# topling/toplingdb

Hardware: NVIDIA H100
Metric: compaction_input_kv_MB_per_s (higher is better)
Workload: dtype u8

## Files before the change

toplingdb_b200/csrc/api.cu:

```cuda
#include <cuda_runtime.h>
#include <stdio.h>
#include <stdlib.h>
#include <string.h>

#include <algorithm>
#include <map>
#include <memory>
#include <mutex>
#include <unordered_map>
#include <string>
#include <thread>
#include <type_traits>
#include <vector>

#include "../../include/b200c.h"
#include "inflate_rules.h"
#include "kernels.h"
#include "range_plan.h"
#include "scan.cuh"
#include "sst_host.h"

using namespace b200c;

namespace {

thread_local std::string g_err;
size_t g_last_want = 0;
std::mutex g_host_allocs_mu;
std::unordered_map<void*, std::pair<size_t, int>> g_host_allocs;
int fail(int code, const std::string& msg) {
  g_err = msg;
  return code;
}
std::string mem_note() {
  size_t fr = 0, tot = 0;
  cudaMemGetInfo(&fr, &tot);
  cudaGetLastError();
  return " (requested " + std::to_string(g_last_want) + " bytes; device free " + std::to_string(fr) + " of " + std::to_string(tot) + ")";
}
#define CU(call)                                                                                                  \
  do {                                                                                                            \
    cudaError_t e_ = (call);                                                                                      \
    if (e_ != cudaSuccess) {                                                                                      \
      cudaGetLastError();                                                                                         \
      return fail(e_ == cudaErrorMemoryAllocation ? B200C_ERR_OUT_OF_MEMORY : B200C_ERR_CUDA,                      \
                  std::string(#call) + ": " + cudaGetErrorString(e_) + (e_ == cudaErrorMemoryAllocation ? mem_note() : ""));  \
    }                                                                                                             \
  } while (0)

constexpr int kCacheDevices = 16;
inline size_t size_class(size_t n) {
  size_t c = 4096;
  while (c < n) c <<= 1;
  if (c >= (size_t(1) << 20)) {
    const size_t step = c >> 4;
    c = (c >> 1) + ((n - (c >> 1) + step - 1) / step) * step;
  }
  return c;
}
class BufCache {
 public:
  BufCache(bool host, const char* env, size_t default_mb) : host_(host) {
    const char* e = getenv(env);
    cap_ = (e ? strtoull(e, nullptr, 10) : default_mb) << 20;
  }
  void* take(int dev, size_t n, size_t* got) {
    if (dev < 0 || dev >= kCacheDevices || cap_ == 0) return nullptr;
    std::lock_guard<std::mutex> l(mu_);
    auto it = free_[dev].lower_bound(n);
    if (it == free_[dev].end() || it->first > 2 * n) return nullptr;
    void* p = it->second;
    *got = it->first;
    held_[dev] -= it->first;
    free_[dev].erase(it);
    return p;
  }
  bool give(int dev, void* p, size_t n) {
    if (dev < 0 || dev >= kCacheDevices || cap_ == 0) return false;
    std::lock_guard<std::mutex> l(mu_);
    if (held_[dev] + n > cap_) return false;
    free_[dev].emplace(n, p);
    held_[dev] += n;
    return true;
  }
  void flush(int dev) {
    if (dev < 0 || dev >= kCacheDevices) return;
    std::multimap<size_t, void*> drop;
    {
      std::lock_guard<std::mutex> l(mu_);
      drop.swap(free_[dev]);
      held_[dev] = 0;
    }
    for (auto& kv : drop) {
      if (host_) cudaFreeHost(kv.second);
      else cudaFree(kv.second);
    }
  }

 private:
  bool host_;
  size_t cap_ = 0;
  std::mutex mu_;
  std::multimap<size_t, void*> free_[kCacheDevices];
  size_t held_[kCacheDevices] = {};
};
BufCache& dev_cache() {
  static BufCache* c = new BufCache(false, "B200C_CACHE_DEVICE_MB", 49152);
  return *c;
}
BufCache& host_cache() {
  static BufCache* c = new BufCache(true, "B200C_CACHE_HOST_MB", 16384);
  return *c;
}
inline int current_device() {
  int d = -1;
  cudaGetDevice(&d);
  return d;
}
cudaError_t cached_alloc(bool host, size_t n, void** out, size_t* cap, int* dev_out) {
  const int dev = current_device();
  const size_t want = size_class(n);
  *dev_out = dev;
  BufCache& c = host ? host_cache() : dev_cache();
  if (void* p = c.take(dev, want, cap)) {
    *out = p;
    return cudaSuccess;
  }
  g_last_want = want;
  auto raw = [&]() { return host ? cudaHostAlloc(out, want, cudaHostAllocMapped | cudaHostAllocPortable) : cudaMalloc(out, want); };
  cudaError_t e = raw();
  if (e == cudaErrorMemoryAllocation) {
    cudaGetLastError();
    dev_cache().flush(dev);
    host_cache().flush(dev);
    e = raw();
  }
  if (e == cudaSuccess) *cap = want;
  return e;
}
void cached_free(bool host, void* p, size_t cap, int dev) {
  if (!p) return;
  if ((host ? host_cache() : dev_cache()).give(dev, p, cap)) return;
  if (host) cudaFreeHost(p);
  else cudaFree(p);
}

template <bool kPinned>
struct Buf {
  uint8_t* p = nullptr;
  size_t cap = 0;
  int dev = -1;
  Buf() = default;
  Buf(Buf&& o) noexcept : p(o.p), cap(o.cap), dev(o.dev) {
    o.p = nullptr;
    o.cap = 0;
  }
  Buf(const Buf&) = delete;
  Buf& operator=(const Buf&) = delete;
  ~Buf() { cached_free(kPinned, p, cap, dev); }
  cudaError_t reserve(size_t n) {
    if (n <= cap) return cudaSuccess;
    if (p) kPinned ? cudaFreeHost(p) : cudaFree(p);
    p = nullptr;
    cap = 0;
    void* q = nullptr;
    const cudaError_t e = cached_alloc(kPinned, n + (n >> 4) + 256, &q, &cap, &dev);
    if (e == cudaSuccess) p = static_cast<uint8_t*>(q);
    return e;
  }
  template <class T>
  T* as() const {
    return reinterpret_cast<T*>(p);
  }
};
using DevBuf = Buf<false>;
using HostBuf = Buf<true>;
static_assert(!std::is_copy_constructible_v<DevBuf> && !std::is_copy_assignable_v<DevBuf>, "a buffer has one owner");

struct KeyBufs {
  DevBuf pfx, tr, vref, meta;
  cudaError_t reserve(uint64_t n) {
    cudaError_t e = pfx.reserve(16 * (n + 1));
    if (e == cudaSuccess) e = tr.reserve(8 * (n + 1));
    if (e == cudaSuccess) e = vref.reserve(8 * (n + 1));
    if (e == cudaSuccess) e = meta.reserve(4 * (n + 1));
    return e;
  }
  KeyColsMut mut() const { return {pfx.as<ulonglong2>(), tr.as<uint64_t>(), vref.as<uint64_t>(), meta.as<uint32_t>()}; }
  KeyCols cols(uint64_t n) const { return {pfx.as<ulonglong2>(), tr.as<uint64_t>(), vref.as<uint64_t>(), meta.as<uint32_t>(), n}; }
};

struct Input {
  int level;
  uint64_t file_number;
  const uint8_t* data;
  uint64_t len;
  int mem_kind;
  DevBuf staged;
  cudaEvent_t up_ev = nullptr;
  bool uploaded = false;
  bool shared_copy = false;
  DevBuf index_inflated;
  std::vector<uint8_t> index_host;
  const uint8_t* dev = nullptr;
  InputTail tail;
};
constexpr uint64_t kTailFetch = 4096;
struct Output {
  b200c_file_meta meta;
  uint64_t dev_off = 0;
  uint64_t host_off = 0;
};
struct KernelTime {
  const char* name;
  cudaEvent_t a, b;
  float us;
};

}

struct b200c_job {
  b200c_params p;
  std::vector<uint64_t> snapshots, fct;
  std::string cf_name, db_id, db_session_id, db_host_id;
  std::vector<Input> inputs;
  std::vector<Output> outputs;
  b200c_stats stats;
  int stage_done = 0;
  uint64_t launches = 0;
  int sms = 132;
  cudaStream_t st = nullptr;
  cudaStream_t st2 = nullptr;
  cudaStream_t st_up = nullptr;
  cudaEvent_t ev[5] = {nullptr, nullptr, nullptr, nullptr, nullptr};
  cudaEvent_t evx[4] = {nullptr, nullptr, nullptr, nullptr};
  DevBuf files_d, blk_off, blk_size, blk_state, scan_tmp, run_start, small;
  KeyBufs dec, mrg;
  DevBuf splits, tile_state, snaps_d;
  DevBuf esz, eshared, tstat, nxt, disk, rows, tstate, grows, gstate, gflag, gsync, idx_contrib, idx_contrib_off, blocks, files_rec, idx_esz, idx_eoff, idx_sep, out_buf, out_base_d;
  uint64_t n_total = 0, n_out = 0, nblk_in = 0, nblocks_out = 0;
  uint32_t nfiles_out = 0, nruns = 0;
  DevBuf bloom_contrib, bloom_contrib_off;
  DevBuf bloom_hashes;
  DevBuf kv_arena, kv_offs, kv_klens;
  DevBuf run_bounds, run_first_d;
  std::vector<uint64_t> run_start_h;
  HostBuf host_out;
  std::vector<GpKey> gp_small, gp_large;
  std::vector<uint64_t> gp_size;
  std::vector<uint8_t> gp_same;
  DevBuf gp_keys_d, gp_ranks_d, gp_size_d, gp_same_d, gp_cuts_d;
  BoundKey range_lo{}, range_hi{};
  DevBuf clip_d;
  DevBuf cslot, cslot_off, arena;
  std::vector<cudaEvent_t> range_events;
  std::vector<std::string> range_bounds;
  cudaEvent_t wait_ev = nullptr;
  DevBuf vfiles_d, vrun_start;
  HostBuf pin_small, pin_tails, pin_rd, pin_up;
  size_t pin_up_used = 0;
  std::vector<KernelTime> ktimes;
  size_t kt_used = 0;
  size_t kt_begin(const char* name, cudaStream_t s = nullptr) {
    if (!p.profile) return 0;
    if (kt_used == ktimes.size()) {
      KernelTime k{name, nullptr, nullptr, 0.f};
      cudaEventCreate(&k.a);
      cudaEventCreate(&k.b);
      ktimes.push_back(k);
    }
    ktimes[kt_used].name = name;
    cudaEventRecord(ktimes[kt_used].a, s ? s : st);
    return kt_used++;
  }
  void kt_end(size_t slot = ~(size_t)0, cudaStream_t s = nullptr) {
    if (!p.profile) return;
    cudaEventRecord(ktimes[slot == ~(size_t)0 ? kt_used - 1 : slot].b, s ? s : st);
  }
};

namespace {

enum { kSlotErr = 0, kSlotTicket = 1, kSlotTotalIn = 2, kSlotMinS1 = 3, kSlotTotals = 4 , kSlotDecTicket = 6, kSlotGpCuts = 7, kSlotCounters = 8 , kSlotClip = 16 , kSlotStitchDone = 18, kSlotArena = 19 , kSmallSlots = 32 };

int map_dev_err(uint32_t e) {
  e &= ~(uint32_t)kFlagHasSingleDelete;
  if (e == 0) return B200C_OK;
  std::string m = "device reported:";
  int code = B200C_ERR_CORRUPTION;
  if (e & kErrCorruptBlock) m += " corrupt-block";
  if (e & kErrChecksum) m += " block-checksum-mismatch";
  if (e & kErrKeyOrder) m += " key-order/partition";
  if (e & kErrCountMismatch) m += " entry-count-mismatch";
  if (e & kErrParanoid) m += " Paranoid checksums do not match (an output file does not read back as written)";
  if (e & kErrSingleDelContract) m += " SingleDelete and Delete of the same key in one snapshot stripe (enforce_single_del_contracts)";
  const uint32_t unsup = kErrKeyTooLong | kErrValueTooLong | kErrBadType | kErrCompressed | kErrBlockTooLong | kErrIrregularRestarts |
                         kErrGroupTooLong | kErrSdWriteConflict;
  if (e & unsup) {
    if (!(e & ~(unsup))) code = B200C_ERR_NOT_SUPPORTED;
    if (e & kErrKeyTooLong) m += " user-key-longer-than-16-bytes";
    if (e & kErrValueTooLong) m += " value>=128MiB";
    if (e & kErrBadType) m += " value-type-outside-{Value,Deletion,SingleDeletion}";
    if (e & kErrGroupTooLong) m += " SingleDelete-on-a-key-with-too-many-versions-or-with-more-than-16-runs";
    if (e & kErrSdWriteConflict) m += " SingleDelete-with-an-earliest_write_conflict_snapshot";
    if (e & kErrCompressed) m += " compressed-block";
    if (e & kErrBlockTooLong) m += " output-block-with-too-many-entries";
    if (e & kErrIrregularRestarts) m += " restart-intervals-of-unequal-length";
  }
  if (e & kErrInternal) {
    m += " internal";
    code = B200C_ERR_CUDA;
  }
  return fail(code, m);
}

bool trailer_ok(const Input& in, const uint8_t* blk, uint64_t size, const uint8_t* trailer) {
  const uint32_t stored = (uint32_t)trailer[1] | (uint32_t)trailer[2] << 8 | (uint32_t)trailer[3] << 16 | (uint32_t)trailer[4] << 24;
  return !in.tail.checksum_type || host_block_checksum(in.tail.checksum_type, blk, size, trailer[0]) == stored;
}

int fetch_tail(b200c_job* j, Input& in, const uint8_t* prefetched = nullptr) {
  auto read = [&](uint64_t off, uint64_t n, std::vector<uint8_t>& buf) -> int {
    buf.resize(n);
    if (in.mem_kind == B200C_MEM_HOST) {
      memcpy(buf.data(), in.data + off, n);
    } else {
      CU(cudaMemcpyAsync(buf.data(), in.data + off, n, cudaMemcpyDeviceToHost, j->st));
      CU(cudaStreamSynchronize(j->st));
    }
    return B200C_OK;
  };
  if (in.len < 53) return fail(B200C_ERR_CORRUPTION, "input shorter than a footer");
  const uint64_t tail_n = std::min<uint64_t>(in.len, kTailFetch);
  std::vector<uint8_t> tail, tmp;
  int rc = B200C_OK;
  if (prefetched) tail.assign(prefetched, prefetched + tail_n);
  else rc = read(in.len - tail_n, tail_n, tail);
  if (rc) return rc;
  std::string e = parse_footer(tail.data() + tail_n - 53, in.len, &in.tail);
  if (!e.empty()) return fail(B200C_ERR_CORRUPTION, e);
  auto view = [&](uint64_t off, uint64_t n, const uint8_t** p) -> int {
    if (off >= in.len - tail_n && off + n <= in.len) {
      *p = tail.data() + (off - (in.len - tail_n));
      return B200C_OK;
    }
    int r = read(off, n, tmp);
    *p = tmp.data();
    return r;
  };
  const uint8_t* blk;
  rc = view(in.tail.meta_off, in.tail.meta_size + 5, &blk);
  if (rc) return rc;
  if (!trailer_ok(in, blk, in.tail.meta_size, blk + in.tail.meta_size)) return fail(B200C_ERR_CORRUPTION, "metaindex block checksum mismatch");
  std::map<std::string, std::pair<uint64_t, uint64_t>> meta;
  e = parse_metaindex(blk, in.tail.meta_size, &meta);
  if (!e.empty()) return fail(B200C_ERR_CORRUPTION, e);
  for (auto& kv : meta) {
    if (kv.first == "rocksdb.range_del") in.tail.has_range_del = true;
    if (kv.first.compare(0, 11, "fullfilter.") == 0 || kv.first.compare(0, 18, "partitionedfilter.") == 0) in.tail.has_filter = true;
    if (kv.first == "rocksdb.compression_dict") in.tail.has_dict = true;
  }
  auto it = meta.find("rocksdb.properties");
  if (it == meta.end()) return fail(B200C_ERR_CORRUPTION, "input has no properties block");
  in.tail.props_off = it->second.first;
  in.tail.props_size = it->second.second;
  if (in.tail.props_off + in.tail.props_size + 5 > in.len) return fail(B200C_ERR_CORRUPTION, "properties handle out of range");
  rc = view(in.tail.props_off, in.tail.props_size + 5, &blk);
  if (rc) return rc;
  if (!trailer_ok(in, blk, in.tail.props_size, blk + in.tail.props_size)) return fail(B200C_ERR_CORRUPTION, "properties block checksum mismatch");
  e = parse_properties(blk, in.tail.props_size, &in.tail);
  if (!e.empty()) return fail(B200C_ERR_CORRUPTION, e);
  if (in.tail.index_type != 0)
    return fail(B200C_ERR_NOT_SUPPORTED, "input index type " + std::to_string(in.tail.index_type) + " (only kBinarySearch runs on the device)");
  if (in.tail.has_range_del || in.tail.num_range_deletions)
    return fail(B200C_ERR_NOT_SUPPORTED, "input holds range tombstones (CompactionRangeDelAggregator is not on the device path)");
  if (in.tail.num_merge_operands) return fail(B200C_ERR_NOT_SUPPORTED, "input holds merge operands");
  if (in.tail.has_dict) return fail(B200C_ERR_NOT_SUPPORTED, "input uses a compression dictionary");
  if (!in.tail.comparator_name.empty() && in.tail.comparator_name != "leveldb.BytewiseComparator")
    return fail(B200C_ERR_NOT_SUPPORTED, "comparator " + in.tail.comparator_name + " (only leveldb.BytewiseComparator runs on the device)");
  if (in.tail.num_data_blocks > 0xffffffffull) return fail(B200C_ERR_NOT_SUPPORTED, "too many data blocks");
  return B200C_OK;
}

bool input_is_compressed(const Input& in) { return !in.tail.compression_name.empty() && in.tail.compression_name != "NoCompression"; }
int host_inflated_index(const Input& in, std::vector<uint8_t>* out) {
  out->clear();
  const uint64_t off = in.tail.index_off, size = in.tail.index_size;
  if (off + size + 5 > in.len) return fail(B200C_ERR_CORRUPTION, "index handle out of range");
  uint8_t trailer[5];
  if (in.mem_kind == B200C_MEM_HOST) memcpy(trailer, in.data + off + size, 5);
  else CU(cudaMemcpy(trailer, in.data + off + size, 5, cudaMemcpyDeviceToHost));
  if (trailer[0] == 0) return B200C_OK;
  if (trailer[0] != 2) return fail(B200C_ERR_NOT_SUPPORTED, "index block compressed with a codec the device path does not decode");
  std::vector<uint8_t> comp;
  const uint8_t* cp = in.data + off;
  if (in.mem_kind != B200C_MEM_HOST) {
    comp.resize(size);
    CU(cudaMemcpy(comp.data(), in.data + off, size, cudaMemcpyDeviceToHost));
    cp = comp.data();
  }
  if (!trailer_ok(in, cp, size, trailer)) return fail(B200C_ERR_CORRUPTION, "index block checksum mismatch");
  uint64_t u = 0;
  uint32_t h = 0;
  for (int sft = 0; h < 5 && h < size; sft += 7) {
    const uint8_t c = cp[h++];
    u |= (uint64_t)(c & 127) << sft;
    if (c < 128) break;
  }
  if (u < 8 || u > (1ull << 31)) return fail(B200C_ERR_CORRUPTION, "compressed index block announces a bad size");
  out->resize(u);
  std::unique_ptr<b200c::InfWork> iw(new b200c::InfWork);
  if (b200c::inflate_raw(cp + h, (uint32_t)(size - h), out->data(), (uint32_t)u, iw.get()) != (long)u)
    return fail(B200C_ERR_CORRUPTION, "compressed index block does not inflate to its announced size");
  return B200C_OK;
}

int host_index_block(const Input& in, std::vector<uint8_t>* buf, const uint8_t** blk, uint64_t* len) {
  if (in.tail.index_off + in.tail.index_size + 5 > in.len) return fail(B200C_ERR_CORRUPTION, "index handle out of range");
  buf->clear();
  if (input_is_compressed(in))
    if (int rc = host_inflated_index(in, buf)) return rc;
  if (!buf->empty()) {
    *blk = buf->data();
    *len = buf->size();
    return B200C_OK;
  }
  *blk = in.data + in.tail.index_off;
  *len = in.tail.index_size;
  if (in.mem_kind != B200C_MEM_HOST) {
    buf->resize(*len);
    CU(cudaMemcpy(buf->data(), *blk, *len, cudaMemcpyDeviceToHost));
    *blk = buf->data();
  }
  return B200C_OK;
}

void ikey_bytes(const KeyRec& k, uint8_t* out, uint32_t* len) {
  uint32_t n = 0;
  for (uint32_t t = 0; t < k.ulen && t < 16; t++) out[n++] = (uint8_t)((t < 8 ? k.hi >> (56 - 8 * t) : k.lo >> (56 - 8 * (t - 8))) & 0xff);
  for (int t = 0; t < 8; t++) out[n++] = (uint8_t)(k.tr >> (8 * t));
  *len = n;
}

int upload_small(b200c_job* j, void* dev_dst, const void* host_src, size_t n) {
  const size_t kCap = 256 * 1024;
  CU(j->pin_up.reserve(kCap));
  const size_t off = (j->pin_up_used + 15) & ~(size_t)15;
  if (off + n > kCap) {
    CU(cudaMemcpyAsync(dev_dst, host_src, n, cudaMemcpyHostToDevice, j->st));
    return B200C_OK;
  }
  memcpy(j->pin_up.p + off, host_src, n);
  j->pin_up_used = off + n;
  launch_copy_small(j->pin_up.p + off, dev_dst, (uint32_t)n, j->st);
  return B200C_OK;
}

constexpr size_t kRdSmall = kSmallSlots * 8;
int gather_small(b200c_job* j, const FileRec* files) {
  const uint64_t* small = j->small.as<uint64_t>();
  CU(j->pin_rd.reserve(kRdSmall + sizeof(FileRec) * (size_t)kMaxOutFiles));
  launch_gather_small(small, (uint32_t)kRdSmall, files, files ? small + kSlotTotals + 1 : nullptr, j->pin_rd.p, j->st);
  return B200C_OK;
}
void take_small(b200c_job* j, uint64_t* h, const FileRec* files, std::vector<FileRec>* frs) {
  memcpy(h, j->pin_rd.p, kRdSmall);
  if (files && frs) {
    uint64_t n = h[kSlotTotals + 1];
    if (n > kMaxOutFiles) n = kMaxOutFiles;
    frs->resize(n);
    memcpy(frs->data(), j->pin_rd.p + kRdSmall, sizeof(FileRec) * n);
  }
}
int read_small(b200c_job* j, uint64_t* h, const FileRec* files = nullptr, std::vector<FileRec>* frs = nullptr) {
  if (int rc = gather_small(j, files)) return rc;
  CU(cudaStreamSynchronize(j->st));
  CU(cudaGetLastError());
  take_small(j, h, files, frs);
  return B200C_OK;
}
int checked_sync(b200c_job* j, uint64_t* h, const FileRec* files = nullptr, std::vector<FileRec>* frs = nullptr) {
  if (int rc = read_small(j, h, files, frs)) return rc;
  return map_dev_err((uint32_t)h[kSlotErr]);
}

int write_tails(b200c_job* j, const std::vector<FileRec>& frs, const std::vector<uint64_t>& base_off) {
  const b200c_params& P = j->p;
  const uint32_t nfiles = (uint32_t)frs.size();
  j->outputs.resize(nfiles);
  std::vector<TailCopy> tcs(nfiles);
  for (uint32_t f = 0; f < nfiles; f++) {
    const FileRec& fr = frs[f];
    OutputTailInput ti;
    ti.checksum_type = P.checksum;
    ti.format_version = P.format_version;
    ti.data_size = fr.data_size;
    ti.index_size = fr.index_size;
    ti.filter_size = fr.filter_bytes ? fr.filter_bytes - 5 : 0;
    ti.filter_entries = fr.filter_entries;
    ti.num_entries = fr.n_entries;
    ti.num_deletions = fr.num_deletions;
    ti.raw_key_size = fr.raw_key_size;
    ti.raw_value_size = fr.raw_value_size;
    ti.num_data_blocks = fr.n_blocks;
    ti.index_key_is_user_key = !fr.index_has_seq && P.format_version > 2;
    ti.column_family_id = P.column_family_id;
    ti.column_family_name = j->cf_name;
    ti.db_id = j->db_id;
    ti.db_session_id = j->db_session_id;
    ti.db_host_id = j->db_host_id;
    ti.creation_time = P.creation_time;
    ti.oldest_key_time = P.oldest_key_time;
    ti.file_creation_time = j->fct.empty() ? 0 : j->fct[std::min<size_t>(f, j->fct.size() - 1)];
    ti.orig_file_number = P.first_file_number + f;
    std::vector<uint8_t> tail = build_output_tail(ti);
    const uint64_t tail_off = fr.data_size + fr.filter_bytes + fr.index_size + 5;
    if (tail_off + tail.size() > base_off[f + 1] - base_off[f]) return fail(B200C_ERR_CUDA, "internal: output image overflow");
    const size_t so = (size_t)f * 4096;
    if (tail.size() > 4096) return fail(B200C_ERR_CUDA, "internal: tail larger than its staging slot");
    memcpy(j->pin_tails.p + so, tail.data(), tail.size());
    tcs[f] = TailCopy{base_off[f] + tail_off, (uint32_t)so, (uint32_t)tail.size()};
    Output& o = j->outputs[f];
    memset(&o.meta, 0, sizeof o.meta);
    o.dev_off = base_off[f];
    o.meta.file_number = ti.orig_file_number;
    o.meta.file_size = tail_off + tail.size();
    o.meta.smallest_seqno = fr.smallest_seq;
    o.meta.largest_seqno = fr.largest_seq;
    o.meta.num_entries = fr.n_entries;
    o.meta.num_deletions = fr.num_deletions;
    o.meta.raw_key_size = fr.raw_key_size;
    o.meta.raw_value_size = fr.raw_value_size;
    o.meta.num_data_blocks = fr.n_blocks;
    o.meta.data_size = fr.data_size;
    o.meta.index_size = fr.index_size;
    ikey_bytes(fr.smallest, o.meta.smallest_ikey, &o.meta.smallest_ikey_len);
    ikey_bytes(fr.largest, o.meta.largest_ikey, &o.meta.largest_ikey_len);
    j->stats.total_output_bytes += o.meta.file_size;
  }
  const size_t rec_bytes = sizeof(TailCopy) * nfiles;
  memcpy(j->pin_small.p, tcs.data(), rec_bytes);
  launch_scatter_tails(reinterpret_cast<const TailCopy*>(j->pin_small.p), nfiles, j->pin_tails.p, j->out_buf.as<uint8_t>(), j->st);
  j->launches++;
  return B200C_OK;
}

int paranoid_reread(b200c_job* j, KeyCols mcols, const std::vector<FileRec>& frs, const std::vector<uint64_t>& base_off) {
  const b200c_params& P = j->p;
  cudaStream_t st = j->st;
  const uint32_t nfiles = (uint32_t)frs.size();
  const uint64_t nblocks = j->nblocks_out, n_out = mcols.n;
  uint64_t* small = j->small.as<uint64_t>();
  uint32_t* err = reinterpret_cast<uint32_t*>(small + kSlotErr);
  std::vector<FileDesc> ofd(nfiles);
  uint32_t g = 0, maxb = 0;
  for (uint32_t f = 0; f < nfiles; f++) {
    const FileRec& fr = frs[f];
    FileDesc d;
    memset(&d, 0, sizeof d);
    d.base = j->out_buf.as<uint8_t>() + base_off[f];
    d.len = j->outputs[f].meta.file_size;
    d.index_off = fr.data_size + fr.filter_bytes;
    d.index_size = (uint32_t)fr.index_size;
    d.value_delta = P.format_version >= 4;
    d.cksum = P.checksum;
    d.gblk_first = g;
    d.nblocks = (uint32_t)fr.n_blocks;
    d.index_user_key = (!fr.index_has_seq && P.format_version > 2) ? 1u : 0u;
    g += d.nblocks;
    maxb = std::max(maxb, d.nblocks);
    ofd[f] = d;
  }
  if (g != nblocks) return fail(B200C_ERR_CUDA, "internal: block count of the outputs changed");
  CU(j->vfiles_d.reserve(sizeof(FileDesc) * nfiles));
  if (int rc = upload_small(j, j->vfiles_d.p, ofd.data(), sizeof(FileDesc) * nfiles)) return rc;
  CU(cudaStreamSynchronize(st));
  CU(j->blk_off.reserve(8 * (nblocks + 1)));
  CU(j->blk_size.reserve(4 * (nblocks + 1)));
  CU(j->blk_state.reserve(8 * (nblocks + 1)));
  CU(j->vrun_start.reserve(8 * ((size_t)nfiles + 1)));
  CU(j->dec.reserve(n_out));
  if (const char* flip = getenv("B200C_TEST_FLIP_OUTPUT_BYTE")) {
    const uint64_t at = strtoull(flip, nullptr, 10);
    if (at < j->outputs[0].meta.file_size) launch_flip_byte(j->out_buf.as<uint8_t>() + base_off[0] + at, st);
  }
  CU(cudaMemsetAsync(small + kSlotDecTicket, 0, 8, st));
  CU(cudaMemsetAsync(small + kSlotTotalIn, 0, 8, st));
  CU(cudaMemsetAsync(j->vrun_start.p, 0, 8 * ((size_t)nfiles + 1), st));
  CU(cudaMemsetAsync(j->blk_state.p, 0, 8 * (nblocks + 1), st));
  const FileDesc* vf = j->vfiles_d.as<FileDesc>();
  j->kt_begin("verify.reread");
  launch_index_decode(vf, (int)nfiles, maxb, j->blk_off.as<uint64_t>(), j->blk_size.as<uint32_t>(), BoundKey{}, 0, BoundKey{}, 0, err, st);
  launch_block_decode_fused(vf, (int)nfiles, j->blk_off.as<uint64_t>(), j->blk_size.as<uint32_t>(), (uint32_t)nblocks, 1, n_out, j->dec.mut(),
                            j->blk_state.as<unsigned long long>(), reinterpret_cast<uint32_t*>(small + kSlotDecTicket),
                            j->vrun_start.as<uint64_t>(), small + kSlotTotalIn, err, j->sms, st);
  launch_compare_columns(mcols, j->dec.cols(n_out), n_out, err, j->sms, st);
  j->kt_end();
  j->launches += 3;
  uint64_t hv[kSmallSlots];
  if (int rc = read_small(j, hv)) return rc;
  if ((uint32_t)hv[kSlotErr] & ~(uint32_t)kFlagHasSingleDelete) {
    map_dev_err((uint32_t)hv[kSlotErr]);
    const std::string detail = g_err;
    return fail(B200C_ERR_CORRUPTION, "Paranoid checksums do not match: " + detail);
  }
  if (hv[kSlotTotalIn] != n_out) return fail(B200C_ERR_CORRUPTION, "Paranoid checksums do not match (entry count of the outputs)");
  return B200C_OK;
}

int encode_stage(b200c_job* j, KeyCols mcols, uint64_t n_out, uint32_t min_s1, uint32_t max_s1, EncodeWork& W, uint32_t* err, uint64_t* small) {
  const b200c_params& P = j->p;
  cudaStream_t st = j->st;
  uint64_t h[kSmallSlots];
  std::vector<FileRec> frs;
  std::vector<uint64_t> base_off;
  if (n_out) {
    if (P.index_block_restart_interval != 1)
      return fail(B200C_ERR_NOT_SUPPORTED, "index_block_restart_interval != 1 is not built on the device");
    EncodeParams ep{};
    ep.block_size = P.block_size;
    ep.block_size_limit = P.block_size_deviation ? (uint32_t)(((uint64_t)P.block_size * (100 - P.block_size_deviation) + 99) / 100) : 0;
    ep.restart_interval = P.block_restart_interval;
    ep.checksum = P.checksum;
    ep.format_version = P.format_version;
    ep.output_level = (uint32_t)P.output_level;
    ep.max_output_file_size = P.max_output_file_size;
    if (!j->gp_small.empty() && P.output_level > 0) {
      const uint32_t G = (uint32_t)j->gp_small.size();
      CU(j->gp_keys_d.reserve(sizeof(GpKey) * 2 * G));
      CU(j->gp_ranks_d.reserve(8 * 3 * (size_t)G));
      CU(j->gp_size_d.reserve(8 * (size_t)G));
      CU(j->gp_same_d.reserve(G + 16));
      CU(j->gp_cuts_d.reserve(sizeof(GpCut) * (2 * (size_t)G + 2)));
      GpKey* keys = j->gp_keys_d.as<GpKey>();
      if (int rc = upload_small(j, keys, j->gp_small.data(), sizeof(GpKey) * G)) return rc;
      if (int rc = upload_small(j, keys + G, j->gp_large.data(), sizeof(GpKey) * G)) return rc;
      if (int rc = upload_small(j, j->gp_size_d.p, j->gp_size.data(), 8 * (size_t)G)) return rc;
      if (int rc = upload_small(j, j->gp_same_d.p, j->gp_same.data(), G)) return rc;
      uint64_t* ranks = j->gp_ranks_d.as<uint64_t>();
      launch_gp_ranks(mcols, keys, keys + G, G, ranks, ranks + G, ranks + 2 * G, st);
      j->launches += 1;
      ep.gp.n = G;
      ep.gp.dynamic_file_size = P.level_compaction_dynamic_file_size;
      ep.gp.lo = ranks;
      ep.gp.eq = ranks + G;
      ep.gp.hi = ranks + 2 * G;
      ep.gp.size = j->gp_size_d.as<uint64_t>();
      ep.gp.next_same = j->gp_same_d.as<uint8_t>();
      ep.gp.target_output_file_size = P.target_output_file_size ? P.target_output_file_size : P.max_output_file_size;
      ep.gp.max_compaction_bytes = P.max_compaction_bytes ? P.max_compaction_bytes : ep.gp.target_output_file_size * 25;
      ep.gp_cuts = j->gp_cuts_d.as<GpCut>();
      ep.gp_ncuts = reinterpret_cast<uint32_t*>(small + kSlotGpCuts);
    }
    uint64_t hop = (uint64_t)(P.block_size - 1) / std::max<uint32_t>(min_s1, 1) + 3;
    if (hop > (uint64_t)kEncHalo) return fail(B200C_ERR_NOT_SUPPORTED, "block_size / smallest entry exceeds the encoder's 2048-entry block window");
    const uint32_t hc = (uint32_t)hop;
    const uint64_t etiles = (n_out + kEncTile - 1) / kEncTile;
    CU(j->rows.reserve(sizeof(TileRow) * etiles * hc));
    CU(j->tstate.reserve(sizeof(TileState) * etiles));
    const uint64_t egroups = (etiles + kEncGroupTiles - 1) / kEncGroupTiles;
    CU(j->grows.reserve(sizeof(TileRow) * egroups * hc));
    CU(j->gstate.reserve(sizeof(TileState) * egroups));
    CU(j->gflag.reserve(4 * egroups));
    CU(j->nxt.reserve(2 * (n_out + 1)));
    CU(j->disk.reserve(4 * (n_out + 1)));
    CU(j->files_rec.reserve(sizeof(FileRec) * (kMaxOutFiles + 2)));
    W.rows = j->rows.as<TileRow>();
    W.tstate = j->tstate.as<TileState>();
    W.grows = j->grows.as<TileRow>();
    W.gstate = j->gstate.as<TileState>();
    W.gflag = j->gflag.as<uint32_t>();
    W.nxt = j->nxt.as<uint16_t>();
    W.disk = j->disk.as<uint32_t>();
    W.files = j->files_rec.as<FileRec>();
    W.scan_tmp = j->scan_tmp.as<uint64_t>();
    CU(j->gsync.reserve(8 * egroups + 16));
    CU(cudaMemsetAsync(j->gsync.p, 0, 8 * egroups + 16, st));
    W.gdone = j->gsync.as<uint32_t>();
    W.gready = W.gdone + egroups;
    uint32_t* sflag = reinterpret_cast<uint32_t*>(small + kSlotStitchDone);
    CU(cudaEventRecord(j->evx[0], st));
    CU(cudaStreamWaitEvent(j->st2, j->evx[0], 0));
    {
      const size_t slot = j->kt_begin("~encode.stitch", j->st2);
      launch_encode_stitch(mcols, ep, W, etiles, hc, err, 1, sflag, j->st2, &j->launches);
      j->kt_end(slot, j->st2);
    }
    j->kt_begin("encode.tables");
    launch_encode_tables(mcols, ep, W, etiles, hc, max_s1, err, st);
    j->kt_end();
    {
      const size_t slot = j->kt_begin("~encode.stitch_retry", j->st2);
      launch_encode_stitch(mcols, ep, W, etiles, hc, err, 2, sflag, j->st2, &j->launches);
      j->kt_end(slot, j->st2);
    }
    CU(cudaEventRecord(j->evx[1], j->st2));
    CU(cudaStreamWaitEvent(st, j->evx[1], 0));
    j->kt_begin("encode.tilestate");
    launch_encode_tilestate(mcols, W, etiles, hc, err, st, &j->launches);
    j->kt_end();
    j->launches += 1;
    if (P.bloom_millibits_per_key) {
      j->kt_begin("encode.bloom_count");
      CU(j->bloom_hashes.reserve(8 * (n_out + 1)));
      launch_bloom_count(mcols, n_out, W.files, small + kSlotTotals + 1, P.bloom_millibits_per_key, j->bloom_hashes.as<uint64_t>(), j->sms, st);
      j->kt_end();
      j->launches += 2;
    }
    if (int rc = checked_sync(j, h, W.files, &frs)) return rc;
    const uint64_t nblocks = j->nblocks_out = h[kSlotTotals];
    const uint32_t nfiles = j->nfiles_out = (uint32_t)h[kSlotTotals + 1];
    if (nfiles == 0 || nfiles > kMaxOutFiles) return fail(B200C_ERR_CUDA, "internal: bad output file count");
    CU(j->blocks.reserve(sizeof(BlockRec) * (nblocks + 1)));
    CU(j->idx_esz.reserve(4 * (nblocks + 1)));
    CU(j->idx_eoff.reserve(8 * (nblocks + 1)));
    CU(j->idx_sep.reserve(sizeof(KeyRec) * (nblocks + 1)));
    W.blocks = j->blocks.as<BlockRec>();
    W.idx_esz = j->idx_esz.as<uint32_t>();
    W.idx_eoff = j->idx_eoff.as<uint64_t>();
    W.idx_sep = j->idx_sep.as<KeyRec>();
    CU(j->pin_tails.reserve((size_t)nfiles * 4096 + 64));
    CU(j->pin_small.reserve(sizeof(TailCopy) * nfiles));
    base_off.resize(nfiles + 1);
    uint64_t off = 0;
    for (uint32_t f = 0; f < nfiles; f++) {
      base_off[f] = off;
      uint64_t cap = frs[f].data_size + frs[f].filter_bytes + frs[f].n_blocks * 48 + 64 + 4096;
      off += (cap + 255) & ~255ull;
    }
    base_off[nfiles] = off;
    CU(j->out_buf.reserve(off + 256));
    {
      std::vector<uint64_t> coff(nfiles + 1, 0);
      for (uint32_t f = 0; f < nfiles; f++) coff[f + 1] = coff[f] + (frs[f].n_blocks * 48 + 64) / 1024 + 1;
      CU(j->idx_contrib.reserve(64 * (coff[nfiles] + 1)));
      CU(j->idx_contrib_off.reserve(8 * (nfiles + 1)));
      if (int rc = upload_small(j, j->idx_contrib_off.p, coff.data(), 8 * (nfiles + 1))) return rc;
      W.idx_contrib = j->idx_contrib.as<uint64_t>();
      W.idx_contrib_off = j->idx_contrib_off.as<uint64_t>();
    }
    std::vector<uint8_t*> bases(nfiles);
    for (uint32_t f = 0; f < nfiles; f++) bases[f] = j->out_buf.as<uint8_t>() + base_off[f];
    CU(j->out_base_d.reserve(8 * nfiles));
    if (int rc = upload_small(j, j->out_base_d.p, bases.data(), 8 * nfiles)) return rc;
    uint8_t* const* out_base_d = j->out_base_d.as<uint8_t*>();
    j->kt_begin("encode.blocklist");
    launch_encode_blocklist(mcols, ep, W, etiles, nblocks, err, st);
    j->kt_end();
    j->kt_begin("encode.filestats+index_size");
    launch_encode_index_size(mcols, ep, W, nblocks, j->sms, st, &j->launches);
    launch_encode_filestats(mcols, W, nfiles, st);
    j->kt_end();
    if (int rc = gather_small(j, W.files)) return rc;
    CU(cudaEventRecord(j->evx[2], st));
    uint64_t data_bytes = 0;
    for (uint32_t f = 0; f < nfiles; f++) data_bytes += frs[f].data_size;
    j->kt_begin("encode.emit");
    launch_encode_emit(mcols, ep, W, nblocks, out_base_d, data_bytes, err, j->sms, st);
    j->kt_end();
    j->launches += 3;
    CU(cudaStreamWaitEvent(j->st2, j->evx[2], 0));
    {
      const size_t slot = j->kt_begin("~encode.index", j->st2);
      launch_encode_index_write(ep, W, nblocks, nfiles, out_base_d, j->sms, j->st2, &j->launches);
      j->kt_end(slot, j->st2);
    }
    CU(cudaEventRecord(j->evx[3], j->st2));
    if (P.bloom_millibits_per_key) {
      j->kt_begin("encode.bloom_build");
      std::vector<uint64_t> boff(nfiles + 1, 0);
      uint64_t max_fb = 0;
      for (uint32_t f = 0; f < nfiles; f++) {
        boff[f + 1] = boff[f] + frs[f].filter_bytes / 1024 + 1;
        max_fb = std::max<uint64_t>(max_fb, frs[f].filter_bytes);
      }
      CU(j->bloom_contrib.reserve(64 * (boff[nfiles] + 1)));
      CU(j->bloom_contrib_off.reserve(8 * (nfiles + 1)));
      if (int rc = upload_small(j, j->bloom_contrib_off.p, boff.data(), 8 * (nfiles + 1))) return rc;
      launch_bloom_build(j->bloom_hashes.as<uint64_t>(), n_out, W.files, nfiles, (uint32_t)std::min<uint64_t>(max_fb, 0xffffffffull), P.bloom_millibits_per_key, P.checksum,
                         out_base_d, j->bloom_contrib.as<uint64_t>(), j->bloom_contrib_off.as<uint64_t>(), st);
      j->kt_end();
      j->launches += 3;
    }
    CU(cudaEventSynchronize(j->evx[2]));
    CU(cudaGetLastError());
    take_small(j, h, W.files, &frs);
    CU(cudaStreamWaitEvent(st, j->evx[3], 0));
    int rc = map_dev_err((uint32_t)h[kSlotErr]);
    if (rc == B200C_OK && frs.size() != nfiles) rc = fail(B200C_ERR_CUDA, "internal: output file count changed");
    if (rc == B200C_OK) rc = write_tails(j, frs, base_off);
    if (rc != B200C_OK) {
      cudaStreamSynchronize(st);
      return rc;
    }
    if (P.paranoid_file_checks) {
      if (int rc = checked_sync(j, h)) return rc;
      return paranoid_reread(j, mcols, frs, base_off);
    }
  }
  return B200C_OK;
}

int finish_run(b200c_job* j) {
  const b200c_params& P = j->p;
  cudaStream_t st = j->st;
  CU(cudaEventRecord(j->ev[3], st));
  if (P.output_mem == B200C_MEM_HOST) {
    uint64_t tot = 0;
    for (auto& o : j->outputs) {
      o.host_off = tot;
      tot += (o.meta.file_size + 63) & ~63ull;
    }
    CU(j->host_out.reserve(tot + 64));
    for (auto& o : j->outputs)
      CU(cudaMemcpyAsync(j->host_out.p + o.host_off, j->out_buf.as<uint8_t>() + o.dev_off, o.meta.file_size, cudaMemcpyDeviceToHost, st));
  }
  CU(cudaEventRecord(j->ev[4], st));
  {
    uint64_t h[kSmallSlots];
    if (int rc = checked_sync(j, h)) return rc;
  }
  float ms;
  cudaEventElapsedTime(&ms, j->ev[0], j->ev[1]);
  j->stats.decode_us = ms * 1000.0;
  cudaEventElapsedTime(&ms, j->ev[1], j->ev[2]);
  j->stats.merge_us = ms * 1000.0;
  cudaEventElapsedTime(&ms, j->ev[2], j->ev[3]);
  j->stats.encode_us = ms * 1000.0;
  cudaEventElapsedTime(&ms, j->ev[0], j->ev[4]);
  j->stats.total_us = ms * 1000.0;
  for (size_t i = 0; i < j->kt_used; i++) {
    float kms = 0;
    cudaEventElapsedTime(&kms, j->ktimes[i].a, j->ktimes[i].b);
    j->ktimes[i].us = kms * 1000.f;
  }
  j->stats.num_output_files = j->nfiles_out;
  j->stats.kernel_launches = j->launches;
  j->stage_done = 3;
  return B200C_OK;
}

int encode_columns(b200c_job* j, uint64_t n, const void* pfx, const void* tr, const void* vref, const void* meta, bool prepared = false);

int run_merge_encode(b200c_job* j, int until, KeyCols decc, RunBounds runs, uint64_t n_decoded, uint64_t N, bool clipped,
                     uint64_t range_value_bytes, uint64_t* small, uint32_t* err);

int job_prepare(b200c_job* j) {
  CU(cudaSetDevice(j->p.device));
  if (!j->st) {
    CU(cudaStreamCreateWithFlags(&j->st, cudaStreamNonBlocking));
    {
      int prio_lo = 0, prio_hi = 0;
      CU(cudaDeviceGetStreamPriorityRange(&prio_lo, &prio_hi));
      CU(cudaStreamCreateWithPriority(&j->st2, cudaStreamNonBlocking, prio_hi));
    }
    for (auto& e : j->ev) CU(cudaEventCreate(&e));
    for (auto& e : j->evx) CU(cudaEventCreateWithFlags(&e, cudaEventDisableTiming));
    cudaDeviceProp prop;
    CU(cudaGetDeviceProperties(&prop, j->p.device));
    j->sms = prop.multiProcessorCount;
  }
  j->outputs.clear();
  j->stage_done = 0;
  j->launches = 0;
  j->nblocks_out = 0;
  j->nfiles_out = 0;
  j->kt_used = 0;
  j->pin_up_used = 0;
  memset(&j->stats, 0, sizeof j->stats);
  return B200C_OK;
}

int run_job(b200c_job* j, int until) {
  const b200c_params& P = j->p;
  if (int rc = job_prepare(j)) return rc;
  cudaStream_t st = j->st;
  if (j->wait_ev) CU(cudaStreamWaitEvent(st, j->wait_ev, 0));
  const int k = (int)j->inputs.size();
  if (k == 0) return fail(B200C_ERR_INVALID_ARGUMENT, "job has no inputs");

  CU(cudaEventRecord(j->ev[0], st));
  uint64_t nblk = 0, n_props = 0, in_bytes = 0;
  bool any_compressed = false;
  std::vector<FileDesc> fds(k);
  {
    bool any_dev = false;
    for (int i = 0; i < k; i++) any_dev = any_dev || j->inputs[i].mem_kind != B200C_MEM_HOST;
    if (any_dev) {
      CU(j->pin_small.reserve((size_t)k * kTailFetch));
      for (int i = 0; i < k; i++) {
        const Input& in = j->inputs[i];
        if (in.mem_kind == B200C_MEM_HOST || in.len < 53) continue;
        const uint64_t tn = std::min<uint64_t>(in.len, kTailFetch);
        CU(cudaMemcpyAsync(j->pin_small.p + (size_t)i * kTailFetch, in.data + in.len - tn, tn, cudaMemcpyDeviceToHost, st));
      }
      CU(cudaStreamSynchronize(st));
    }
  }
  for (int i = 0; i < k; i++) {
    Input& in = j->inputs[i];
    int rc = fetch_tail(j, in, in.mem_kind != B200C_MEM_HOST && in.len >= 53 ? j->pin_small.p + (size_t)i * kTailFetch : nullptr);
    if (rc) return rc;
    if (in.mem_kind == B200C_MEM_HOST) {
      if (in.uploaded) {
        CU(cudaStreamWaitEvent(st, in.up_ev, 0));
        in.uploaded = false;
      } else {
        CU(in.staged.reserve(in.len + 64));
        CU(cudaMemcpyAsync(in.staged.p, in.data, in.len, cudaMemcpyHostToDevice, st));
      }
      in.dev = in.staged.as<uint8_t>();
    } else {
      if ((uintptr_t)in.data & 15) return fail(B200C_ERR_INVALID_ARGUMENT, "device input images must be 16-byte aligned");
      in.dev = in.data;
    }
    FileDesc& fd = fds[i];
    fd.base = in.dev;
    fd.len = in.len;
    fd.index_off = in.tail.index_off;
    fd.index_size = (uint32_t)in.tail.index_size;
    fd.value_delta = in.tail.format_version >= 4;
    fd.cksum = in.tail.checksum_type;
    fd.gblk_first = (uint32_t)nblk;
    fd.nblocks = (uint32_t)in.tail.num_data_blocks;
    fd.index_user_key = in.tail.index_key_is_user_key ? 1u : 0u;
    fd.index_ptr = nullptr;
    if (input_is_compressed(in)) any_compressed = true;
    nblk += in.tail.num_data_blocks;
    n_props += in.tail.num_entries;
    in_bytes += in.len;
    if (in.tail.index_size > 0xffffffffull) return fail(B200C_ERR_NOT_SUPPORTED, "index block >= 4 GiB");
  }
  if (any_compressed) {
    std::vector<int> rcs(k, B200C_OK);
    std::vector<std::string> msgs(k);
    std::vector<std::thread> pool;
    for (int i = 0; i < k; i++) {
      if (!input_is_compressed(j->inputs[i])) continue;
      pool.emplace_back([&, i]() {
        cudaSetDevice(P.device);
        rcs[i] = host_inflated_index(j->inputs[i], &j->inputs[i].index_host);
        if (rcs[i]) msgs[i] = g_err;
      });
    }
    for (auto& th : pool) th.join();
    for (int i = 0; i < k; i++) {
      if (rcs[i]) return fail(rcs[i], msgs[i]);
      Input& in = j->inputs[i];
      if (!input_is_compressed(in) || in.index_host.empty()) continue;
      CU(in.index_inflated.reserve(in.index_host.size() + 64));
      CU(cudaMemcpyAsync(in.index_inflated.p, in.index_host.data(), in.index_host.size(), cudaMemcpyHostToDevice, st));
      fds[i].index_ptr = in.index_inflated.as<uint8_t>();
      fds[i].index_size = (uint32_t)in.index_host.size();
    }
  }
  if (nblk > 0xfffffff0ull) return fail(B200C_ERR_NOT_SUPPORTED, "too many data blocks");
  j->nblk_in = nblk;
  j->n_total = n_props;
  j->stats.num_input_files = k;
  j->stats.total_input_bytes = in_bytes;
  j->stats.num_input_records = n_props;

  CU(j->small.reserve(kSmallSlots * 8));
  CU(cudaMemsetAsync(j->small.p, 0, kSmallSlots * 8, st));
  uint64_t* small = j->small.as<uint64_t>();
  uint32_t* err = reinterpret_cast<uint32_t*>(small + kSlotErr);
  {
    uint32_t ff = 0xffffffffu;
    if (int rc = upload_small(j, small + kSlotMinS1, &ff, 4)) return rc;
  }
  CU(j->files_d.reserve(sizeof(FileDesc) * k));
  if (int rc = upload_small(j, j->files_d.p, fds.data(), sizeof(FileDesc) * k)) return rc;
  const uint64_t N = n_props;
  CU(j->blk_off.reserve(8 * (nblk + 1)));
  CU(j->blk_size.reserve(4 * (nblk + 1)));
  CU(j->blk_state.reserve(8 * (nblk + 1)));
  CU(j->scan_tmp.reserve(8 * ((std::max<uint64_t>(nblk, N) / kScanTile) + 2)));
  CU(j->run_start.reserve(8 * (k + 1)));
  CU(j->dec.reserve(N));
  const FileDesc* files_d = j->files_d.as<FileDesc>();

  uint32_t maxb = 0;
  for (auto& f : fds) maxb = std::max(maxb, f.nblocks);
  if (nblk) {
    j->kt_begin("decode.index");
    launch_index_decode(files_d, k, maxb, j->blk_off.as<uint64_t>(), j->blk_size.as<uint32_t>(), j->range_lo, P.has_range_start, j->range_hi,
                        P.has_range_end, err, st);
    j->kt_end();
    j->launches++;
  }
  const uint8_t* arena = nullptr;
  if (nblk && any_compressed) {
    CU(j->cslot.reserve(4 * (nblk + 1)));
    CU(j->cslot_off.reserve(8 * (nblk + 1)));
    j->kt_begin("decode.inflate");
    launch_block_usize(files_d, j->blk_off.as<uint64_t>(), j->blk_size.as<uint32_t>(), (uint32_t)nblk, j->cslot.as<uint32_t>(), err, st);
    exclusive_scan<uint32_t>(j->cslot.as<uint32_t>(), j->cslot_off.as<uint64_t>(), nblk, j->scan_tmp.as<uint64_t>(), small + kSlotArena, st, &j->launches);
    uint64_t hc[kSmallSlots];
    if (int rc = checked_sync(j, hc)) return rc;
    CU(j->arena.reserve(hc[kSlotArena] + 256));
    arena = j->arena.as<uint8_t>();
    launch_inflate_blocks(files_d, j->blk_off.as<uint64_t>(), j->blk_size.as<uint32_t>(), j->cslot.as<uint32_t>(), j->cslot_off.as<uint64_t>(),
                          (uint32_t)nblk, j->arena.as<uint8_t>(), P.verify_input_checksums, err, j->sms, st);
    j->kt_end();
    j->launches += 3;
  }
  CU(cudaMemsetAsync(j->run_start.p, 0, 8 * (k + 1), st));
  if (nblk) {
    CU(cudaMemsetAsync(j->blk_state.p, 0, 8 * (nblk + 1), st));
    j->kt_begin("decode.blocks");
    launch_block_decode_fused(files_d, k, j->blk_off.as<uint64_t>(), j->blk_size.as<uint32_t>(), (uint32_t)nblk, P.verify_input_checksums, N,
                              j->dec.mut(), j->blk_state.as<unsigned long long>(), reinterpret_cast<uint32_t*>(small + kSlotDecTicket),
                              j->run_start.as<uint64_t>(), small + kSlotTotalIn, err, j->sms, st, arena);
    j->kt_end();
    j->launches++;
  }
  CU(cudaEventRecord(j->ev[1], st));
  const KeyCols decc = j->dec.cols(N);
  if (until == 1) {
    uint64_t h[kSmallSlots];
    j->run_start_h.resize(k + 1);
    CU(cudaMemcpyAsync(j->run_start_h.data(), j->run_start.p, 8 * (k + 1), cudaMemcpyDeviceToHost, st));
    if (int rc = checked_sync(j, h)) return rc;
    if (h[kSlotTotalIn] != N && !(P.has_range_start || P.has_range_end))
      return fail(B200C_ERR_CORRUPTION, "decoded entry count differs from rocksdb.num.entries");
    j->stage_done = 1;
    j->stats.kernel_launches = j->launches;
    return B200C_OK;
  }

  std::vector<uint32_t> run_first;
  for (int i = 0; i < k; i++)
    if (i == 0 || j->inputs[i].level <= 0 || j->inputs[i].level != j->inputs[i - 1].level) run_first.push_back((uint32_t)i);
  const uint32_t K = (uint32_t)run_first.size();
  run_first.push_back((uint32_t)k);
  if (K > (uint32_t)kMaxRuns) return fail(B200C_ERR_NOT_SUPPORTED, "more than 64 sorted runs (L0 files + levels)");
  j->nruns = K;
  CU(j->run_bounds.reserve(16 * (size_t)(K + 1)));
  CU(j->run_first_d.reserve(4 * (size_t)(K + 2)));
  if (int rc = upload_small(j, j->run_first_d.p, run_first.data(), 4 * (size_t)(K + 1))) return rc;
  launch_run_bounds(decc, j->run_start.as<uint64_t>(), j->run_first_d.as<uint32_t>(), K, j->run_bounds.as<uint64_t>(), err, st);
  j->launches++;
  RunBounds runs{j->run_bounds.as<uint64_t>(), j->run_bounds.as<uint64_t>() + K};
  const bool clipped = P.has_range_start || P.has_range_end;
  const uint64_t n_decoded = N;
  uint64_t N_in = N, range_value_bytes = 0;
  if (clipped) {
    CU(j->clip_d.reserve(16 * (size_t)(K + 1)));
    j->kt_begin("merge.clip");
    launch_clip_runs(decc, runs, K, j->range_lo, P.has_range_start, j->range_hi, P.has_range_end,
                     j->clip_d.as<uint64_t>(), reinterpret_cast<unsigned long long*>(small + kSlotClip), st);
    j->kt_end();
    j->launches++;
    uint64_t hc[kSmallSlots];
    if (int rc = checked_sync(j, hc)) return rc;
    N_in = hc[kSlotClip];
    range_value_bytes = hc[kSlotClip + 1];
    if (N_in > n_decoded) return fail(B200C_ERR_CUDA, "internal: clipped entry count exceeds the input");
    runs = RunBounds{j->clip_d.as<uint64_t>(), j->clip_d.as<uint64_t>() + K};
    j->stats.num_input_records = N_in;
  }
  return run_merge_encode(j, until, decc, runs, n_decoded, N_in, clipped, range_value_bytes, small, err);
}

int run_merge_encode(b200c_job* j, int until, KeyCols decc, RunBounds runs, uint64_t n_decoded, uint64_t N, bool clipped,
                     uint64_t range_value_bytes, uint64_t* small, uint32_t* err) {
  const b200c_params& P = j->p;
  cudaStream_t st = j->st;
  const size_t k = j->nruns;
  const uint64_t mtiles = (N + kMergeNominal - 1) / kMergeNominal;
  CU(j->splits.reserve(8 * (mtiles + 1) * k));
  CU(j->tile_state.reserve(8 * (mtiles + 1)));
  CU(cudaMemsetAsync(j->tile_state.p, 0, 8 * (mtiles + 1), st));
  CU(j->snaps_d.reserve(8 * (P.num_snapshots + 1)));
  if (P.num_snapshots)
    if (int rc = upload_small(j, j->snaps_d.p, j->snapshots.data(), 8 * P.num_snapshots)) return rc;
  CU(j->mrg.reserve(N));
  CU(j->esz.reserve(4 * (N + 1)));
  CU(j->eshared.reserve(N + 1));
  CU(j->tstat.reserve(sizeof(TileStat) * (mtiles + 2)));
  MergeParams mp;
  mp.nruns = (uint32_t)k;
  mp.bottommost = P.bottommost_level != 0;
  mp.nsnapshots = P.num_snapshots;
  mp.snapshots = j->snaps_d.as<uint64_t>();
  mp.earliest_snapshot = P.num_snapshots ? j->snapshots[0] : kMaxSeq;
  mp.filter = P.compaction_filter;
  mp.ttl = P.ttl;
  mp.now = P.ttl_now;
  mp.write_conflict_snapshot = P.earliest_write_conflict_snapshot != 0 && P.earliest_write_conflict_snapshot < kMaxSeq;
  MergeCounters* counters = reinterpret_cast<MergeCounters*>(small + kSlotCounters);
  EncodeWork W;
  memset(&W, 0, sizeof W);
  W.esz = j->esz.as<uint32_t>();
  W.eshared = j->eshared.as<uint8_t>();
  W.tstat = j->tstat.as<TileStat>();
  W.min_s1 = reinterpret_cast<uint32_t*>(small + kSlotMinS1);
  W.totals = small + kSlotTotals;
  if (N) {
    j->kt_begin("merge.partition");
    launch_merge_partition(decc, runs, (uint32_t)k, N, mtiles, j->splits.as<uint64_t>(), err, j->sms, st);
    j->kt_end();
    const MergeSizes msz{W.esz, W.eshared, W.tstat, W.min_s1};
    W.tprefix = j->tile_state.as<unsigned long long>();
    W.nstat = mtiles;
    j->kt_begin("merge.tiles");
    launch_merge_tiles(decc, runs, mp, N, mtiles, j->splits.as<uint64_t>(),
                       j->tile_state.as<unsigned long long>(), reinterpret_cast<uint32_t*>(small + kSlotTicket), j->mrg.mut(), counters, msz, err, st);
    j->kt_end();
    j->kt_begin("merge.sizes_fix");
    launch_merge_sizes_fix(j->mrg.cols(0), j->tile_state.as<unsigned long long>(), mtiles, msz, st);
    j->kt_end();
    j->launches += 3;
  }
  CU(cudaEventRecord(j->ev[2], st));
  uint64_t h[kSmallSlots];
  if (int rc = checked_sync(j, h)) return rc;
  if (clipped ? h[kSlotTotalIn] > n_decoded : h[kSlotTotalIn] != n_decoded)
    return fail(B200C_ERR_CORRUPTION, "decoded entry count differs from rocksdb.num.entries");
  MergeCounters mc;
  memcpy(&mc, h + kSlotCounters, sizeof mc);
  const uint64_t n_out = mc.n_out;
  j->n_out = n_out;
  j->stats.num_output_records = n_out;
  j->stats.num_input_deletion_records = mc.n_input_deletions;
  j->stats.num_records_replaced = mc.n_hidden;
  j->stats.num_expired_deletion_records = mc.n_obsolete;
  j->stats.num_record_drop_user = mc.n_user_drop;
  j->stats.total_input_raw_key_bytes = mc.raw_key_bytes;
  {
    uint64_t all = 0;
    for (auto& in : j->inputs) all += in.tail.raw_value_size;
    if (clipped) all = range_value_bytes;
    j->stats.total_input_raw_value_bytes = all - mc.raw_value_bytes;
  }
  if (until == 2) {
    j->stage_done = 2;
    j->stats.kernel_launches = j->launches;
    return B200C_OK;
  }

  if (int rc = encode_stage(j, j->mrg.cols(n_out), n_out, (uint32_t)h[kSlotMinS1], (uint32_t)(h[kSlotMinS1] >> 32), W, err, small)) return rc;
  return finish_run(j);
}

int encode_columns(b200c_job* j, uint64_t n, const void* pfx, const void* tr, const void* vref, const void* meta, bool prepared) {
  int rc = prepared ? B200C_OK : job_prepare(j);
  if (rc) return rc;
  cudaStream_t st = j->st;
  CU(cudaEventRecord(j->ev[0], st));
  CU(cudaEventRecord(j->ev[1], st));
  CU(cudaEventRecord(j->ev[2], st));
  CU(j->small.reserve(kSmallSlots * 8));
  CU(cudaMemsetAsync(j->small.p, 0, kSmallSlots * 8, st));
  uint64_t* small = j->small.as<uint64_t>();
  uint32_t* err = reinterpret_cast<uint32_t*>(small + kSlotErr);
  uint32_t ff = 0xffffffffu;
  CU(cudaMemcpyAsync(small + kSlotMinS1, &ff, 4, cudaMemcpyHostToDevice, st));
  MergeCounters* counters = reinterpret_cast<MergeCounters*>(small + kSlotCounters);
  CU(cudaMemcpyAsync(&counters->n_out, &n, 8, cudaMemcpyHostToDevice, st));
  CU(j->esz.reserve(4 * (n + 1)));
  CU(j->eshared.reserve(n + 1));
  CU(j->tstat.reserve(sizeof(TileStat) * (n / kEncTile + 2)));
  CU(j->tile_state.reserve(8 * (n / kEncTile + 2)));
  CU(j->scan_tmp.reserve(8 * ((n / kScanTile) + 2)));
  EncodeWork W;
  memset(&W, 0, sizeof W);
  W.esz = j->esz.as<uint32_t>();
  W.eshared = j->eshared.as<uint8_t>();
  W.tstat = j->tstat.as<TileStat>();
  W.min_s1 = reinterpret_cast<uint32_t*>(small + kSlotMinS1);
  W.totals = small + kSlotTotals;
  KeyCols mcols{static_cast<const ulonglong2*>(pfx), static_cast<const uint64_t*>(tr), static_cast<const uint64_t*>(vref),
                static_cast<const uint32_t*>(meta), n};
  if (n) {
    j->kt_begin("encode.sizes");
    W.tprefix = j->tile_state.as<unsigned long long>();
    W.nstat = (n + kEncTile - 1) / kEncTile;
    launch_encode_sizes(mcols, reinterpret_cast<const unsigned long long*>(&counters->n_out), W, j->tile_state.as<unsigned long long>(), n, j->sms, st);
    j->kt_end();
    j->launches++;
  }
  uint64_t h[kSmallSlots];
  rc = checked_sync(j, h);
  if (rc) return rc;
  rc = encode_stage(j, mcols, n, (uint32_t)h[kSlotMinS1], (uint32_t)(h[kSlotMinS1] >> 32), W, err, small);
  if (rc) return rc;
  j->n_out = n;
  j->stats.num_output_records = n;
  return finish_run(j);
}

}

extern "C" {

const char* b200c_last_error(void) { return g_err.c_str(); }
uint32_t b200c_abi_version(void) { return B200C_ABI_VERSION; }
int b200c_device_count(void) {
  int n = 0;
  cudaError_t e = cudaGetDeviceCount(&n);
  if (e != cudaSuccess) {
    cudaGetLastError();
    g_err = std::string("cudaGetDeviceCount: ") + cudaGetErrorString(e);
    return -B200C_ERR_NO_DEVICE;
  }
  return n;
}

void b200c_params_init(b200c_params* p) {
  memset(p, 0, sizeof *p);
  p->abi_version = B200C_ABI_VERSION;
  p->device = 0;
  p->output_level = 1;
  p->bottommost_level = 0;
  p->max_output_file_size = 64ull << 20;
  p->block_size = 4096;
  p->block_size_deviation = 10;
  p->block_restart_interval = 16;
  p->index_block_restart_interval = 1;
  p->format_version = 5;
  p->checksum = B200C_CKSUM_XXH3;
  p->verify_input_checksums = 1;
  p->level_compaction_dynamic_file_size = 1;
  p->column_family_name = "default";
  p->output_mem = B200C_MEM_HOST;
}

int b200c_job_create(const b200c_params* p, b200c_job** out) {
  if (!p || !out) return fail(B200C_ERR_INVALID_ARGUMENT, "null argument");
  if (p->abi_version != B200C_ABI_VERSION) return fail(B200C_ERR_INVALID_ARGUMENT, "ABI version mismatch");
  if (p->block_size < 64 || p->block_size > (1u << 20)) return fail(B200C_ERR_INVALID_ARGUMENT, "block_size out of range");
  if (p->block_restart_interval < 1) return fail(B200C_ERR_INVALID_ARGUMENT, "block_restart_interval < 1");
  if (p->block_size_deviation > 100) return fail(B200C_ERR_INVALID_ARGUMENT, "block_size_deviation > 100");
  if (p->format_version < 3 || p->format_version > 5) return fail(B200C_ERR_NOT_SUPPORTED, "output format_version must be 3..5");
  if (p->compaction_filter != B200C_FILTER_NONE && p->compaction_filter != B200C_FILTER_REMOVE_EMPTY_VALUE &&
      p->compaction_filter != B200C_FILTER_TTL)
    return fail(B200C_ERR_NOT_SUPPORTED, "compaction filter is not one of the built-in device filters");
  if (p->checksum != B200C_CKSUM_XXH3 && p->checksum != B200C_CKSUM_CRC32C && p->checksum != B200C_CKSUM_NONE)
    return fail(B200C_ERR_NOT_SUPPORTED, "output checksum must be kNoChecksum, kCRC32c or kXXH3");
  for (uint32_t i = 1; i < p->num_snapshots; i++)
    if (p->snapshots[i] <= p->snapshots[i - 1]) return fail(B200C_ERR_INVALID_ARGUMENT, "snapshots must be strictly ascending");
  int n = b200c_device_count();
  if (n <= 0) return fail(B200C_ERR_NO_DEVICE, "no CUDA device: the compaction path has no CPU implementation in this library");
  if (p->device < 0 || p->device >= n) return fail(B200C_ERR_INVALID_ARGUMENT, "device ordinal out of range");
  b200c_job* j = new b200c_job();
  j->p = *p;
  if (p->num_snapshots) j->snapshots.assign(p->snapshots, p->snapshots + p->num_snapshots);
  if (p->num_file_creation_times) j->fct.assign(p->file_creation_times, p->file_creation_times + p->num_file_creation_times);
  j->cf_name = p->column_family_name ? p->column_family_name : "";
  j->db_id = p->db_id ? p->db_id : "";
  j->db_session_id = p->db_session_id ? p->db_session_id : "";
  j->db_host_id = p->db_host_id ? p->db_host_id : "";
  j->p.snapshots = nullptr;
  j->p.file_creation_times = nullptr;
  auto pack = [](const void* key, uint32_t len, GpKey* k) {
    uint8_t b[16] = {0};
    if (len) memcpy(b, key, len);
    k->hi = k->lo = 0;
    for (int i = 0; i < 8; i++) k->hi = (k->hi << 8) | b[i], k->lo = (k->lo << 8) | b[8 + i];
    k->ulen = len;
    k->pad = 0;
  };
  for (uint32_t i = 0; i < p->num_grandparents; i++) {
    const b200c_grandparent& g = p->grandparents[i];
    if (g.smallest_len > kMaxUserKey || g.largest_len > kMaxUserKey || (!g.smallest_user_key && g.smallest_len) ||
        (!g.largest_user_key && g.largest_len)) {
      delete j;
      return fail(B200C_ERR_NOT_SUPPORTED, "grandparent boundary key longer than 16 bytes");
    }
    GpKey a, b;
    pack(g.smallest_user_key, g.smallest_len, &a);
    pack(g.largest_user_key, g.largest_len, &b);
    if (i && (j->gp_large[i - 1].hi > a.hi || (j->gp_large[i - 1].hi == a.hi && (j->gp_large[i - 1].lo > a.lo ||
              (j->gp_large[i - 1].lo == a.lo && j->gp_large[i - 1].ulen > a.ulen))))) {
      delete j;
      return fail(B200C_ERR_INVALID_ARGUMENT, "grandparents must be sorted and non-overlapping");
    }
    j->gp_small.push_back(a);
    j->gp_large.push_back(b);
    j->gp_size.push_back(g.file_size);
  }
  for (uint32_t i = 0; i < p->num_grandparents; i++) {
    const bool same = i + 1 < p->num_grandparents && j->gp_small[i + 1].hi == j->gp_large[i].hi &&
                      j->gp_small[i + 1].lo == j->gp_large[i].lo && j->gp_small[i + 1].ulen == j->gp_large[i].ulen;
    j->gp_same.push_back(same ? 1 : 0);
  }
  j->p.grandparents = nullptr;
  if (p->bloom_millibits_per_key && (p->format_version < 5 || p->bloom_millibits_per_key < 1000)) {
    delete j;
    return fail(B200C_ERR_NOT_SUPPORTED, "Bloom filter block needs format_version >= 5 (FastLocalBloom) and >= 1000 millibits per key");
  }
  if ((p->has_range_start && (p->range_start_len > kMaxUserKey || (!p->range_start_user_key && p->range_start_len))) ||
      (p->has_range_end && (p->range_end_len > kMaxUserKey || (!p->range_end_user_key && p->range_end_len)))) {
    delete j;
    return fail(B200C_ERR_NOT_SUPPORTED, "sub-compaction range bound longer than 16 bytes");
  }
  if (p->has_range_start) pack(p->range_start_user_key, p->range_start_len, &j->range_lo);
  if (p->has_range_end) pack(p->range_end_user_key, p->range_end_len, &j->range_hi);
  j->p.range_start_user_key = j->p.range_end_user_key = nullptr;
  memset(&j->stats, 0, sizeof j->stats);
  *out = j;
  return B200C_OK;
}

int b200c_job_add_input(b200c_job* j, int level, uint64_t file_number, const void* data, uint64_t len, int mem_kind) {
  if (!j || !data) return fail(B200C_ERR_INVALID_ARGUMENT, "null argument");
  if (mem_kind != B200C_MEM_HOST && mem_kind != B200C_MEM_DEVICE && mem_kind != B200C_MEM_HOST_DEFERRED)
    return fail(B200C_ERR_INVALID_ARGUMENT, "bad mem_kind");
  const bool deferred = mem_kind == B200C_MEM_HOST_DEFERRED;
  if (deferred) mem_kind = B200C_MEM_HOST;
  j->inputs.emplace_back();
  Input& in = j->inputs.back();
  in.level = level;
  in.file_number = file_number;
  in.data = static_cast<const uint8_t*>(data);
  in.len = len;
  in.mem_kind = mem_kind;
  if (mem_kind == B200C_MEM_HOST && !deferred && len >= (1u << 20)) {
    if (cudaSetDevice(j->p.device) == cudaSuccess && (j->st_up || cudaStreamCreateWithFlags(&j->st_up, cudaStreamNonBlocking) == cudaSuccess) &&
        in.staged.reserve(len + 64) == cudaSuccess && cudaEventCreateWithFlags(&in.up_ev, cudaEventDisableTiming) == cudaSuccess &&
        cudaMemcpyAsync(in.staged.p, data, len, cudaMemcpyHostToDevice, j->st_up) == cudaSuccess &&
        cudaEventRecord(in.up_ev, j->st_up) == cudaSuccess) {
      in.uploaded = true;
    } else {
      cudaGetLastError();
    }
  }
  return B200C_OK;
}

namespace {
static_assert(kPlanMaxUserKey == kMaxUserKey, "range planning and the device columns agree on the key width");
}

int b200c_job_plan_ranges(b200c_job* j, uint32_t max_ranges, uint64_t min_range_bytes, uint8_t* keys, uint32_t* key_lens, uint32_t* n_boundaries) {
  if (!j || !n_boundaries || (max_ranges > 1 && (!keys || !key_lens))) return fail(B200C_ERR_INVALID_ARGUMENT, "null argument");
  *n_boundaries = 0;
  if (max_ranges <= 1 || j->inputs.empty()) return B200C_OK;
  if (b200c_device_count() <= 0) return fail(B200C_ERR_NO_DEVICE, "no CUDA device");
  CU(cudaSetDevice(j->p.device));
  std::vector<Anchor> anchors;
  uint64_t total = 0;
  std::vector<uint8_t> idx;
  for (Input& in : j->inputs) {
    if (int rc = fetch_tail(j, in)) return rc;
    total += in.tail.data_size ? in.tail.data_size : in.len;
    if (in.tail.num_data_blocks < 2) continue;
    const uint8_t* blk;
    uint64_t blk_len;
    if (int rc = host_index_block(in, &idx, &blk, &blk_len)) return rc;
    const std::string e = index_anchors(blk, blk_len, in.tail, 128, &anchors);
    if (!e.empty()) return fail(B200C_ERR_CORRUPTION, e);
  }
  const std::vector<Anchor> bnd = plan_boundaries(std::move(anchors), total, max_ranges, min_range_bytes);
  uint32_t nb = 0;
  for (const Anchor& a : bnd) {
    memcpy(keys + (size_t)nb * kMaxUserKey, a.key, kMaxUserKey);
    key_lens[nb] = a.klen;
    nb++;
  }
  *n_boundaries = nb;
  return B200C_OK;
}

int b200c_job_create_sub(b200c_job* parent, const b200c_params* p, b200c_job** out) {
  if (!parent || !p || !out) return fail(B200C_ERR_INVALID_ARGUMENT, "null argument");
  if (p->device != parent->p.device) return fail(B200C_ERR_INVALID_ARGUMENT, "a sub-job runs on its parent's device");
  if (parent->inputs.empty()) return fail(B200C_ERR_STATE, "parent job has no inputs");
  CU(cudaSetDevice(parent->p.device));
  for (Input& in : parent->inputs) {
    if (in.mem_kind != B200C_MEM_HOST || !parent->range_events.empty()) continue;
    if (in.uploaded) {
      CU(cudaEventSynchronize(in.up_ev));
    } else if (!in.shared_copy) {
      CU(in.staged.reserve(in.len + 64));
      CU(cudaMemcpy(in.staged.p, in.data, in.len, cudaMemcpyHostToDevice));
    }
    in.shared_copy = true;
  }
  b200c_job* j = nullptr;
  if (int rc = b200c_job_create(p, &j)) return rc;
  for (const Input& in : parent->inputs) {
    j->inputs.emplace_back();
    Input& s = j->inputs.back();
    s.level = in.level;
    s.file_number = in.file_number;
    s.len = in.len;
    s.mem_kind = B200C_MEM_DEVICE;
    s.data = in.mem_kind == B200C_MEM_HOST ? in.staged.as<uint8_t>() : in.data;
  }
  if (!parent->range_events.empty()) {
    size_t r = parent->range_events.size() - 1;
    if (p->has_range_end) {
      const std::string end(static_cast<const char*>(p->range_end_user_key ? p->range_end_user_key : ""), p->range_end_len);
      for (size_t i = 0; i < parent->range_bounds.size(); i++)
        if (parent->range_bounds[i] == end) {
          r = i;
          break;
        }
    }
    j->wait_ev = parent->range_events[r];
  }
  *out = j;
  return B200C_OK;
}

int b200c_job_upload_by_ranges(b200c_job* j, const uint8_t* keys, const uint32_t* key_lens, uint32_t nb) {
  if (!j || (nb && (!keys || !key_lens))) return fail(B200C_ERR_INVALID_ARGUMENT, "null argument");
  if (j->inputs.empty()) return fail(B200C_ERR_STATE, "job has no inputs");
  if (!j->range_events.empty()) return fail(B200C_ERR_STATE, "the inputs of this job are already uploaded by ranges");
  if (b200c_device_count() <= 0) return fail(B200C_ERR_NO_DEVICE, "no CUDA device");
  CU(cudaSetDevice(j->p.device));
  if (!j->st_up) CU(cudaStreamCreateWithFlags(&j->st_up, cudaStreamNonBlocking));
  std::vector<Anchor> bounds(nb);
  for (uint32_t r = 0; r < nb; r++) {
    if (key_lens[r] > (uint32_t)kMaxUserKey) return fail(B200C_ERR_NOT_SUPPORTED, "range boundary longer than 16 bytes");
    memset(&bounds[r], 0, sizeof(Anchor));
    memcpy(bounds[r].key, keys + (size_t)r * kMaxUserKey, key_lens[r]);
    bounds[r].klen = key_lens[r];
    if (r && anchor_cmp(bounds[r - 1], bounds[r]) >= 0) return fail(B200C_ERR_INVALID_ARGUMENT, "range boundaries must be strictly ascending");
  }
  const size_t k = j->inputs.size();
  std::vector<std::vector<uint64_t>> cuts(k, std::vector<uint64_t>(nb, 0));
  std::vector<uint64_t> data_end(k, 0);
  std::vector<uint8_t> idx;
  for (size_t f = 0; f < k; f++) {
    Input& in = j->inputs[f];
    if (in.mem_kind != B200C_MEM_HOST || in.uploaded)
      return fail(B200C_ERR_STATE, "upload by ranges needs host inputs added with B200C_MEM_HOST_DEFERRED");
    if (int rc = fetch_tail(j, in)) return rc;
    const uint8_t* blk;
    uint64_t blk_len;
    if (int rc = host_index_block(in, &idx, &blk, &blk_len)) return rc;
    const std::string e = index_range_cuts(blk, blk_len, in.tail, in.len, bounds.data(), nb, cuts[f].data(), &data_end[f]);
    if (!e.empty()) return fail(B200C_ERR_CORRUPTION, e);
    CU(in.staged.reserve(in.len + 64));
  }
  for (size_t f = 0; f < k; f++) {
    Input& in = j->inputs[f];
    if (in.len > data_end[f])
      CU(cudaMemcpyAsync(in.staged.as<uint8_t>() + data_end[f], in.data + data_end[f], in.len - data_end[f], cudaMemcpyHostToDevice, j->st_up));
  }
  j->range_events.resize((size_t)nb + 1, nullptr);
  for (uint32_t r = 0; r <= nb; r++) {
    for (size_t f = 0; f < k; f++) {
      Input& in = j->inputs[f];
      const uint64_t lo = r == 0 ? 0 : cuts[f][r - 1], hi = r == nb ? data_end[f] : cuts[f][r];
      if (hi > lo) CU(cudaMemcpyAsync(in.staged.as<uint8_t>() + lo, in.data + lo, hi - lo, cudaMemcpyHostToDevice, j->st_up));
    }
    CU(cudaEventCreateWithFlags(&j->range_events[r], cudaEventDisableTiming));
    CU(cudaEventRecord(j->range_events[r], j->st_up));
  }
  j->range_bounds.clear();
  for (uint32_t r = 0; r < nb; r++) j->range_bounds.emplace_back(reinterpret_cast<const char*>(bounds[r].key), bounds[r].klen);
  for (Input& in : j->inputs) in.shared_copy = true;
  return B200C_OK;
}

int b200c_host_alloc(int device, uint64_t bytes, void** out) {
  if (!out) return fail(B200C_ERR_INVALID_ARGUMENT, "null argument");
  *out = nullptr;
  if (b200c_device_count() <= 0) return fail(B200C_ERR_NO_DEVICE, "no CUDA device");
  CU(cudaSetDevice(device));
  size_t cap = 0;
  int dev = -1;
  CU(cached_alloc(true, bytes ? bytes : 1, out, &cap, &dev));
  std::lock_guard<std::mutex> l(g_host_allocs_mu);
  g_host_allocs[*out] = {cap, dev};
  return B200C_OK;
}
void b200c_host_free(void* p) {
  if (!p) return;
  std::pair<size_t, int> rec{0, -1};
  {
    std::lock_guard<std::mutex> l(g_host_allocs_mu);
    auto it = g_host_allocs.find(p);
    if (it == g_host_allocs.end()) return;
    rec = it->second;
    g_host_allocs.erase(it);
  }
  cached_free(true, p, rec.first, rec.second);
}

int b200c_job_run(b200c_job* j) {
  if (!j) return fail(B200C_ERR_INVALID_ARGUMENT, "null job");
  return run_job(j, 3);
}
int b200c_job_run_until(b200c_job* j, int stage) {
// ... 194 lines not shown
```

toplingdb_b200/csrc/encode.cu:

```cuda
#include "bloom_rules.h"
#include "common.cuh"
#include "gp_rules.h"
#include "kernels.h"
#include "scan.cuh"

namespace b200c {

constexpr int kTT = kEncTile;
constexpr int kW = kEncTile + kEncHalo;
constexpr int kEncThreads = 256;

__global__ void __launch_bounds__(256)
encode_sizes_kernel(KeyCols m, const unsigned long long* __restrict__ n_dev, uint32_t* __restrict__ esz, uint8_t* __restrict__ eshared,
                    TileStat* __restrict__ tstat, unsigned long long* __restrict__ tprefix, uint32_t* __restrict__ min_s1) {
  const uint64_t n = *n_dev;
  const uint64_t ntiles = (n + kEncTile - 1) / kEncTile;
  uint32_t mn = 0xffffffffu, mxs = 0;
  __shared__ unsigned long long red[5];
  __shared__ uint32_t s_mn, s_mx;
  if (threadIdx.x == 0) {
    s_mn = 0xffffffffu;
    s_mx = 0;
  }
  for (uint64_t tile = blockIdx.x; tile < ntiles; tile += gridDim.x) {
// ... 73 lines not shown
    if (threadIdx.x == 0) {
      tstat[tile] = TileStat{red[0], red[1], red[2], red[3], red[4]};
      tprefix[tile] = t1;
    }
    __syncthreads();
  }
  mn = __reduce_min_sync(0xffffffffu, mn);
  mxs = __reduce_max_sync(0xffffffffu, mxs);
  __syncthreads();
  if ((threadIdx.x & 31) == 0) {
    atomicMin(&s_mn, mn);
    atomicMax(&s_mx, mxs);
  }
  __syncthreads();
  if (threadIdx.x == 0 && s_mn != 0xffffffffu) {
    atomicMin(min_s1, s_mn);
    atomicMax(min_s1 + 1, s_mx);
  }
}

template <typename PT>
struct Window {
  PT P[kW + 1];
  uint32_t Q[kW];
  uint64_t ws[33];
  uint32_t wlen;
  uint32_t at_end;
  uint32_t smax;
};

template <typename PT>
__device__ void build_window(Window<PT>& w, const KeyCols& m, const uint32_t* esz, const uint8_t* eshared, uint64_t n, uint64_t tile,
                             uint32_t R) {
  const uint64_t wstart = tile * (uint64_t)kTT;
  const uint32_t wlen = (uint32_t)((n - wstart) < (uint64_t)kW ? (n - wstart) : (uint64_t)kW);
  uint32_t mx = 0;
  if (threadIdx.x == 0) w.smax = 0;
  constexpr int kBatch = 8;
  for (uint32_t jb = 0; jb < wlen; jb += kBatch * kEncThreads) {
    uint32_t s1v[kBatch], shv[kBatch], mtv[kBatch];
#pragma unroll
    for (int i = 0; i < kBatch; i++) {
      const uint32_t j = jb + i * kEncThreads + threadIdx.x;
      s1v[i] = shv[i] = mtv[i] = 0;
      if (j < wlen) {
        s1v[i] = esz[wstart + j];
        shv[i] = eshared[wstart + j];
        mtv[i] = m.meta[wstart + j];
      }
    }
#pragma unroll
    for (int i = 0; i < kBatch; i++) {
      const uint32_t j = jb + i * kEncThreads + threadIdx.x;
      if (j < wlen) {
        const uint32_t sh = shv[i], ks = meta_ulen(mtv[i]) + 8;
        const uint32_t d = 1u + varint_len32(ks) + sh - varint_len32(sh) - varint_len32(ks - sh);
        w.Q[j] = d;
        w.P[j + 1] = (PT)s1v[i];
        mx = s1v[i] + d > mx ? s1v[i] + d : mx;
      }
    }
  }
  __syncthreads();
  constexpr int kPer = ((kW + kEncThreads - 1) / kEncThreads) | 1;
  const uint32_t j0 = threadIdx.x * kPer;
  uint64_t loc[kPer], sum = 0;
#pragma unroll
  for (int i = 0; i < kPer; i++) {
    const uint32_t j = j0 + i;
    loc[i] = j < wlen ? w.P[j + 1] : 0;
    sum += loc[i];
  }
#pragma unroll
  for (int d = 16; d; d >>= 1) {
    uint32_t o = __shfl_xor_sync(0xffffffffu, mx, d);
    mx = o > mx ? o : mx;
  }
  uint64_t ex = block_excl_scan64(sum, nullptr, w.ws);
  if ((threadIdx.x & 31) == 0) atomicMax(&w.smax, mx);
#pragma unroll
  for (int i = 0; i < kPer; i++) {
    uint32_t j = j0 + i;
    if (j <= wlen && j <= (uint32_t)kW) w.P[j] = (PT)ex;
    ex += loc[i];
  }
  if (threadIdx.x == 0) {
    w.wlen = wlen;
    w.at_end = (wstart + wlen == n);
  }
  __syncthreads();
  if ((R & (R - 1)) == 0 && R <= 32 && kEncThreads % R == 0) {
    const uint32_t c = threadIdx.x & (R - 1), part = threadIdx.x / R, nparts = kEncThreads / R;
    const uint32_t per_class = (wlen + R - 1) / R;
    const uint32_t chunk = (per_class + nparts - 1) / nparts;
    const uint32_t first = part * chunk;
    uint32_t sum = 0;
    for (uint32_t i = 0; i < chunk; i++) {
      const uint32_t j = c + R * (first + i);
      if (j < wlen) sum += w.Q[j];
    }
    __shared__ uint32_t part_sum[kEncThreads];
    part_sum[threadIdx.x] = sum;
    __syncthreads();
    uint32_t run = 0;
    for (uint32_t q = 0; q < part; q++) run += part_sum[c + R * q];
    for (uint32_t i = 0; i < chunk; i++) {
      const uint32_t j = c + R * (first + i);
      if (j < wlen) {
        run += w.Q[j];
        w.Q[j] = run;
      }
    }
    __syncthreads();
  } else {
    for (uint32_t off = R; off < wlen; off <<= 1) {
      uint32_t add[kPer];
#pragma unroll
      for (int i = 0; i < kPer; i++) {
        uint32_t j = j0 + i;
        add[i] = (j < wlen && j >= off) ? w.Q[j - off] : 0;
      }
      __syncthreads();
#pragma unroll
      for (int i = 0; i < kPer; i++) {
        uint32_t j = j0 + i;
        if (j < wlen) w.Q[j] += add[i];
      }
      __syncthreads();
    }
  }
}

struct CutParams {
  uint32_t BS, LIM, R, rshift;
};
__host__ __device__ __forceinline__ CutParams make_cut(uint32_t bs, uint32_t lim, uint32_t r) {
  CutParams c{bs, lim, r, 32};
  if ((r & (r - 1)) == 0) {
    uint32_t sft = 0;
    while ((1u << sft) < r) sft++;
    c.rshift = sft;
  }
  return c;
}
__device__ __forceinline__ uint32_t div_r(uint32_t x, const CutParams& cp) { return cp.rshift < 32 ? x >> cp.rshift : x / cp.R; }
template <typename PT>
struct BlockStart {
  uint32_t a;
  PT pa;
  uint32_t qa;
};
template <typename PT>
__device__ __forceinline__ BlockStart<PT> block_start(const Window<PT>& w, uint32_t a, const CutParams& cp) {
  BlockStart<PT> s;
  s.a = a;
  s.pa = w.P[a];
  s.qa = a >= cp.R ? w.Q[a - cp.R] : 0u;
  return s;
}
template <typename PT>
__device__ __forceinline__ PT blk_payload(const Window<PT>& w, const BlockStart<PT>& s, uint32_t b, const CutParams& cp) {
  const uint32_t nrm1 = div_r(b - 1 - s.a, cp);
  const uint32_t last = s.a + cp.R * nrm1;
  const uint32_t q = w.Q[last] - s.qa;
  return (PT)(w.P[b] - s.pa) + (PT)q + (PT)(4u * (nrm1 + 1) + 4u);
}
template <typename PT>
__device__ __forceinline__ PT blk_payload(const Window<PT>& w, uint32_t a, uint32_t b, const CutParams& cp) {
  return blk_payload(w, block_start(w, a, cp), b, cp);
}
template <typename PT>
__device__ __forceinline__ uint32_t next_block(const Window<PT>& w, uint32_t a, const CutParams& cp, uint32_t hint, PT* pay_out) {
  const uint32_t wlen = w.wlen;
  const BlockStart<PT> bs = block_start(w, a, cp);
  PT thr = (PT)(cp.BS - 1);
  if (cp.LIM) {
    thr = (PT)cp.LIM;
    const uint64_t guard = (uint64_t)w.smax + 7;
    if (cp.BS > guard && cp.BS - guard - 1 > thr) thr = (PT)(cp.BS - guard - 1);
  }
  uint32_t lo = a + 1, hi = wlen + 1;
  PT ec_hi = 0;
  if (hint > a + 1 && hint <= wlen) {
    const PT ph = blk_payload(w, bs, hint, cp);
    uint32_t step = 1;
    if (ph > thr) {
      hi = hint;
      ec_hi = ph;
      while (hi - lo >= step) {
        const uint32_t mid = hi - step;
        const PT pm = blk_payload(w, bs, mid, cp);
        if (pm > thr) {
          hi = mid;
          ec_hi = pm;
          step <<= 1;
        } else {
          lo = mid + 1;
          break;
        }
      }
    } else {
      lo = hint + 1;
      while (lo + step - 1 <= wlen) {
        const uint32_t mid = lo + step - 1;
        const PT pm = blk_payload(w, bs, mid, cp);
        if (pm > thr) {
          hi = mid;
          ec_hi = pm;
          break;
        }
        lo = mid + 1;
        step <<= 1;
      }
    }
  }
  while (lo < hi) {
    const uint32_t mid = (lo + hi) >> 1;
    const PT pm = blk_payload(w, bs, mid, cp);
    if (pm > thr) {
      hi = mid;
      ec_hi = pm;
    } else {
      lo = mid + 1;
    }
  }
  if (lo >= wlen) {
    if (!w.at_end) return 0xffffffffu;
    *pay_out = blk_payload(w, bs, wlen, cp);
    return wlen;
  }
  PT ec = ec_hi;
  uint32_t m = lo - a;
  uint32_t mr = cp.rshift < 32 ? (m & (cp.R - 1)) : (m % cp.R);
  for (uint32_t b = lo; b < wlen; b++) {
    if (ec >= cp.BS) {
      *pay_out = ec;
      return b;
    }
    const PT s1 = (PT)(w.P[b + 1] - w.P[b]);
    const bool at_restart = mr == 0;
    const PT d = at_restart ? (PT)(w.Q[b] - (b >= cp.R ? w.Q[b - cp.R] : 0u)) : (PT)0;
    if (cp.LIM) {
      const PT dfull = at_restart ? d : (PT)(w.Q[b] - (b >= cp.R ? w.Q[b - cp.R] : 0u));
      if (ec + s1 + dfull + 3 + (at_restart ? 4 : 0) > cp.BS) {
        *pay_out = ec;
        return b;
      }
    }
    ec += s1 + (at_restart ? d + 4 : 0);
    mr = mr + 1 == cp.R ? 0 : mr + 1;
  }
  if (!w.at_end) return 0xffffffffu;
  *pay_out = ec;
  return wlen;
}

constexpr int kEncGroup = kEncGroupTiles;
__device__ __forceinline__ TileRow ldcg_row(const TileRow* p) {
  const uint4 v = __ldcg(reinterpret_cast<const uint4*>(p));
  TileRow r;
  r.exit = v.x;
  r.nblk = v.y;
  r.bytes = (uint64_t)v.z | ((uint64_t)v.w << 32);
  return r;
}
static_assert(sizeof(TileRow) == 16, "TileRow is moved as one 16-byte vector");
__device__ void compose_group(const EncodeWork& wk, uint64_t n, uint64_t g, uint64_t t0, uint64_t t1, uint32_t hc) {
  const uint64_t gstart = t0 * (uint64_t)kTT;
  for (uint32_t c = threadIdx.x; c < hc; c += blockDim.x) {
    uint64_t x = gstart + c, bytes = 0;
    uint32_t nb = 0;
    bool bad = false;
    for (uint64_t t = t0; t < t1 && x < n; t++) {
      const uint64_t tstart = t * (uint64_t)kTT, tend = (tstart + kTT) < n ? (tstart + kTT) : n;
      if (x >= tend) continue;
      const uint64_t cc = x - tstart;
      if (cc >= hc) {
        bad = true;
        break;
      }
      const TileRow r = ldcg_row(&wk.rows[t * hc + cc]);
      if (r.exit == 0xffffffffu) {
        bad = true;
        break;
      }
      x = tstart + r.exit;
      nb += r.nblk;
      bytes += r.bytes;
    }
    TileRow o;
    o.exit = bad ? 0xffffffffu : (uint32_t)(x - gstart);
    o.nblk = nb;
    o.bytes = bytes;
    wk.grows[g * hc + c] = o;
  }
}

template <typename PT>
struct TablesSmem {
  Window<PT> w;
  uint16_t nxt[kTT];
  uint32_t disk[kTT];
};
template <typename PT>
__global__ void __launch_bounds__(kEncThreads, sizeof(PT) == 4 ? 3 : 2)
encode_tables_kernel(KeyCols m, EncodeParams ep, EncodeWork wk, uint64_t n, uint32_t hc, uint16_t* __restrict__ g_nxt,
                     uint32_t* __restrict__ g_disk, uint32_t* __restrict__ err) {
  extern __shared__ __align__(16) uint8_t smem_raw[];
  TablesSmem<PT>& s = *reinterpret_cast<TablesSmem<PT>*>(smem_raw);
  const uint64_t tile = blockIdx.x, wstart = tile * (uint64_t)kTT;
  const CutParams cp = make_cut(ep.block_size, ep.block_size_limit, ep.restart_interval);
  build_window(s.w, m, wk.esz, wk.eshared, n, tile, cp.R);
  const uint32_t tl = s.w.wlen < (uint32_t)kTT ? s.w.wlen : (uint32_t)kTT;
  {
    constexpr int kPer = kTT / kEncThreads;
    const PT total = s.w.P[s.w.wlen];
    const uint32_t per_block = total ? (uint32_t)(((uint64_t)ep.block_size * s.w.wlen) / total) : 0;
    uint32_t prev_pos = 0, prev_b = 0;
    for (int i = 0; i < kPer; i++) {
      const uint32_t j = threadIdx.x * kPer + ((i + threadIdx.x) & (kPer - 1));
      if (j >= tl) continue;
      uint32_t hint = j + 1 + per_block;
      if (prev_b) hint = prev_b + j - prev_pos;
      if (hint > s.w.wlen) hint = s.w.wlen;
      PT pay = 0;
      uint32_t b = next_block(s.w, j, cp, hint, &pay);
      prev_pos = j;
      prev_b = b == 0xffffffffu ? 0 : b;
      uint16_t nx = 0xffff;
      uint32_t dk = 0;
      if (b != 0xffffffffu) {
        nx = (uint16_t)b;
        const uint64_t pay5 = (uint64_t)pay + 5;
        dk = pay5 > 0xffffffffull ? 0xffffffffu : (uint32_t)pay5;
      }
      s.nxt[j] = nx;
      s.disk[j] = dk;
    }
  }
  __syncthreads();
  for (uint32_t j = threadIdx.x; j < tl; j += kEncThreads) {
    g_nxt[wstart + j] = s.nxt[j];
    g_disk[wstart + j] = s.disk[j];
  }
  __syncthreads();
  for (uint32_t c = threadIdx.x; c < hc; c += kEncThreads) {
    uint32_t x = c, nb = 0;
    uint64_t bytes = 0;
    bool bad = false;
    while (x < tl) {
      uint32_t y = s.nxt[x];
      if (y == 0xffff || y <= x) {
        bad = true;
        break;
      }
      bytes += s.disk[x];
      nb++;
      x = y;
    }
    TileRow r;
    r.exit = bad ? 0xffffffffu : x;
    r.nblk = nb;
    r.bytes = bytes;
    wk.rows[tile * hc + c] = r;
  }
  (void)err;
  __threadfence();
  __syncthreads();
  __shared__ uint32_t s_last;
  const uint64_t g = tile / kEncGroupTiles, ntiles = (n + kTT - 1) / kTT;
  const uint64_t t0 = g * kEncGroupTiles, t1 = (t0 + kEncGroupTiles) < ntiles ? (t0 + kEncGroupTiles) : ntiles;
  if (threadIdx.x == 0) s_last = atomicAdd(&wk.gdone[g], 1u) + 1 == (uint32_t)(t1 - t0);
  __syncthreads();
  if (!s_last) return;
  __threadfence();
  compose_group(wk, n, g, t0, t1, hc);
  __threadfence();
  __syncthreads();
  if (threadIdx.x == 0) atomicExch(&wk.gready[g], 1u);
}

struct WalkState {
  uint64_t a;
  uint64_t blk;
  uint64_t foff;
  uint64_t f_first_entry, f_first_blk;
  uint32_t f;
};
__device__ __forceinline__ void close_file(FileRec* files, WalkState& st, uint64_t end_entry, uint32_t* err) {
  if (files == nullptr) return;
  if (st.f >= kMaxOutFiles) {
    atomicOr(err, kErrInternal);
    return;
  }
  FileRec& fr = files[st.f];
  fr.first_entry = st.f_first_entry;
  fr.n_entries = end_entry - st.f_first_entry;
  fr.first_block = st.f_first_blk;
  fr.n_blocks = st.blk - st.f_first_blk;
  fr.data_size = st.foff;
  fr.index_size = 0;
  fr.raw_key_size = fr.raw_value_size = fr.num_deletions = 0;
  fr.smallest_seq = ~0ull;
  fr.largest_seq = 0;
  fr.index_has_seq = 0;
  fr.filter_entries = fr.filter_bytes = 0;
}
__device__ __forceinline__ uint64_t single_entry_block_bytes(const KeyCols& m, const EncodeWork& wk, uint64_t y) {
  uint32_t sh = wk.eshared[y], ks = meta_ulen(m.meta[y]) + 8;
  uint64_t s0 = (uint64_t)wk.esz[y] + 1u + varint_len32(ks) + sh - varint_len32(sh) - varint_len32(ks - sh);
  return s0 + 4 + 4 + 5;
}
__device__ uint64_t truncated_block_bytes(const KeyCols& m, const EncodeWork& wk, uint32_t R, uint64_t a, uint64_t e) {
  uint64_t sum = 0;
  for (uint64_t j0 = a; j0 < e; j0 += 8) {
    uint32_t s1[8], sh[8], mt[8];
#pragma unroll
    for (int q = 0; q < 8; q++) {
      const uint64_t j = j0 + q;
      s1[q] = sh[q] = mt[q] = 0;
      if (j < e) {
        s1[q] = wk.esz[j];
        sh[q] = wk.eshared[j];
        mt[q] = m.meta[j];
      }
    }
#pragma unroll
    for (int q = 0; q < 8; q++) {
      const uint64_t j = j0 + q;
      if (j < e) {
        sum += s1[q];
        if ((j - a) % R == 0) {
          const uint32_t ks = meta_ulen(mt[q]) + 8;
          sum += 1u + varint_len32(ks) + sh[q] - varint_len32(sh[q]) - varint_len32(ks - sh[q]);
        }
      }
    }
  }
  const uint64_t nrest = (e - a + R - 1) / R;
  return sum + 4 * nrest + 4 + 5;
}

template <int kGp>
__device__ __forceinline__ bool chase_tile(const uint16_t* nxt, const uint32_t* disk, uint64_t tstart, uint32_t tl, uint64_t n,
                                           const EncodeParams& ep, const KeyCols& m, const EncodeWork& wk, WalkState& st_io, FileRec* files,
                                           BlockRec* emit, uint64_t emit_cap, uint32_t* err, GpState* gp_io = nullptr) {
  WalkState st = st_io;
  GpState g{};
  if (kGp == 1) g = *gp_io;
  uint32_t ncuts = 0, cut_i = 0;
  if (kGp == 2) {
    ncuts = *ep.gp_ncuts;
    uint32_t lo = 0, hi = ncuts;
    while (lo < hi) {
      const uint32_t mid = (lo + hi) >> 1;
      if (ep.gp_cuts[mid].entry <= st.a) lo = mid + 1;
      else hi = mid;
    }
    cut_i = lo;
  }
  const uint64_t tend = tstart + tl;
  const bool cut_files = ep.output_level != 0;
  const uint64_t fmax = ep.max_output_file_size;
  bool ok = true;
  while (st.a < tend) {
    const uint32_t x = (uint32_t)(st.a - tstart);
    const uint32_t yr = nxt[x];
    if (yr == 0xffff || yr <= x) {
      ok = false;
      break;
    }
    const uint64_t y = tstart + yr;
    if (kGp != 0 && cut_files) {
      uint64_t cut_at = ~0ull, cut_bytes = 0;
      if (kGp == 1) {
        uint64_t ev;
        while ((ev = gp_next_event(g, ep.gp)) <= y && ev < n) {
          const uint64_t prev_overlapped = g.overlapped;
          const uint32_t crossed = gp_advance(g, ep.gp, ev);
          if (ev > st.f_first_entry && gp_should_stop(g, ep.gp, crossed, prev_overlapped, st.foff)) {
            cut_at = ev;
            cut_bytes = ev == y ? (uint64_t)disk[x] : truncated_block_bytes(m, wk, ep.restart_interval, st.a, ev);
            const uint32_t ci = *ep.gp_ncuts;
            ep.gp_cuts[ci] = GpCut{cut_at, cut_bytes};
            *ep.gp_ncuts = ci + 1;
            break;
          }
        }
      } else if (cut_i < ncuts && ep.gp_cuts[cut_i].entry <= y) {
        cut_at = ep.gp_cuts[cut_i].entry;
        cut_bytes = ep.gp_cuts[cut_i].block_bytes;
        cut_i++;
      }
      if (cut_at != ~0ull) {
        if (emit && st.blk < emit_cap) emit[st.blk] = BlockRec{st.a, st.foff, st.f, (uint32_t)(cut_at - st.a)};
        st.foff += cut_bytes;
        st.blk++;
        close_file(files, st, cut_at, err);
        st.f++;
        st.foff = 0;
        st.f_first_entry = cut_at;
        st.f_first_blk = st.blk;
        st.a = cut_at;
        if (kGp == 1) gp_file_started(g, ep.gp, cut_at);
        continue;
      }
    }
    if (emit && st.blk < emit_cap) emit[st.blk] = BlockRec{st.a, st.foff, st.f, (uint32_t)(y - st.a)};
    st.foff += disk[x];
    st.blk++;
    if (y >= n) {
      close_file(files, st, n, err);
      st.a = n;
      st.f++;
      break;
    }
    if (cut_files && st.foff >= fmax) {
      const uint64_t d1 = single_entry_block_bytes(m, wk, y);
      if (emit && st.blk < emit_cap) emit[st.blk] = BlockRec{y, st.foff, st.f, 1u};
      st.foff += d1;
      st.blk++;
      close_file(files, st, y + 1, err);
      st.f++;
      st.foff = 0;
      st.f_first_entry = y + 1;
      st.f_first_blk = st.blk;
      st.a = y + 1;
      if (kGp == 1 && y + 1 < n) {
        gp_advance(g, ep.gp, y + 1);
        gp_file_started(g, ep.gp, y + 1);
      }
    } else {
      st.a = y;
    }
  }
  st_io = st;
  if (kGp == 1) *gp_io = g;
  return ok;
}

struct StitchSmem {
  uint16_t nxt[kTT];
  uint32_t disk[kTT];
  uint64_t nd[kTT];
  WalkState st;
  GpState gp;
  uint64_t g, t, tend;
  uint64_t ga, ta;
  uint32_t gn, tn;
  uint64_t req_idx;
  uint32_t req;
  uint32_t done;
  uint32_t refill;
};
template <typename T, int kDepth>
__device__ __forceinline__ void coop_copy_cg(T* __restrict__ dst, const T* __restrict__ src, uint32_t n) {
  const uint32_t nt = blockDim.x;
  for (uint32_t base = 0; base < n; base += kDepth * nt) {
    T v[kDepth];
#pragma unroll
    for (int k = 0; k < kDepth; k++) {
      const uint32_t i = base + k * nt + threadIdx.x;
      if (i < n) v[k] = __ldcg(src + i);
    }
#pragma unroll
    for (int k = 0; k < kDepth; k++) {
      const uint32_t i = base + k * nt + threadIdx.x;
      if (i < n) dst[i] = v[k];
    }
  }
}
__global__ void __launch_bounds__(kEncThreads)
encode_stitch_kernel(KeyCols m, EncodeParams ep, EncodeWork wk, uint64_t n, uint64_t ntiles, uint32_t hc, uint32_t cache_bytes,
                     uint32_t* __restrict__ err, uint32_t attempt, uint32_t* __restrict__ sflag, uint32_t timeout_ns) {
  extern __shared__ __align__(16) uint8_t smem_raw[];
  StitchSmem& s = *reinterpret_cast<StitchSmem*>(smem_raw);
  if (attempt == 2 && *reinterpret_cast<volatile uint32_t*>(sflag) != 0) return;
  bool first_wait = attempt == 1;
  TileRow* gcache = reinterpret_cast<TileRow*>(smem_raw + ((sizeof(StitchSmem) + 15) & ~(size_t)15));
  TileRow* tcache = gcache + cache_bytes / sizeof(TileRow);
  const uint32_t cache_rows = cache_bytes / (uint32_t)sizeof(TileRow) / hc;
  const uint64_t ngroups = (ntiles + kEncGroup - 1) / kEncGroup;
  if (threadIdx.x == 0) {
    s.st = WalkState{0, 0, 0, 0, 0, 0};
    s.gp = gp_initial_state();
    if (ep.gp.n) {
      *ep.gp_ncuts = 0;
      if (n) gp_advance(s.gp, ep.gp, 0);
    }
    s.done = (n == 0);
    s.req = 0;
    s.g = s.t = s.tend = 0;
    s.ga = s.ta = 0;
    s.gn = s.tn = 0;
  }
  __syncthreads();
  for (;;) {
    if (threadIdx.x == 0) {
      WalkState st = s.st;
      const GpState gps = s.gp;
      const uint64_t next_ev = ep.gp.n ? gp_next_event(gps, ep.gp) : ~0ull;
      uint64_t cg = s.g, ct = s.t;
      const uint64_t ctend_in = s.tend, cga = s.ga, cta = s.ta;
      uint64_t ctend = ctend_in;
      const uint32_t cgn = s.gn, ctn = s.tn;
      uint32_t req = 0, fin = 0;
      uint64_t req_idx = 0;
      for (;;) {
        if (st.a >= n) {
          fin = 1;
          break;
        }
        if (ct < ctend) {
          const uint64_t t = ct, tstart = t * (uint64_t)kTT, tend = (tstart + kTT) < n ? (tstart + kTT) : n;
          if (st.a < tend && !(t >= cta && t < cta + ctn)) {
            req = 3;
            req_idx = t;
            break;
          }
          TileState ts{st.a, st.blk, st.foff, st.f, 0};
          wk.tstate[t] = ts;
          ct++;
          if (st.a >= tend) continue;
          const uint64_t cc = st.a - tstart;
          TileRow r;
          r.exit = 0xffffffffu;
          if (cc < hc) r = tcache[(t - cta) * hc + cc];
          const bool table_ok = cc < hc && r.exit != 0xffffffffu;
          const bool cut = !table_ok || (ep.output_level != 0 && st.foff + r.bytes >= ep.max_output_file_size) || tstart + r.exit >= n ||
                           next_ev <= tstart + r.exit;
          if (cut) {
            req = 1;
            req_idx = t;
            break;
          }
          st.a = tstart + r.exit;
          st.blk += r.nblk;
          st.foff += r.bytes;
          continue;
        }
        if (cg >= ngroups) {
          fin = 1;
          break;
        }
        const uint64_t gg = cg, t0 = gg * kEncGroup, gstart = t0 * (uint64_t)kTT;
        const uint64_t t1 = (t0 + kEncGroup) < ntiles ? (t0 + kEncGroup) : ntiles;
        const uint64_t gend = (t1 * (uint64_t)kTT) < n ? (t1 * (uint64_t)kTT) : n;
        if (st.a < gend && !(gg >= cga && gg < cga + cgn)) {
          req = 2;
          req_idx = gg;
          break;
        }
        TileState gs{st.a, st.blk, st.foff, st.f, 0};
        wk.gstate[gg] = gs;
        wk.gflag[gg] = 0;
        cg++;
        if (st.a >= gend) continue;
        const uint64_t cc = st.a - gstart;
        TileRow r;
        r.exit = 0xffffffffu;
        if (cc < hc) r = gcache[(gg - cga) * hc + cc];
        const bool table_ok = cc < hc && r.exit != 0xffffffffu;
        const bool cut = !table_ok || (ep.output_level != 0 && st.foff + r.bytes >= ep.max_output_file_size) || gstart + r.exit >= n ||
                         next_ev <= gstart + r.exit;
        if (cut) {
          wk.gflag[gg] = 1;
          ct = t0;
          ctend = t1;
          continue;
        }
        st.a = gstart + r.exit;
        st.blk += r.nblk;
        st.foff += r.bytes;
      }
      s.st = st;
      s.g = cg;
      s.t = ct;
      s.tend = ctend;
      s.req = req;
      s.req_idx = req_idx;
      if (fin) s.done = 1;
    }
    __syncthreads();
    const uint32_t req = s.req;
    const uint64_t ridx = s.req_idx;
    uint32_t done = s.done;
    if (req == 2 || req == 3) {
      const uint64_t total = req == 2 ? ngroups : s.tend;
      uint32_t cnt = (uint32_t)((total - ridx) < cache_rows ? (total - ridx) : cache_rows);
      if (req == 2) {
        if (threadIdx.x == 0) {
          volatile uint32_t* rdy = wk.gready;
          if (first_wait) {
            unsigned long long t0, t1;
            asm volatile("mov.u64 %0, %globaltimer;" : "=l"(t0));
            while (rdy[ridx] == 0) {
              __nanosleep(256);
              asm volatile("mov.u64 %0, %globaltimer;" : "=l"(t1));
              if (t1 - t0 > timeout_ns) {
                s.done = 2;
                break;
              }
            }
          } else {
            while (rdy[ridx] == 0) __nanosleep(256);
          }
          uint32_t have = 1;
          while (have < cnt && rdy[ridx + have] != 0) have++;
          s.refill = have;
          __threadfence();
        }
        __syncthreads();
        if (s.done == 2) return;
        first_wait = false;
        cnt = s.refill;
      }
      const uint4* src = reinterpret_cast<const uint4*>((req == 2 ? wk.grows : wk.rows) + ridx * hc);
      uint4* dst = reinterpret_cast<uint4*>(req == 2 ? gcache : tcache);
      coop_copy_cg<uint4, 8>(dst, src, cnt * hc);
      if (threadIdx.x == 0) {
        if (req == 2) {
          s.ga = ridx;
          s.gn = cnt;
        } else {
          s.ta = ridx;
          s.tn = cnt;
        }
      }
    } else if (req == 1) {
      const uint64_t tstart = ridx * (uint64_t)kTT;
      const uint32_t tl = (uint32_t)(((tstart + kTT) < n ? (tstart + kTT) : n) - tstart);
      const uint32_t c0 = (uint32_t)(s.st.a > tstart ? (s.st.a - tstart) & ~7ull : 0);
      const uint32_t c1 = (tl + 7u) & ~7u;
      coop_copy_cg<uint4, 4>(reinterpret_cast<uint4*>(s.nxt + c0), reinterpret_cast<const uint4*>(wk.nxt + tstart + c0), (c1 - c0) / 8);
      coop_copy_cg<uint4, 8>(reinterpret_cast<uint4*>(s.disk + c0), reinterpret_cast<const uint4*>(wk.disk + tstart + c0), (c1 - c0) / 4);
      __syncthreads();
      if (ep.gp.n == 0) {
        for (uint32_t i = c0 + threadIdx.x; i < tl; i += blockDim.x) s.nd[i] = ((uint64_t)s.nxt[i] << 32) | s.disk[i];
        __syncthreads();
      }
      if (threadIdx.x == 0) {
        WalkState st = s.st;
        GpState g = s.gp;
        bool chased = true;
        if (ep.gp.n) {
          chased = chase_tile<1>(s.nxt, s.disk, tstart, tl, n, ep, m, wk, st, wk.files, nullptr, 0, err, &g);
        } else {
          const uint32_t nd_base = (uint32_t)__cvta_generic_to_shared(s.nd);
          const uint64_t left = n - tstart;
          const uint32_t nlocal = left < 0xffffull ? (uint32_t)left : 0xffffu;
          const bool cut_files = ep.output_level != 0;
          const uint64_t fmax = ep.max_output_file_size;
          uint32_t x = (uint32_t)(st.a - tstart);
          uint64_t foff = st.foff, blk = st.blk;
          while (x < tl) {
            for (;;) {
              uint64_t v;
              asm volatile("ld.shared.u64 %0, [%1];" : "=l"(v) : "r"(nd_base + 8u * x));
              const uint32_t yr = (uint32_t)(v >> 32), d = (uint32_t)v;
              const uint64_t nf = foff + d;
              if (yr <= x || yr >= nlocal || (cut_files && nf >= fmax)) break;
              foff = nf;
              blk++;
              x = yr;
              if (x >= tl) break;
            }
            if (x >= tl) break;
            st.a = tstart + x;
            st.foff = foff;
            st.blk = blk;
            chased = chase_tile<0>(s.nxt, s.disk, tstart, x + 1, n, ep, m, wk, st, wk.files, nullptr, 0, err);
            if (!chased || st.a >= n) break;
            x = (uint32_t)(st.a - tstart);
            foff = st.foff;
            blk = st.blk;
          }
          if (chased && st.a < n && x >= tl && st.a < tstart + x) {
            st.a = tstart + x;
            st.foff = foff;
            st.blk = blk;
          }
        }
        s.gp = g;
        if (!chased) {
          atomicOr(err, kErrBlockTooLong);
          s.done = 1;
        }
        s.st = st;
      }
      __syncthreads();
      done = s.done;
    }
    __syncthreads();
    if (done) break;
  }
  if (threadIdx.x == 0) {
    wk.totals[0] = s.st.blk;
    wk.totals[1] = s.st.f;
    TileState ts{n, s.st.blk, 0, s.st.f, 0};
    for (uint64_t t = s.t; t < s.tend; t++) wk.tstate[t] = ts;
    for (uint64_t gg = s.g; gg < ngroups; gg++) {
      wk.gstate[gg] = ts;
      wk.gflag[gg] = 0;
    }
    __threadfence();
    if (attempt == 1) atomicExch(sflag, 1u);
  }
}

__global__ void encode_tilestate_kernel(EncodeWork wk, uint64_t n, uint64_t ntiles, uint32_t hc, uint32_t* __restrict__ err) {
  const uint64_t g = blockIdx.x * (uint64_t)blockDim.x + threadIdx.x;
  const uint64_t ngroups = (ntiles + kEncGroup - 1) / kEncGroup;
  if (g >= ngroups || wk.gflag[g]) return;
  const TileState gs = wk.gstate[g];
  uint64_t a = gs.entry, blk = gs.blk, foff = gs.file_off;
  const uint64_t t0 = g * kEncGroup, t1 = (t0 + kEncGroup) < ntiles ? (t0 + kEncGroup) : ntiles;
  for (uint64_t t = t0; t < t1; t++) {
    const uint64_t tstart = t * (uint64_t)kTT, tend = (tstart + kTT) < n ? (tstart + kTT) : n;
    TileState ts{a < n ? a : n, blk, foff, gs.file_idx, 0};
    wk.tstate[t] = ts;
    if (a >= n || a >= tend) continue;
    const uint64_t cc = a - tstart;
    if (cc >= hc) {
      atomicOr(err, kErrBlockTooLong);
      return;
    }
    const TileRow r = wk.rows[t * hc + cc];
    if (r.exit == 0xffffffffu) {
      atomicOr(err, kErrBlockTooLong);
      return;
    }
    a = tstart + r.exit;
    blk += r.nblk;
    foff += r.bytes;
  }
}

struct BlistSmem {
  uint16_t nxt[kTT];
  uint32_t disk[kTT];
  uint8_t is_start[kTT];
  uint64_t ws[33];
  uint32_t serial;
};
__global__ void __launch_bounds__(kEncThreads)
encode_blocklist_kernel(KeyCols m, EncodeParams ep, EncodeWork wk, uint64_t n, uint64_t nblk_cap, uint32_t* __restrict__ err) {
  __shared__ BlistSmem s;
  const uint64_t tile = blockIdx.x, tstart = tile * (uint64_t)kTT;
  const uint64_t tend = (tstart + kTT) < n ? (tstart + kTT) : n;
  const uint32_t tl = (uint32_t)(tend - tstart);
  const TileState ts = wk.tstate[tile];
  if (ts.entry >= tend) return;
  for (uint32_t j = threadIdx.x; j < tl; j += kEncThreads) {
    s.nxt[j] = wk.nxt[tstart + j];
    s.disk[j] = wk.disk[tstart + j];
    s.is_start[j] = 0;
  }
  __syncthreads();
  if (threadIdx.x == 0) {
    uint32_t x = (uint32_t)(ts.entry - tstart);
    uint64_t bytes = 0;
    bool bad = false, ends = false;
    while (x < tl) {
      uint32_t y = s.nxt[x];
      if (y == 0xffff || y <= x) {
        bad = true;
        break;
      }
      s.is_start[x] = 1;
      bytes += s.disk[x];
      if (tstart + y >= n) ends = true;
      x = y;
    }
    if (bad) atomicOr(err, kErrBlockTooLong);
    bool gp_cut = false;
    if (ep.gp.n && !bad) {
      const uint32_t nc = *ep.gp_ncuts;
      uint32_t lo = 0, hi = nc;
      while (lo < hi) {
        const uint32_t mid = (lo + hi) >> 1;
        if (ep.gp_cuts[mid].entry <= ts.entry) lo = mid + 1;
        else hi = mid;
      }
      gp_cut = lo < nc && ep.gp_cuts[lo].entry <= tstart + x;
    }
    s.serial = bad ? 2 : ((ends || gp_cut || (ep.output_level != 0 && ts.file_off + bytes >= ep.max_output_file_size)) ? 1 : 0);
    if (s.serial == 1) {
      WalkState st;
      st.a = ts.entry;
      st.blk = ts.blk;
      st.foff = ts.file_off;
      st.f = ts.file_idx;
      st.f_first_entry = 0;
      st.f_first_blk = 0;
      const bool chased = ep.gp.n ? chase_tile<2>(s.nxt, s.disk, tstart, tl, n, ep, m, wk, st, nullptr, wk.blocks, nblk_cap, err)
                                  : chase_tile<0>(s.nxt, s.disk, tstart, tl, n, ep, m, wk, st, nullptr, wk.blocks, nblk_cap, err);
      if (!chased) atomicOr(err, kErrBlockTooLong);
    }
  }
  __syncthreads();
  if (s.serial != 0) return;
  constexpr int kPer = kTT / kEncThreads;
  const uint32_t j0 = threadIdx.x * kPer;
  uint32_t cnt = 0;
  uint64_t bytes = 0;
#pragma unroll
  for (int i = 0; i < kPer; i++) {
    uint32_t j = j0 + i;
    if (j < tl && s.is_start[j]) {
      cnt++;
      bytes += s.disk[j];
    }
  }
  uint64_t packed = ((uint64_t)cnt << 48) | bytes;
  uint64_t ex = block_excl_scan64(packed, nullptr, s.ws);
  uint64_t r = ts.blk + (ex >> 48), off = ts.file_off + (ex & ((1ull << 48) - 1));
#pragma unroll
  for (int i = 0; i < kPer; i++) {
    uint32_t j = j0 + i;
    if (j < tl && s.is_start[j]) {
      if (r < nblk_cap) wk.blocks[r] = BlockRec{tstart + j, off, ts.file_idx, (uint32_t)(s.nxt[j] - j)};
      r++;
      off += s.disk[j];
    }
  }
}

__device__ __forceinline__ uint64_t index_entries_bytes(const EncodeWork& wk, uint64_t b0, uint64_t nb) {
  return wk.idx_eoff[b0 + nb - 1] + wk.idx_esz[b0 + nb - 1] - wk.idx_eoff[b0];
}

__global__ void encode_filestats_kernel(KeyCols m, EncodeWork wk, uint32_t nfiles) {
  const uint32_t f = blockIdx.x;
  if (f >= nfiles) return;
  const uint64_t f0 = wk.files[f].first_entry, f1 = f0 + wk.files[f].n_entries;
  __shared__ unsigned long long red[5];
  if (threadIdx.x < 5) red[threadIdx.x] = threadIdx.x == 3 ? ~0ull : 0ull;
  __syncthreads();
  const unsigned long long kVal = (1ull << 62) - 1;
  unsigned long long kb = 0, vb = 0, nd = 0, smin = ~0ull, smax = 0;
  if (f1 > f0) {
    auto tile_start = [&](uint64_t t) -> uint64_t { return t ? (wk.tprefix[t - 1] & kVal) : 0; };
    auto first_tile_starting_at_or_after = [&](uint64_t e) -> uint64_t {
      uint64_t lo = 0, hi = wk.nstat;
      while (lo < hi) {
        const uint64_t mid = lo + ((hi - lo) >> 1);
        if (tile_start(mid) < e) lo = mid + 1;
        else hi = mid;
      }
      return lo;
    };
    const uint64_t tA = first_tile_starting_at_or_after(f0);
    uint64_t tB = 0;
    {
      uint64_t lo = 0, hi = wk.nstat;
      while (lo < hi) {
        const uint64_t mid = lo + ((hi - lo) >> 1);
        if ((wk.tprefix[mid] & kVal) <= f1) lo = mid + 1;
        else hi = mid;
      }
      tB = lo;
    }
    auto scan_entries = [&](uint64_t lo, uint64_t hi) {
      for (uint64_t i = lo + threadIdx.x; i < hi; i += blockDim.x) {
        const uint64_t tr = m.tr[i];
        const uint32_t mt = m.meta[i];
        kb += meta_ulen(mt) + 8;
        vb += meta_vlen(mt);
        nd += is_deletion_type((uint32_t)(tr & 0xff));
        const uint64_t sq = tr >> 8;
        smin = sq < smin ? sq : smin;
        smax = sq > smax ? sq : smax;
      }
    };
    if (tA >= tB) {
      scan_entries(f0, f1);
    } else {
      scan_entries(f0, tile_start(tA));
      scan_entries(wk.tprefix[tB - 1] & kVal, f1);
      for (uint64_t t = tA + threadIdx.x; t < tB; t += blockDim.x) {
        const TileStat ts = wk.tstat[t];
        kb += ts.raw_key;
        vb += ts.raw_value;
        nd += ts.deletions;
        smin = ts.smallest_seq < smin ? ts.smallest_seq : smin;
        smax = ts.largest_seq > smax ? ts.largest_seq : smax;
      }
    }
    if (threadIdx.x < 2) {
      const uint64_t i = threadIdx.x == 0 ? f0 : f1 - 1;
      const ulonglong2 p = m.pfx[i];
      const KeyRec kr{p.x, p.y, m.tr[i], meta_ulen(m.meta[i]), 0};
      if (threadIdx.x == 0) wk.files[f].smallest = kr;
      else wk.files[f].largest = kr;
    }
  }
#pragma unroll
  for (int d = 16; d; d >>= 1) {
    kb += __shfl_xor_sync(0xffffffffu, kb, d);
    vb += __shfl_xor_sync(0xffffffffu, vb, d);
    nd += __shfl_xor_sync(0xffffffffu, nd, d);
    const unsigned long long a = __shfl_xor_sync(0xffffffffu, smin, d), b = __shfl_xor_sync(0xffffffffu, smax, d);
    smin = a < smin ? a : smin;
    smax = b > smax ? b : smax;
  }
  if ((threadIdx.x & 31) == 0) {
    atomicAdd(&red[0], kb);
    atomicAdd(&red[1], vb);
    atomicAdd(&red[2], nd);
    atomicMin(&red[3], smin);
    atomicMax(&red[4], smax);
  }
  __syncthreads();
  if (threadIdx.x == 0) {
    wk.files[f].raw_key_size = red[0];
    wk.files[f].raw_value_size = red[1];
    wk.files[f].num_deletions = red[2];
    wk.files[f].smallest_seq = red[3];
    wk.files[f].largest_seq = red[4];
    const uint64_t b0 = wk.files[f].first_block, nb = wk.files[f].n_blocks;
    if (nb) wk.files[f].index_size = index_entries_bytes(wk, b0, nb) + 4 * nb + 4;
  }
}

constexpr int kEmitWarps = 4;
__device__ __forceinline__ void key_suffix_words(uint64_t hi, uint64_t lo, uint32_t ulen, uint64_t tr, uint32_t sh, uint64_t* S0,
                                                 uint64_t* S1, uint64_t* S2) {
  const uint64_t U0 = bswap64(hi), U1 = bswap64(lo);
  uint64_t I0, I1, I2;
  {
    const uint32_t ws = ulen >> 3, bs = (ulen & 7) * 8;
    const uint64_t T0 = tr << bs, T1 = bs ? tr >> (64 - bs) : 0;
    if (ws == 0) {
      I0 = U0 | T0;
      I1 = T1;
      I2 = 0;
    } else if (ws == 1) {
      I0 = U0;
      I1 = U1 | T0;
      I2 = T1;
    } else {
      I0 = U0;
      I1 = U1;
      I2 = tr;
    }
  }
  const uint32_t ws = sh >> 3, bs = (sh & 7) * 8;
  const uint64_t A = ws == 0 ? I0 : ws == 1 ? I1 : ws == 2 ? I2 : 0;
  const uint64_t B = ws == 0 ? I1 : ws == 1 ? I2 : 0;
  const uint64_t Cw = ws == 0 ? I2 : 0;
  *S0 = bs ? (A >> bs) | (B << (64 - bs)) : A;
  *S1 = bs ? (B >> bs) | (Cw << (64 - bs)) : B;
  *S2 = Cw >> bs;
}
__device__ __forceinline__ void store_stream28(uint8_t* p, const uint32_t* w, uint32_t L) {
  uint32_t head = (4 - (uint32_t)((uintptr_t)p & 3)) & 3;
  if (head > L) head = L;
  if (head > 0) p[0] = (uint8_t)w[0];
  if (head > 1) p[1] = (uint8_t)(w[0] >> 8);
  if (head > 2) p[2] = (uint8_t)(w[0] >> 16);
  const uint32_t bs = head * 8, nwords = (L - head) >> 2;
  uint32_t* d32 = reinterpret_cast<uint32_t*>(p + head);
  uint32_t tailv = 0;
#pragma unroll
  for (int k = 0; k < 7; k++) {
    const uint32_t v = __funnelshift_r(w[k], w[k + 1], bs);
    if ((uint32_t)k < nwords) d32[k] = v;
    if ((uint32_t)k == nwords) tailv = v;
  }
  const uint32_t done = head + 4 * nwords, rem = L - done;
  if (rem > 0) p[done] = (uint8_t)tailv;
  if (rem > 1) p[done + 1] = (uint8_t)(tailv >> 8);
  if (rem > 2) p[done + 2] = (uint8_t)(tailv >> 16);
}
__device__ __forceinline__ void store_bytes24(uint8_t* p, uint64_t S0, uint64_t S1, uint64_t S2, uint32_t n) {
#pragma unroll
  for (int k = 0; k < 8; k++)
    if ((uint32_t)k < n) p[k] = (uint8_t)(S0 >> (8 * k));
#pragma unroll
  for (int k = 0; k < 8; k++)
    if ((uint32_t)(8 + k) < n) p[8 + k] = (uint8_t)(S1 >> (8 * k));
#pragma unroll
  for (int k = 0; k < 8; k++)
    if ((uint32_t)(16 + k) < n) p[16 + k] = (uint8_t)(S2 >> (8 * k));
}
__device__ __forceinline__ void copy_value_small(uint8_t* dst, const uint8_t* src, uint32_t n) {
  const uint32_t a = (uint32_t)((uintptr_t)src & 3);
  const uint32_t* ws = reinterpret_cast<const uint32_t*>((uintptr_t)src - a);
  const uint32_t nw = (a + n + 3) >> 2;
  uint32_t w[18];
#pragma unroll
  for (int i = 0; i < 17; i++) w[i] = (uint32_t)i < nw ? __ldg(ws + i) : 0u;
  w[17] = 0;
  uint32_t head = (4 - (uint32_t)((uintptr_t)dst & 3)) & 3;
  if (head > n) head = n;
  {
    const uint32_t v = __funnelshift_r(w[0], w[1], a * 8);
    if (head > 0) dst[0] = (uint8_t)v;
    if (head > 1) dst[1] = (uint8_t)(v >> 8);
    if (head > 2) dst[2] = (uint8_t)(v >> 16);
  }
  const uint32_t t0 = a + head, bs = (t0 & 3) * 8;
  const uint32_t nwords = (n - head) >> 2;
  uint32_t* d32 = reinterpret_cast<uint32_t*>(dst + head);
  uint32_t last;
  if ((t0 >> 2) == 0) {
#pragma unroll
    for (int mI = 0; mI < 16; mI++)
      if ((uint32_t)mI < nwords) d32[mI] = __funnelshift_r(w[mI], w[mI + 1], bs);
    last = 0;
  } else {
#pragma unroll
    for (int mI = 0; mI < 16; mI++)
      if ((uint32_t)mI < nwords) d32[mI] = __funnelshift_r(w[mI + 1], w[mI + 2], bs);
    last = 1;
  }
// ... 338 lines not shown
#pragma unroll
    for (int i = 0; i < kEmitPerLane; i++) {
      unsigned big = __ballot_sync(0xffffffffu, vs[i] > 64);
      while (big) {
        const int sl = __ffs(big) - 1;
        big &= big - 1;
        const uint32_t vl = __shfl_sync(0xffffffffu, vs[i], sl);
        const uint32_t vo = __shfl_sync(0xffffffffu, voff[i], sl);
        emit_copy_long_value(img + vo, (const uint8_t*)(uintptr_t)c_vref[sl * kEmitPerLane + i], vl, lane);
      }
    }
    load_next();
    emit_block_finish(img, gdst, shift, body, nrest, ep.checksum, xtab, lane);
  }
  if (lane == 0) asm volatile("cp.async.bulk.wait_group 0;" ::: "memory");
  (void)err;
}

constexpr int kEmitLongWarps = 8, kEmitLongCtasPerSm = 4;
__global__ void __launch_bounds__(kEmitLongWarps * 32, kEmitLongCtasPerSm)
encode_emit_long_kernel(KeyCols m, EncodeParams ep, EncodeWork wk, uint64_t nblocks, uint8_t* const* __restrict__ out_base,
                   uint32_t slot_bytes, uint32_t* __restrict__ err) {
  extern __shared__ __align__(128) uint8_t smem[];
  __shared__ XxhLaneTab s_xtab;
  const unsigned lane = threadIdx.x & 31, w = threadIdx.x >> 5;
  uint8_t* const slot = smem + (size_t)w * slot_bytes;
  fill_xxh_lane_tab(&s_xtab);
  __syncthreads();
  const uint32_t xtab = (uint32_t)__cvta_generic_to_shared(&s_xtab);
  const uint32_t R = ep.restart_interval;
  const uint32_t rmask = (R & (R - 1)) == 0 ? R - 1 : 0xffffffffu;
  const uint64_t stride = (uint64_t)gridDim.x * kEmitLongWarps;
  for (uint64_t b = (uint64_t)blockIdx.x * kEmitLongWarps + w; b < nblocks; b += stride) {
    const BlockRec br = wk.blocks[b];
    const uint32_t E = br.n_entries;
    const uint64_t e0 = br.first_entry;
    uint8_t* const gdst = out_base[br.file_idx] + br.file_off;
    const uint32_t shift = (uint32_t)((uintptr_t)gdst & 15);
    uint8_t* const img = slot + shift;
    const uint32_t nrest = (E + R - 1) / R;
    uint32_t sz[kEmitPerLane], pk[kEmitPerLane], vs[kEmitPerLane];
    uint64_t vrf[kEmitPerLane];
    uint32_t tsum = 0;
    uint64_t inc = 0;
    bool fallback = E > (uint32_t)kEmitMaxEntries;
    if (!fallback) {
      uint32_t mtv[kEmitPerLane], shv[kEmitPerLane];
#pragma unroll
      for (int i = 0; i < kEmitPerLane; i++) {
        const uint32_t x = lane * kEmitPerLane + i;
        mtv[i] = 0;
        shv[i] = 0;
        vrf[i] = 0;
        if (x < E) {
          mtv[i] = m.meta[e0 + x];
          shv[i] = wk.eshared[e0 + x];
          vrf[i] = m.vref[e0 + x];
        }
      }
#pragma unroll
      for (int i = 0; i < kEmitPerLane; i++) {
        const uint32_t x = lane * kEmitPerLane + i;
        sz[i] = pk[i] = vs[i] = 0;
        if (x < E) {
          sz[i] = entry_pack(mtv[i], shv[i], x, R, rmask, &pk[i], &vs[i]);
          tsum += sz[i];
        }
      }
      inc = warp_incl_scan64(tsum);
      fallback = __shfl_sync(0xffffffffu, inc, 31) + 4ull * nrest + 4 + 5 + 32 + 16 > slot_bytes;
    }
    if (lane == 0) bulk_wait_read0();
    __syncwarp();
    if (fallback) {
      emit_block_warp(m, wk.eshared, br, gdst, slot, slot_bytes, R, ep.checksum, xtab);
      continue;
    }
    const uint32_t body = (uint32_t)__shfl_sync(0xffffffffu, inc, 31);
    uint32_t off[kEmitPerLane];
    {
      uint32_t run = (uint32_t)(inc - tsum);
#pragma unroll
      for (int i = 0; i < kEmitPerLane; i++) {
        off[i] = run;
        run += sz[i];
      }
    }
    uint32_t voff[kEmitPerLane];
    {
      ulonglong2 ppv[kEmitPerLane];
      uint64_t trv[kEmitPerLane];
#pragma unroll
      for (int i = 0; i < kEmitPerLane; i++) {
        const uint32_t x = lane * kEmitPerLane + i;
        ppv[i] = make_ulonglong2(0, 0);
        trv[i] = 0;
        if (x < E) {
          ppv[i] = m.pfx[e0 + x];
          trv[i] = m.tr[e0 + x];
        }
      }
#pragma unroll
      for (int i = 0; i < kEmitPerLane; i++) {
        const uint32_t x = lane * kEmitPerLane + i;
        voff[i] = 0;
        if (x < E) {
          voff[i] = emit_entry_key(img, off[i], pk[i], vs[i], ppv[i].x, ppv[i].y, trv[i], x, body, R, rmask);
        }
      }
    }
    {
      constexpr int kNW = 9;
      bool all_short = true;
#pragma unroll
      for (int i = 0; i < kEmitPerLane; i++) all_short = all_short && vs[i] <= 32;
      if (all_short) {
        uint32_t vw[kEmitPerLane][kNW + 1];
#pragma unroll
        for (int i = 0; i < kEmitPerLane; i++) {
          const uint32_t a = (uint32_t)(vrf[i] & 3);
          const uint32_t* wsrc = reinterpret_cast<const uint32_t*>((uintptr_t)vrf[i] - a);
          const uint32_t nw = vs[i] ? (a + vs[i] + 3) >> 2 : 0;
#pragma unroll
          for (int k = 0; k < kNW; k++) vw[i][k] = (uint32_t)k < nw ? __ldg(wsrc + k) : 0u;
          vw[i][kNW] = 0;
        }
#pragma unroll
        for (int i = 0; i < kEmitPerLane; i++) store_value_words<kNW>(img + voff[i], vw[i], (uint32_t)(vrf[i] & 3), vs[i]);
      } else {
#pragma unroll
        for (int i = 0; i < kEmitPerLane; i++)
          if (vs[i] && vs[i] <= 64) copy_value_small(img + voff[i], (const uint8_t*)(uintptr_t)vrf[i], vs[i]);
      }
    }
#pragma unroll
    for (int i = 0; i < kEmitPerLane; i++) {
      unsigned big = __ballot_sync(0xffffffffu, vs[i] > 64);
      while (big) {
        const int sl = __ffs(big) - 1;
        big &= big - 1;
        const uint32_t vl = __shfl_sync(0xffffffffu, vs[i], sl);
        const uint32_t vo = __shfl_sync(0xffffffffu, voff[i], sl);
        const uint64_t vrr = __shfl_sync(0xffffffffu, vrf[i], sl);
        emit_copy_long_value(img + vo, (const uint8_t*)(uintptr_t)vrr, vl, lane);
      }
    }
    emit_block_finish(img, gdst, shift, body, nrest, ep.checksum, xtab, lane);
  }
  if (lane == 0) asm volatile("cp.async.bulk.wait_group 0;" ::: "memory");
  (void)err;
}

__global__ void encode_index_sep_kernel(KeyCols m, EncodeWork wk, uint64_t nblocks) {
  for (uint64_t b = blockIdx.x * (uint64_t)blockDim.x + threadIdx.x; b < nblocks; b += (uint64_t)gridDim.x * blockDim.x) {
    const BlockRec br = wk.blocks[b];
    const uint64_t le = br.first_entry + br.n_entries - 1;
    ulonglong2 lp = m.pfx[le];
    uint32_t lul = meta_ulen(m.meta[le]);
    KeyRec sep{lp.x, lp.y, m.tr[le], lul, 0};
    const bool has_next = b + 1 < nblocks && wk.blocks[b + 1].file_idx == br.file_idx;
    if (has_next) {
      const uint64_t ne = le + 1;
      ulonglong2 np = m.pfx[ne];
      uint32_t nul = meta_ulen(m.meta[ne]);
      if (np.x == lp.x && np.y == lp.y && nul == lul) {
        atomicOr(&wk.files[br.file_idx].index_has_seq, 1u);
      } else {
        uint8_t s[kMaxUserKey], l[kMaxUserKey];
        for (uint32_t t = 0; t < lul; t++) s[t] = (uint8_t)ikey_byte(lp.x, lp.y, lul, 0, t);
        for (uint32_t t = 0; t < nul; t++) l[t] = (uint8_t)ikey_byte(np.x, np.y, nul, 0, t);
        uint32_t minl = lul < nul ? lul : nul, d = 0, tn = lul;
        while (d < minl && s[d] == l[d]) d++;
        bool changed = false;
        if (d < minl && s[d] < l[d]) {
          if (d < nul - 1 || (uint32_t)s[d] + 1 < (uint32_t)l[d]) {
            s[d]++;
            tn = d + 1;
            changed = true;
          } else {
            d++;
            while (d < tn) {
              if (s[d] < 0xff) {
                s[d]++;
                tn = d + 1;
                changed = true;
                break;
              }
              d++;
            }
          }
        }
        if (changed) {
          uint64_t hi = 0, lo = 0;
          for (uint32_t t = 0; t < 8; t++) hi = (hi << 8) | (t < tn ? s[t] : 0);
          for (uint32_t t = 8; t < 16; t++) lo = (lo << 8) | (t < tn ? s[t] : 0);
          sep = KeyRec{hi, lo, (kMaxSeq << 8) | 0x16, tn, 1};
        }
      }
    }
    wk.idx_sep[b] = sep;
  }
}
__device__ __forceinline__ uint64_t block_payload_size(const EncodeWork& wk, uint64_t b, uint64_t nblocks) {
  const BlockRec br = wk.blocks[b];
  const bool has_next = b + 1 < nblocks && wk.blocks[b + 1].file_idx == br.file_idx;
  uint64_t end = has_next ? wk.blocks[b + 1].file_off : wk.files[br.file_idx].data_size;
  return end - br.file_off - 5;
}
__global__ void encode_index_size_kernel(EncodeWork wk, uint64_t nblocks, uint32_t format_version) {
  for (uint64_t b = blockIdx.x * (uint64_t)blockDim.x + threadIdx.x; b < nblocks; b += (uint64_t)gridDim.x * blockDim.x) {
    const BlockRec br = wk.blocks[b];
    const KeyRec sep = wk.idx_sep[b];
    const uint32_t klen = sep.ulen + (wk.files[br.file_idx].index_has_seq ? 8 : 0);
    const uint32_t hlen = (uint32_t)varint_len(br.file_off) + (uint32_t)varint_len(block_payload_size(wk, b, nblocks));
    wk.idx_esz[b] = 1 + (uint32_t)varint_len(klen) + (format_version >= 4 ? 0 : (uint32_t)varint_len(hlen)) + klen + hlen;
  }
}
__global__ void encode_index_write_kernel(EncodeWork wk, uint64_t nblocks, uint32_t format_version,
                                          uint8_t* const* __restrict__ out_base) {
  for (uint64_t b = blockIdx.x * (uint64_t)blockDim.x + threadIdx.x; b < nblocks; b += (uint64_t)gridDim.x * blockDim.x) {
    const BlockRec br = wk.blocks[b];
    const FileRec& fr = wk.files[br.file_idx];
    const KeyRec sep = wk.idx_sep[b];
    const uint32_t klen = sep.ulen + (fr.index_has_seq ? 8 : 0);
    const uint64_t eoff = wk.idx_eoff[b] - wk.idx_eoff[fr.first_block];
    const uint64_t entries_bytes = index_entries_bytes(wk, fr.first_block, fr.n_blocks);
    uint8_t* ib = out_base[br.file_idx] + fr.data_size + fr.filter_bytes;
    uint8_t* p = ib + eoff;
    uint8_t h[20];
    uint32_t hn = (uint32_t)put_varint(h, br.file_off);
    hn += (uint32_t)put_varint(h + hn, block_payload_size(wk, b, nblocks));
    p += put_varint(p, 0);
    p += put_varint(p, klen);
    if (format_version < 4) p += put_varint(p, hn);
    for (uint32_t t = 0; t < klen; t++) *p++ = (uint8_t)ikey_byte(sep.hi, sep.lo, sep.ulen, sep.tr, t);
    for (uint32_t t = 0; t < hn; t++) *p++ = h[t];
    const uint64_t bi = b - fr.first_block;
    put_fixed32(ib + entries_bytes + 4 * bi, (uint32_t)eoff);
    if (bi == 0) put_fixed32(ib + entries_bytes + 4 * fr.n_blocks, (uint32_t)fr.n_blocks);
  }
}
enum FileBlock : uint32_t { kIndexBlock, kFilterBlock };
__device__ __forceinline__ uint64_t file_block(const FileRec& fr, uint32_t which, uint64_t* start) {
  if (which == kFilterBlock) {
    *start = fr.data_size;
    return fr.filter_bytes ? fr.filter_bytes - 5 : 0;
  }
  *start = fr.data_size + fr.filter_bytes;
  return fr.n_blocks ? fr.index_size : 0;
}
__global__ void file_block_contrib_kernel(const FileRec* __restrict__ files, uint32_t nfiles, uint32_t which, uint8_t* const* __restrict__ out_base,
                                          uint64_t* __restrict__ contrib, const uint64_t* __restrict__ contrib_off) {
  const uint32_t f = blockIdx.y;
  if (f >= nfiles) return;
  uint64_t start;
  const uint64_t len = file_block(files[f], which, &start);
  if (len <= 240) return;
  const uint8_t* p = out_base[f] + start;
  const uint64_t nb_blocks = (len - 1) / 1024;
  const unsigned lane = threadIdx.x & 31;
  const XxhLaneSecret ks = xxh_lane_secret();
  for (uint64_t k = (uint64_t)blockIdx.x * (blockDim.x >> 5) + (threadIdx.x >> 5); k < nb_blocks; k += (uint64_t)gridDim.x * (blockDim.x >> 5)) {
    const uint64_t part = xxh3_block_contrib<false>(p + 1024 * k, 16, ks);
    if (lane < 8) contrib[(contrib_off[f] + k) * 8 + lane] = part;
  }
}
__global__ void file_block_trailer_kernel(const FileRec* __restrict__ files, uint32_t nfiles, uint32_t which, uint32_t cksum,
                                          uint8_t* const* __restrict__ out_base, const uint64_t* __restrict__ contrib,
                                          const uint64_t* __restrict__ contrib_off) {
  const uint32_t f = blockIdx.x * (blockDim.x >> 5) + (threadIdx.x >> 5);
  if (f >= nfiles) return;
  uint64_t start;
  const uint64_t len = file_block(files[f], which, &start);
  if (len == 0) return;
  uint8_t* p = out_base[f] + start;
  uint32_t ck;
  if (cksum == 4) ck = (uint32_t)xxh3_64_warp_t<false>(p, len, contrib + contrib_off[f] * 8);
  else ck = block_checksum_warp(cksum, p, len, 0);
  if ((threadIdx.x & 31) == 0) put_block_trailer(p + len, ck);
}

__global__ void block_checksums_kernel(uint32_t type, const uint8_t* __restrict__ data, const uint64_t* __restrict__ offsets, uint32_t n,
                                       uint8_t last_byte, uint32_t* __restrict__ out) {
  const uint32_t i = blockIdx.x * (blockDim.x >> 5) + (threadIdx.x >> 5);
  if (i >= n) return;
  uint32_t ck = block_checksum_warp(type, data + offsets[i], offsets[i + 1] - offsets[i], last_byte);
  if ((threadIdx.x & 31) == 0) out[i] = ck;
}

__device__ __forceinline__ uint64_t entry_key_hash(const KeyCols& m, uint64_t e) {
  const ulonglong2 p = m.pfx[e];
  return xxph3_of_key(p.x, p.y, meta_ulen(m.meta[e]));
}
__device__ __forceinline__ uint32_t file_of_entry(const FileRec* __restrict__ files, uint32_t nfiles, uint64_t e) {
  uint32_t lo = 0, hi = nfiles;
  while (hi - lo > 1) {
    const uint32_t mid = (lo + hi) >> 1;
    if (files[mid].first_entry <= e) lo = mid;
    else hi = mid;
  }
  return lo;
}
__global__ void __launch_bounds__(256)
bloom_count_kernel(KeyCols m, uint64_t n, FileRec* __restrict__ files, const uint64_t* __restrict__ nfiles_dev, uint64_t* __restrict__ hashes) {
  const uint32_t nfiles = (uint32_t)*nfiles_dev;
  if (nfiles == 0 || nfiles > kMaxOutFiles) return;
  const unsigned lane = threadIdx.x & 31;
  constexpr int kU = 4;
  const uint64_t warp0 = ((uint64_t)blockIdx.x * blockDim.x + threadIdx.x) >> 5, nwarps = ((uint64_t)gridDim.x * blockDim.x) >> 5;
  const uint64_t per_warp = ((n + nwarps - 1) / nwarps + 32 * kU - 1) / (32 * kU) * (32 * kU);
  const uint64_t w_begin = warp0 * per_warp, w_end = w_begin + per_warp < n ? w_begin + per_warp : n;
  unsigned long long acc = 0;
  uint32_t acc_f = 0xffffffffu;
  for (uint64_t e0 = w_begin; e0 < w_end; e0 += 32 * kU) {
    ulonglong2 kp[kU];
    uint32_t km[kU];
#pragma unroll
    for (int u = 0; u < kU; u++) {
      const uint64_t e = e0 + 32 * u + lane;
      if (e < n) {
        kp[u] = m.pfx[e];
        km[u] = m.meta[e];
      }
    }
    const uint64_t e_last = e0 + 32 * kU - 1 < n ? e0 + 32 * kU - 1 : n - 1;
    const uint32_t f_lo = file_of_entry(files, nfiles, e0), f_hi = file_of_entry(files, nfiles, e_last);
    uint64_t carry = 0;
#pragma unroll
    for (int u = 0; u < kU; u++) {
      const uint64_t e = e0 + 32 * u + lane;
      uint32_t f = 0xffffffffu;
      bool add = false;
      const uint64_t h = e < n ? xxph3_of_key(kp[u].x, kp[u].y, meta_ulen(km[u])) : 0;
      if (e < n) hashes[e] = h;
      uint64_t ph = __shfl_up_sync(0xffffffffu, h, 1);
      if (lane == 0) ph = carry;
      if (e < n) {
        f = f_lo == f_hi ? f_lo : file_of_entry(files, nfiles, e);
        const uint64_t ff = files[f].first_entry;
        if (u == 0 && lane == 0 && e > ff) ph = entry_key_hash(m, e - 1);
        add = e == ff || ph != h;
      }
      carry = __shfl_sync(0xffffffffu, h, 31);
      const uint32_t f0 = __shfl_sync(0xffffffffu, f, 0);
      const bool uniform = __all_sync(0xffffffffu, f == f0 || f == 0xffffffffu);
      if (uniform) {
        const unsigned cnt = __popc(__ballot_sync(0xffffffffu, add));
        if (f0 != 0xffffffffu) {
          if (f0 != acc_f) {
            if (lane == 0 && acc) atomicAdd(reinterpret_cast<unsigned long long*>(&files[acc_f].filter_entries), acc);
            acc = 0;
            acc_f = f0;
          }
          acc += cnt;
        }
      } else if (add) {
        atomicAdd(reinterpret_cast<unsigned long long*>(&files[f].filter_entries), 1ull);
      }
    }
  }
  if (lane == 0 && acc) atomicAdd(reinterpret_cast<unsigned long long*>(&files[acc_f].filter_entries), acc);
}
__global__ void bloom_layout_kernel(FileRec* __restrict__ files, const uint64_t* __restrict__ nfiles_dev, uint32_t millibits) {
  const uint32_t nfiles = (uint32_t)*nfiles_dev;
  for (uint32_t f = blockIdx.x * blockDim.x + threadIdx.x; f < nfiles && f < kMaxOutFiles; f += gridDim.x * blockDim.x) {
    const uint64_t cnt = files[f].filter_entries;
    files[f].filter_bytes = cnt ? (uint64_t)bloom_bits_bytes(cnt, millibits) + kBloomMetadataLen + 5 : 0;
  }
}
void launch_bloom_count(KeyCols m, uint64_t n, FileRec* files, const uint64_t* nfiles_dev, uint32_t millibits, uint64_t* hashes, int sms, cudaStream_t st) {
  if (n == 0) return;
  const uint64_t blocks = (n + 1023) / 1024;
  bloom_count_kernel<<<(unsigned)(blocks < (unsigned)sms * 8 ? blocks : (unsigned)sms * 8), 256, 0, st>>>(m, n, files, nfiles_dev, hashes);
  bloom_layout_kernel<<<(kMaxOutFiles + 255) / 256, 256, 0, st>>>(files, nfiles_dev, millibits);
}
constexpr uint32_t kBloomSliceBytes = 176 * 1024;
constexpr int kBloomThreads = 1024;
constexpr uint32_t kBloomStage = 64;
__global__ void __launch_bounds__(kBloomThreads, 1)
bloom_slices_kernel(const uint64_t* __restrict__ hashes, const FileRec* __restrict__ files, uint32_t nfiles, int probes,
                    uint8_t* const* __restrict__ out_base) {
  extern __shared__ __align__(128) uint8_t bsm[];
  const uint32_t f = blockIdx.y;
  if (f >= nfiles) return;
  const FileRec& fr = files[f];
  if (fr.filter_bytes <= kBloomMetadataLen + 5) return;
  const uint32_t bits_bytes = (uint32_t)(fr.filter_bytes - kBloomMetadataLen - 5);
  const uint32_t s0 = blockIdx.x * kBloomSliceBytes;
  if (s0 >= bits_bytes) return;
  const uint32_t s1 = s0 + kBloomSliceBytes < bits_bytes ? s0 + kBloomSliceBytes : bits_bytes;
  uint8_t* const gdst = out_base[f] + fr.data_size + s0;
  const uint32_t shift = (uint32_t)((uintptr_t)gdst & 15);
  uint8_t* const img = bsm + shift;
  uint32_t* const w32 = reinterpret_cast<uint32_t*>(bsm);
  for (uint32_t i = threadIdx.x; i < (kBloomSliceBytes + 16) / 4; i += kBloomThreads) w32[i] = 0;
  __syncthreads();
  const uint64_t e0 = fr.first_entry, e1 = e0 + fr.n_entries;
  constexpr int kU = 8;
  uint64_t* const stage = reinterpret_cast<uint64_t*>(bsm + kBloomSliceBytes + 16) + (threadIdx.x >> 5) * kBloomStage;
  const unsigned lane = threadIdx.x & 31;
  uint32_t queued = 0;
  auto set_bits = [&](uint64_t h) {
    const uint32_t line = bloom_line_offset(h, bits_bytes);
    uint32_t p = bloom_first_probe(h);
    for (int k = 0; k < probes; k++, p = bloom_next_probe(p)) {
      const uint32_t bit = bloom_probe_bit(p);
      const uint32_t byte = shift + (line - s0) + (bit >> 3);
      atomicOr(&w32[byte >> 2], 1u << (8 * (byte & 3) + (bit & 7)));
    }
  };
  for (uint64_t eb = e0; eb < e1; eb += (uint64_t)kU * kBloomThreads) {
    uint64_t hv[kU], pv[kU];
#pragma unroll
    for (int u = 0; u < kU; u++) {
      const uint64_t e = eb + (uint64_t)u * kBloomThreads + threadIdx.x;
      hv[u] = pv[u] = 0;
      if (e < e1) {
        hv[u] = hashes[e];
        if (e > e0) pv[u] = hashes[e - 1];
      }
    }
#pragma unroll
    for (int u = 0; u < kU; u++) {
      const uint64_t e = eb + (uint64_t)u * kBloomThreads + threadIdx.x;
      const uint64_t h = hv[u];
      bool mine = e < e1 && !(e > e0 && pv[u] == h);
      if (mine) {
        const uint32_t line = bloom_line_offset(h, bits_bytes);
        mine = line >= s0 && line < s1;
      }
      const unsigned mask = __ballot_sync(0xffffffffu, mine);
      if (mine) stage[queued + __popc(mask & ((1u << lane) - 1u))] = h;
      queued += __popc(mask);
      __syncwarp();
      if (queued >= 32) {
        const uint64_t hq = stage[lane];
        const uint64_t rest = lane + 32 < queued ? stage[lane + 32] : 0;
        __syncwarp();
        queued -= 32;
        if (lane < queued) stage[lane] = rest;
        set_bits(hq);
        __syncwarp();
      }
    }
  }
  if (lane < queued) set_bits(stage[lane]);
  __syncthreads();
  const uint32_t total = s1 - s0;
  uint32_t head = shift ? 16 - shift : 0;
  if (head > total) head = total;
  const uint32_t mid = (total - head) & ~15u;
  fence_async_smem();
  __syncthreads();
  if (threadIdx.x == 0 && mid) {
    bulk_s2g(gdst + head, (uint32_t)__cvta_generic_to_shared(img + head), mid);
    asm volatile("cp.async.bulk.wait_group 0;" ::: "memory");
  }
  if (threadIdx.x < head) gdst[threadIdx.x] = img[threadIdx.x];
  const uint32_t done = head + mid;
  if (done + threadIdx.x < total) gdst[done + threadIdx.x] = img[done + threadIdx.x];
  if (s1 == bits_bytes && threadIdx.x == 32) {
    uint8_t* md = out_base[f] + fr.data_size + bits_bytes;
    md[0] = 0xff;
    md[1] = 0;
    md[2] = (uint8_t)probes;
    md[3] = 0;
    md[4] = 0;
  }
}
void launch_bloom_build(const uint64_t* hashes, uint64_t n, const FileRec* files, uint32_t nfiles, uint32_t max_filter_bytes, uint32_t millibits,
                        uint32_t cksum, uint8_t* const* out_base, uint64_t* contrib, const uint64_t* contrib_off, cudaStream_t st) {
  if (n == 0 || nfiles == 0) return;
  const int probes = bloom_num_probes((int)millibits);
  static PerDeviceFlag attr;
  const uint64_t dev_bit = attr.bit_of_current_device();
  const int smem = (int)kBloomSliceBytes + 16 + (kBloomThreads / 32) * kBloomStage * 8;
  if (!attr.is_set(dev_bit)) {
    cudaFuncSetAttribute(bloom_slices_kernel, cudaFuncAttributeMaxDynamicSharedMemorySize, smem);
    attr.set(dev_bit);
  }
  const unsigned slices = (max_filter_bytes + kBloomSliceBytes - 1) / kBloomSliceBytes;
  bloom_slices_kernel<<<dim3(slices ? slices : 1, nfiles), kBloomThreads, smem, st>>>(hashes, files, nfiles, probes, out_base);
  if (cksum == 4) file_block_contrib_kernel<<<dim3(32, nfiles), 256, 0, st>>>(files, nfiles, kFilterBlock, out_base, contrib, contrib_off);
  file_block_trailer_kernel<<<(nfiles + 3) / 4, 128, 0, st>>>(files, nfiles, kFilterBlock, cksum, out_base, contrib, contrib_off);
}

__global__ void gp_rank_kernel(KeyCols m, const GpKey* __restrict__ smallest, const GpKey* __restrict__ largest, uint32_t n,
                               uint64_t* __restrict__ lo, uint64_t* __restrict__ eq, uint64_t* __restrict__ hi) {
  const uint32_t i = blockIdx.x * blockDim.x + threadIdx.x;
  if (i >= n) return;
  auto bound = [&](const GpKey& k, bool upper) -> uint64_t {
    uint64_t a = 0, b = m.n;
    while (a < b) {
      const uint64_t mid = a + ((b - a) >> 1);
      const ulonglong2 p = m.pfx[mid];
      const int c = ukey_cmp(p.x, p.y, meta_ulen(m.meta[mid]), k.hi, k.lo, k.ulen);
      if (c < 0 || (upper && c == 0)) a = mid + 1;
      else b = mid;
    }
    return a;
  };
  lo[i] = bound(smallest[i], false);
  eq[i] = bound(largest[i], false);
  hi[i] = bound(largest[i], true);
}
void launch_gp_ranks(KeyCols m, const GpKey* smallest, const GpKey* largest, uint32_t n, uint64_t* lo, uint64_t* eq, uint64_t* hi,
                     cudaStream_t st) {
  if (n) gp_rank_kernel<<<(n + 63) / 64, 64, 0, st>>>(m, smallest, largest, n, lo, eq, hi);
}

__global__ void scatter_tails_kernel(const TailCopy* __restrict__ recs, const uint8_t* __restrict__ staged, uint8_t* __restrict__ out) {
  const TailCopy r = recs[blockIdx.x];
  for (uint32_t i = threadIdx.x; i < r.len; i += blockDim.x) out[r.dst_off + i] = staged[r.src_off + i];
}

__global__ void gather_small_kernel(const uint64_t* __restrict__ small, uint32_t small_words, const FileRec* __restrict__ files,
                                    const uint64_t* __restrict__ nfiles_dev, uint64_t* __restrict__ dst) {
  const uint32_t t = blockIdx.x * blockDim.x + threadIdx.x, nt = gridDim.x * blockDim.x;
  for (uint32_t i = t; i < small_words; i += nt) dst[i] = small[i];
  if (files) {
    uint64_t n = *nfiles_dev;
    if (n > kMaxOutFiles) n = kMaxOutFiles;
    const uint64_t words = n * (sizeof(FileRec) / 8);
    const uint64_t* src = reinterpret_cast<const uint64_t*>(files);
    for (uint64_t i = t; i < words; i += nt) dst[small_words + i] = src[i];
  }
}
static_assert(sizeof(FileRec) % 8 == 0, "FileRec is copied word-wise");

void launch_gather_small(const uint64_t* small, uint32_t small_bytes, const FileRec* files, const uint64_t* nfiles_dev, uint8_t* dst,
                         cudaStream_t st) {
  gather_small_kernel<<<files ? 8 : 1, 256, 0, st>>>(small, small_bytes / 8, files, nfiles_dev, reinterpret_cast<uint64_t*>(dst));
}
__global__ void copy_small_kernel(const uint8_t* __restrict__ src, uint8_t* __restrict__ dst, uint32_t n) {
  for (uint32_t i = threadIdx.x; i < n; i += blockDim.x) dst[i] = src[i];
}
void launch_copy_small(const void* src, void* dst, uint32_t n, cudaStream_t st) {
  if (n) copy_small_kernel<<<1, 256, 0, st>>>(static_cast<const uint8_t*>(src), static_cast<uint8_t*>(dst), n);
}
void launch_scatter_tails(const TailCopy* recs, uint32_t n, const uint8_t* staged, uint8_t* out, cudaStream_t st) {
  if (n) scatter_tails_kernel<<<n, 256, 0, st>>>(recs, staged, out);
}
void launch_encode_sizes(KeyCols m, const unsigned long long* n_dev, EncodeWork w, unsigned long long* tprefix_out, uint64_t n_cap,
                         int sms, cudaStream_t st) {
  if (n_cap == 0) return;
  const uint64_t tiles = (n_cap + kEncTile - 1) / kEncTile;
  encode_sizes_kernel<<<(unsigned)(tiles < (unsigned)sms * 8 ? tiles : (unsigned)sms * 8), 256, 0, st>>>(m, n_dev, w.esz, w.eshared, w.tstat, tprefix_out, w.min_s1);
}
void launch_encode_tables(KeyCols m, EncodeParams ep, EncodeWork w, uint64_t ntiles, uint32_t hc, uint32_t max_s1, uint32_t* err,
                          cudaStream_t st) {
  if (ntiles == 0) return;
  static PerDeviceFlag attr;
  const uint64_t dev_bit = attr.bit_of_current_device();
  if (!attr.is_set(dev_bit)) {
    cudaFuncSetAttribute(encode_tables_kernel<uint32_t>, cudaFuncAttributeMaxDynamicSharedMemorySize, (int)sizeof(TablesSmem<uint32_t>));
    cudaFuncSetAttribute(encode_tables_kernel<uint64_t>, cudaFuncAttributeMaxDynamicSharedMemorySize, (int)sizeof(TablesSmem<uint64_t>));
    attr.set(dev_bit);
  }
  if (((uint64_t)max_s1 + 64) * (uint64_t)(kW + 1) < (1ull << 32))
    encode_tables_kernel<uint32_t><<<(unsigned)ntiles, kEncThreads, sizeof(TablesSmem<uint32_t>), st>>>(m, ep, w, m.n, hc, w.nxt, w.disk, err);
  else
    encode_tables_kernel<uint64_t><<<(unsigned)ntiles, kEncThreads, sizeof(TablesSmem<uint64_t>), st>>>(m, ep, w, m.n, hc, w.nxt, w.disk, err);
}
void launch_encode_stitch(KeyCols m, EncodeParams ep, EncodeWork w, uint64_t ntiles, uint32_t hc, uint32_t* err, uint32_t attempt,
                          uint32_t* sflag, cudaStream_t st, uint64_t* launches) {
  if (ntiles == 0) return;
  static PerDeviceFlag attr;
  const uint64_t dev_bit = attr.bit_of_current_device();
  constexpr size_t kSolo = 200 * 1024;
  if (!attr.is_set(dev_bit)) {
    cudaFuncSetAttribute(encode_stitch_kernel, cudaFuncAttributeMaxDynamicSharedMemorySize, (int)kSolo);
    attr.set(dev_bit);
  }
  const size_t fixed = (sizeof(StitchSmem) + 15) & ~(size_t)15;
  uint32_t cache_bytes = 16 * 1024;
  while (cache_bytes < hc * (uint32_t)sizeof(TileRow)) cache_bytes *= 2;
  size_t smem = fixed + 2 * (size_t)cache_bytes;
  if (attempt == 1) {
    const uint32_t big = (uint32_t)(((kSolo - fixed) / 2) & ~(size_t)15);
    if (big > cache_bytes) cache_bytes = big;
    smem = kSolo;
  }
  encode_stitch_kernel<<<1, kEncThreads, smem, st>>>(m, ep, w, m.n, ntiles, hc, cache_bytes, err, attempt, sflag, 300000u);
  if (launches) *launches += 1;
}
void launch_encode_tilestate(KeyCols m, EncodeWork w, uint64_t ntiles, uint32_t hc, uint32_t* err, cudaStream_t st, uint64_t* launches) {
  if (ntiles == 0) return;
  const uint64_t ngroups = (ntiles + kEncGroup - 1) / kEncGroup;
  encode_tilestate_kernel<<<(unsigned)((ngroups + 63) / 64), 64, 0, st>>>(w, m.n, ntiles, hc, err);
  if (launches) *launches += 1;
}
void launch_encode_blocklist(KeyCols m, EncodeParams ep, EncodeWork w, uint64_t ntiles, uint64_t nblk_cap, uint32_t* err,
                             cudaStream_t st) {
  if (ntiles == 0) return;
  encode_blocklist_kernel<<<(unsigned)ntiles, kEncThreads, 0, st>>>(m, ep, w, m.n, nblk_cap, err);
}
void launch_encode_filestats(KeyCols m, EncodeWork w, uint32_t nfiles, cudaStream_t st) {
  if (m.n == 0 || nfiles == 0) return;
  encode_filestats_kernel<<<nfiles, 256, 0, st>>>(m, w, nfiles);
}
constexpr uint32_t kEmitMaxSmem = 224 * 1024;
uint32_t encode_emit_slice(uint32_t block_size) {
  uint32_t s = block_size + block_size / 4 + 512;
  s = (s + 255) & ~255u;
  if (s < 5632) s = 5632;
  if (s > 24 * 1024) s = 24 * 1024;
  return s;
}
static_assert(kEmitWarps * (24 * 1024 + 2 * kStageBytes) <= kEmitMaxSmem, "the largest slots and their column stages fit one CTA");
void launch_encode_emit(KeyCols m, EncodeParams ep, EncodeWork w, uint64_t nblocks, uint8_t* const* out_base, uint64_t data_bytes,
                        uint32_t* err, int sms, cudaStream_t st) {
  if (nblocks == 0) return;
  static PerDeviceFlag attr;
  const uint64_t dev_bit = attr.bit_of_current_device();
  if (!attr.is_set(dev_bit)) {
    cudaFuncSetAttribute(encode_emit_kernel, cudaFuncAttributeMaxDynamicSharedMemorySize, kEmitMaxSmem);
    cudaFuncSetAttribute(encode_emit_long_kernel, cudaFuncAttributeMaxDynamicSharedMemorySize, kEmitMaxSmem);
    attr.set(dev_bit);
  }
  const bool long_entries = data_bytes > 64 * m.n;
  const int warps = long_entries ? kEmitLongWarps : kEmitWarps, ctas = long_entries ? kEmitLongCtasPerSm : kEmitCtasPerSm;
  const uint32_t slot = encode_emit_slice(ep.block_size);
  const size_t smem = (size_t)warps * (slot + (long_entries ? 0 : 2 * kStageBytes));
  int per_sm = 0;
  cudaOccupancyMaxActiveBlocksPerMultiprocessor(&per_sm, long_entries ? (const void*)encode_emit_long_kernel : (const void*)encode_emit_kernel,
                                                warps * 32, smem);
  if (per_sm < 1) per_sm = 1;
  if (per_sm > ctas) per_sm = ctas;
  const uint64_t want = (nblocks + warps - 1) / warps;
  const uint64_t cap = (uint64_t)sms * per_sm;
  const unsigned grid = (unsigned)(want < cap ? want : cap);
  if (long_entries) encode_emit_long_kernel<<<grid, warps * 32, smem, st>>>(m, ep, w, nblocks, out_base, slot, err);
  else encode_emit_kernel<<<grid, warps * 32, smem, st>>>(m, ep, w, nblocks, out_base, slot, err);
}
static unsigned index_grid(uint64_t nblocks, int sms) {
  const uint64_t g = (nblocks + 255) / 256;
  return (unsigned)(g < (uint64_t)sms * 8 ? g : (uint64_t)sms * 8);
}
void launch_encode_index_size(KeyCols m, EncodeParams ep, EncodeWork w, uint64_t nblocks, int sms, cudaStream_t st, uint64_t* launches) {
  if (nblocks == 0) return;
  const unsigned g = index_grid(nblocks, sms);
  encode_index_sep_kernel<<<g, 256, 0, st>>>(m, w, nblocks);
  encode_index_size_kernel<<<g, 256, 0, st>>>(w, nblocks, ep.format_version);
  exclusive_scan<uint32_t>(w.idx_esz, w.idx_eoff, nblocks, w.scan_tmp, nullptr, st, launches);
  if (launches) *launches += 2;
}
void launch_encode_index_write(EncodeParams ep, EncodeWork w, uint64_t nblocks, uint32_t nfiles, uint8_t* const* out_base, int sms,
                               cudaStream_t st, uint64_t* launches) {
  if (nblocks == 0) return;
  encode_index_write_kernel<<<index_grid(nblocks, sms), 256, 0, st>>>(w, nblocks, ep.format_version, out_base);
  if (ep.checksum == 4) {
    file_block_contrib_kernel<<<dim3(64, nfiles), 256, 0, st>>>(w.files, nfiles, kIndexBlock, out_base, w.idx_contrib, w.idx_contrib_off);
    if (launches) *launches += 1;
  }
  file_block_trailer_kernel<<<(nfiles + 3) / 4, 128, 0, st>>>(w.files, nfiles, kIndexBlock, ep.checksum, out_base, w.idx_contrib, w.idx_contrib_off);
  if (launches) *launches += 2;
}
void launch_block_checksums(uint32_t type, const uint8_t* data, const uint64_t* offsets, uint32_t n, uint8_t last_byte, uint32_t* out,
                            cudaStream_t st) {
  if (n == 0) return;
  block_checksums_kernel<<<(n + 3) / 4, 128, 0, st>>>(type, data, offsets, n, last_byte, out);
}

}
```

toplingdb_b200/csrc/kernels.h:

```cpp
#pragma once
#include <cuda_runtime.h>
#include <stdint.h>

#include <atomic>

#include "common.cuh"
#include "gp_rules.h"

namespace b200c {

struct PerDeviceFlag {
  std::atomic<uint64_t> mask{0};
  uint64_t bit_of_current_device() const {
    int d = 0;
    cudaGetDevice(&d);
    return 1ull << (d & 63);
  }
  bool is_set(uint64_t bit) const { return (mask.load(std::memory_order_acquire) & bit) != 0; }
  void set(uint64_t bit) { mask.fetch_or(bit, std::memory_order_release); }
};

struct FileDesc {
  const uint8_t* base;
  uint64_t len;
  uint64_t index_off;
  uint32_t index_size;
  uint32_t value_delta;
  uint32_t cksum;
  uint32_t gblk_first;
  uint32_t nblocks;
  uint32_t index_user_key;
  const uint8_t* index_ptr;
};

struct BoundKey {
  uint64_t hi, lo;
  uint32_t ulen, pad;
};

void launch_index_decode(const FileDesc* files_dev, int nfiles, uint32_t max_blocks_per_file, uint64_t* blk_off,
                         uint32_t* blk_size, BoundKey start, uint32_t has_start, BoundKey end, uint32_t has_end, uint32_t* err, cudaStream_t st);
void launch_block_decode_fused(const FileDesc* files_dev, int nfiles, const uint64_t* blk_off, const uint32_t* blk_size, uint32_t nblk,
                               uint32_t verify, uint64_t n_total, KeyColsMut out, unsigned long long* blk_state, uint32_t* ticket,
                               uint64_t* run_start, uint64_t* total_out, uint32_t* err, int sms, cudaStream_t st,
                               const uint8_t* arena = nullptr);
void launch_block_usize(const FileDesc* files_dev, const uint64_t* blk_off, const uint32_t* blk_size, uint32_t nblk, uint32_t* slot, uint32_t* err,
                        cudaStream_t st);
void launch_inflate_blocks(const FileDesc* files_dev, uint64_t* blk_off, uint32_t* blk_size, const uint32_t* slot, const uint64_t* slot_off,
                           uint32_t nblk, uint8_t* arena, uint32_t verify, uint32_t* err, int sms, cudaStream_t st);
void launch_flip_byte(uint8_t* p, cudaStream_t st);
void launch_compare_columns(KeyCols written, KeyCols reread, uint64_t n, uint32_t* err, int sms, cudaStream_t st);
void launch_gather_values(KeyCols in, const uint64_t* dst_off, uint8_t* dst, cudaStream_t st);
void launch_meta_vlen(const uint32_t* meta, uint64_t n, uint32_t* vlen, cudaStream_t st);
void launch_kv_to_columns(const uint8_t* arena, const uint64_t* offs, const uint32_t* klens, uint64_t n, KeyColsMut out, uint32_t* err,
                          int sms, cudaStream_t st);

struct TailCopy {
  uint64_t dst_off;
  uint32_t src_off, len;
};
struct FileRec;
void launch_gather_small(const uint64_t* small, uint32_t small_bytes, const FileRec* files, const uint64_t* nfiles_dev, uint8_t* dst,
                         cudaStream_t st);
void launch_copy_small(const void* src, void* dst, uint32_t n, cudaStream_t st);
void launch_scatter_tails(const TailCopy* recs, uint32_t n, const uint8_t* staged, uint8_t* out, cudaStream_t st);

constexpr int kMergeTile = 2048;
constexpr int kSdSpill = 32;
constexpr int kMergeNominal = kMergeTile - kSdSpill;
constexpr int kMaxRuns = 64;
struct MergeParams {
  uint32_t nruns;
  uint32_t bottommost;
  uint32_t nsnapshots;
  const uint64_t* snapshots;
  uint64_t earliest_snapshot;
  uint32_t filter;
  int32_t ttl;
  int64_t now;
  uint32_t write_conflict_snapshot;
};
struct TileStat {
  uint64_t raw_key, raw_value, deletions, smallest_seq, largest_seq;
};
struct MergeSizes {
  uint32_t* esz;
  uint8_t* eshared;
  TileStat* tstat;
  uint32_t* min_s1;
};
struct MergeCounters {
  unsigned long long n_out, n_input_deletions, n_hidden, n_obsolete, raw_key_bytes, raw_value_bytes, n_silent, n_user_drop;
};
struct RunBounds {
  const uint64_t* begin;
  const uint64_t* end;
};
void launch_clip_runs(KeyCols in, RunBounds runs, uint32_t nruns, BoundKey start, uint32_t has_start, BoundKey end,
                      uint32_t has_end, uint64_t* clip, unsigned long long* totals, cudaStream_t st);
void launch_run_bounds(KeyCols in, const uint64_t* file_start, const uint32_t* run_first, uint32_t nruns, uint64_t* bounds, uint32_t* err,
                       cudaStream_t st);
void launch_merge_partition(KeyCols in, RunBounds runs, uint32_t nruns, uint64_t n_total, uint64_t ntiles,
                            uint64_t* splits, uint32_t* err, int sms, cudaStream_t st);
void launch_merge_tiles(KeyCols in, RunBounds runs, MergeParams mp, uint64_t n_total, uint64_t ntiles,
                        const uint64_t* splits, unsigned long long* tile_state, uint32_t* ticket, KeyColsMut out,
                        MergeCounters* counters, MergeSizes ms, uint32_t* err, cudaStream_t st);
void launch_merge_sizes_fix(KeyCols merged, const unsigned long long* tile_state, uint64_t ntiles, MergeSizes ms, cudaStream_t st);

struct GpCut {
  uint64_t entry;
  uint64_t block_bytes;
};
struct EncodeParams {
  uint32_t block_size, block_size_limit , restart_interval;
  uint32_t checksum, format_version, output_level;
  uint64_t max_output_file_size;
  GpCtx gp;
  GpCut* gp_cuts;
  uint32_t* gp_ncuts;
};
using GpKey = BoundKey;
void launch_bloom_count(KeyCols m, uint64_t n, FileRec* files, const uint64_t* nfiles_dev, uint32_t millibits, uint64_t* hashes, int sms, cudaStream_t st);
void launch_bloom_build(const uint64_t* hashes, uint64_t n, const FileRec* files, uint32_t nfiles, uint32_t max_filter_bytes, uint32_t millibits, uint32_t cksum,
                        uint8_t* const* out_base, uint64_t* contrib, const uint64_t* contrib_off, cudaStream_t st);
void launch_gp_ranks(KeyCols m, const GpKey* smallest, const GpKey* largest, uint32_t n, uint64_t* lo, uint64_t* eq, uint64_t* hi,
                     cudaStream_t st);
struct BlockRec {
  uint64_t first_entry;
  uint64_t file_off;
  uint32_t file_idx;
  uint32_t n_entries;
};
struct KeyRec {
  uint64_t hi, lo, tr;
  uint32_t ulen, pad;
};
struct FileRec {
  uint64_t first_entry, n_entries;
  uint64_t first_block, n_blocks;
  uint64_t data_size;
  uint64_t index_size;
  uint64_t raw_key_size, raw_value_size, num_deletions;
  uint64_t smallest_seq, largest_seq;
  KeyRec smallest, largest;
  uint32_t index_has_seq;
  uint64_t filter_entries;
  uint64_t filter_bytes;
};
struct TileRow {
  uint32_t exit;
  uint32_t nblk;
  uint64_t bytes;
};
struct TileState {
  uint64_t entry;
  uint64_t blk;
  uint64_t file_off;
  uint32_t file_idx;
  uint32_t pad;
};
constexpr int kEncTile = 4096;
constexpr int kEncHalo = 2048;
constexpr int kEncGroupTiles = 16;
constexpr uint32_t kMaxOutFiles = 4096;

struct EncodeWork {
  uint32_t* esz;
  uint8_t* eshared;
  TileStat* tstat;
  const unsigned long long* tprefix;
  uint64_t nstat;
  uint32_t* min_s1;
  TileRow* rows;
  TileRow* grows;
  TileState* gstate;
  uint32_t* gflag;
  uint32_t* gdone;
  uint32_t* gready;
  TileState* tstate;
  uint64_t* totals;
  BlockRec* blocks;
  FileRec* files;
  uint32_t* idx_esz;
  uint64_t* idx_eoff;
  KeyRec* idx_sep;
  uint64_t* scan_tmp;
  uint64_t* idx_contrib;
  uint64_t* idx_contrib_off;
  uint16_t* nxt;
  uint32_t* disk;
};
void launch_encode_sizes(KeyCols m, const unsigned long long* n_dev, EncodeWork w, unsigned long long* tprefix_out, uint64_t n_cap, int sms, cudaStream_t st);
void launch_encode_tables(KeyCols m, EncodeParams ep, EncodeWork w, uint64_t ntiles, uint32_t hc, uint32_t max_s1, uint32_t* err,
                          cudaStream_t st);
void launch_encode_stitch(KeyCols m, EncodeParams ep, EncodeWork w, uint64_t ntiles, uint32_t hc, uint32_t* err, uint32_t attempt,
                          uint32_t* sflag, cudaStream_t st, uint64_t* launches);
void launch_encode_tilestate(KeyCols m, EncodeWork w, uint64_t ntiles, uint32_t hc, uint32_t* err, cudaStream_t st, uint64_t* launches);
void launch_encode_blocklist(KeyCols m, EncodeParams ep, EncodeWork w, uint64_t ntiles, uint64_t nblk_cap, uint32_t* err,
                             cudaStream_t st);
void launch_encode_filestats(KeyCols m, EncodeWork w, uint32_t nfiles, cudaStream_t st);
uint32_t encode_emit_slice(uint32_t block_size);
void launch_encode_emit(KeyCols m, EncodeParams ep, EncodeWork w, uint64_t nblocks, uint8_t* const* out_base, uint64_t data_bytes,
                        uint32_t* err, int sms, cudaStream_t st);
void launch_encode_index_size(KeyCols m, EncodeParams ep, EncodeWork w, uint64_t nblocks, int sms, cudaStream_t st, uint64_t* launches);
void launch_encode_index_write(EncodeParams ep, EncodeWork w, uint64_t nblocks, uint32_t nfiles, uint8_t* const* out_base, int sms,
                               cudaStream_t st, uint64_t* launches);
void launch_block_checksums(uint32_t type, const uint8_t* data, const uint64_t* offsets, uint32_t n, uint8_t last_byte,
                            uint32_t* out, cudaStream_t st);

}
```

Baseline: 282,500.

## Remove host sync between merge and encode by sizing encoder from device counts

Drops the host round-trip that read merge counts and min entry size before launching the encode tables stage. Encoding is now enqueued right away, sized to the capacity bound, and reads the real entry count and halo width on the device through a new begin kernel. Both precision variants of the tables kernel are launched, with the device choosing which one runs. If the guessed halo capacity is too small, the encode is re-enqueued after the sync. This adds launches and work sized to capacity rather than the true count, in exchange for one fewer host stall.

```diff
diff --git a/toplingdb_b200/csrc/api.cu b/toplingdb_b200/csrc/api.cu
--- a/toplingdb_b200/csrc/api.cu
+++ b/toplingdb_b200/csrc/api.cu
@@ -4,6 +4,7 @@
 #include <string.h>
 
 #include <algorithm>
+#include <functional>
 #include <map>
 #include <memory>
 #include <mutex>
@@ -240,6 +241,7 @@
   DevBuf esz, eshared, tstat, nxt, disk, rows, tstate, grows, gstate, gflag, gsync, idx_contrib, idx_contrib_off, blocks, files_rec, idx_esz, idx_eoff, idx_sep, out_buf, out_base_d;
   uint64_t n_total = 0, n_out = 0, nblk_in = 0, nblocks_out = 0;
   uint32_t nfiles_out = 0, nruns = 0;
+  uint32_t hc_cap = 0;
   DevBuf bloom_contrib, bloom_contrib_off;
   DevBuf bloom_hashes;
   DevBuf kv_arena, kv_offs, kv_klens;
@@ -281,7 +283,7 @@
 
 namespace {
 
-enum { kSlotErr = 0, kSlotTicket = 1, kSlotTotalIn = 2, kSlotMinS1 = 3, kSlotTotals = 4 , kSlotDecTicket = 6, kSlotGpCuts = 7, kSlotCounters = 8 , kSlotClip = 16 , kSlotStitchDone = 18, kSlotArena = 19 , kSmallSlots = 32 };
+enum { kSlotErr = 0, kSlotTicket = 1, kSlotTotalIn = 2, kSlotMinS1 = 3, kSlotTotals = 4 , kSlotDecTicket = 6, kSlotGpCuts = 7, kSlotCounters = 8 , kSlotClip = 16 , kSlotStitchDone = 18, kSlotArena = 19 , kSlotEnc = 20 , kSmallSlots = 32 };
 
 int map_dev_err(uint32_t e) {
   e &= ~(uint32_t)kFlagHasSingleDelete;
@@ -608,106 +610,147 @@
   return B200C_OK;
 }
 
-int encode_stage(b200c_job* j, KeyCols mcols, uint64_t n_out, uint32_t min_s1, uint32_t max_s1, EncodeWork& W, uint32_t* err, uint64_t* small) {
+struct EncodeSource {
+  const unsigned long long* n_out;
+  const uint64_t* total_in;
+  uint64_t n_decoded;
+  bool clipped;
+};
+
+int enqueue_tables(b200c_job* j, KeyCols mcols, const EncodeParams& ep, const EncodeSource& src, EncodeWork& W, uint32_t* err, uint64_t* small) {
   const b200c_params& P = j->p;
+  const uint64_t n_cap = mcols.n;
+  cudaStream_t st = j->st;
+  const uint32_t hc_cap = j->hc_cap;
+  const uint64_t etiles = (n_cap + kEncTile - 1) / kEncTile;
+  const uint64_t egroups = (etiles + kEncGroupTiles - 1) / kEncGroupTiles;
+  CU(j->rows.reserve(sizeof(TileRow) * etiles * hc_cap));
+  CU(j->tstate.reserve(sizeof(TileState) * etiles));
+  CU(j->grows.reserve(sizeof(TileRow) * egroups * hc_cap));
+  CU(j->gstate.reserve(sizeof(TileState) * egroups));
+  CU(j->gflag.reserve(4 * egroups));
+  CU(j->nxt.reserve(2 * (n_cap + 1)));
+  CU(j->disk.reserve(4 * (n_cap + 1)));
+  CU(j->files_rec.reserve(sizeof(FileRec) * (kMaxOutFiles + 2)));
+  W.enc_n = small + kSlotEnc;
+  W.enc_hc = reinterpret_cast<const uint32_t*>(small + kSlotEnc + 1);
+  W.rows = j->rows.as<TileRow>();
+  W.tstate = j->tstate.as<TileState>();
+  W.grows = j->grows.as<TileRow>();
+  W.gstate = j->gstate.as<TileState>();
+  W.gflag = j->gflag.as<uint32_t>();
+  W.nxt = j->nxt.as<uint16_t>();
+  W.disk = j->disk.as<uint32_t>();
+  W.files = j->files_rec.as<FileRec>();
+  W.scan_tmp = j->scan_tmp.as<uint64_t>();
+  CU(j->gsync.reserve(8 * egroups + 16));
+  CU(cudaMemsetAsync(j->gsync.p, 0, 8 * egroups + 16, st));
+  W.gdone = j->gsync.as<uint32_t>();
+  W.gready = W.gdone + egroups;
+  uint32_t* sflag = reinterpret_cast<uint32_t*>(small + kSlotStitchDone);
+  launch_encode_begin(src.n_out, src.total_in, src.n_decoded, src.clipped, W.min_s1, err, P.block_size, hc_cap, small + kSlotEnc, sflag, st);
+  j->launches += 1;
+  if (ep.gp.n) {
+    const GpKey* keys = j->gp_keys_d.as<GpKey>();
+    uint64_t* ranks = j->gp_ranks_d.as<uint64_t>();
+    launch_gp_ranks(mcols, W.enc_n, keys, keys + ep.gp.n, ep.gp.n, ranks, ranks + ep.gp.n, ranks + 2 * ep.gp.n, st);
+    j->launches += 1;
+  }
+  CU(cudaEventRecord(j->evx[0], st));
+  CU(cudaStreamWaitEvent(j->st2, j->evx[0], 0));
+  {
+    const size_t slot = j->kt_begin("~encode.stitch", j->st2);
+    launch_encode_stitch(mcols, ep, W, etiles, hc_cap, err, 1, sflag, j->st2, &j->launches);
+    j->kt_end(slot, j->st2);
+  }
+  j->kt_begin("encode.tables");
+  launch_encode_tables(mcols, ep, W, etiles, err, st, &j->launches);
+  j->kt_end();
+  {
+    const size_t slot = j->kt_begin("~encode.stitch_retry", j->st2);
+    launch_encode_stitch(mcols, ep, W, etiles, hc_cap, err, 2, sflag, j->st2, &j->launches);
+    j->kt_end(slot, j->st2);
+  }
+  CU(cudaEventRecord(j->evx[1], j->st2));
+  CU(cudaStreamWaitEvent(st, j->evx[1], 0));
+  j->kt_begin("encode.tilestate");
+  launch_encode_tilestate(W, etiles, err, st, &j->launches);
+  j->kt_end();
+  if (P.bloom_millibits_per_key) {
+    j->kt_begin("encode.bloom_count");
+    CU(j->bloom_hashes.reserve(8 * (n_cap + 1)));
+    launch_bloom_count(mcols, W.enc_n, n_cap, W.files, small + kSlotTotals + 1, P.bloom_millibits_per_key, j->bloom_hashes.as<uint64_t>(), j->sms, st);
+    j->kt_end();
+    j->launches += 2;
+  }
+  return B200C_OK;
+}
+
+int encode_stage(b200c_job* j, const KeyCols cols, const EncodeSource& src, EncodeWork& W, uint32_t* err, uint64_t* small,
+                 const std::function<int(const uint64_t* h, uint64_t* n_out)>& counts) {
+  const b200c_params& P = j->p;
+  const uint64_t n_cap = cols.n;
   cudaStream_t st = j->st;
   uint64_t h[kSmallSlots];
   std::vector<FileRec> frs;
   std::vector<uint64_t> base_off;
+  EncodeParams ep{};
+  ep.block_size = P.block_size;
+  ep.block_size_limit = P.block_size_deviation ? (uint32_t)(((uint64_t)P.block_size * (100 - P.block_size_deviation) + 99) / 100) : 0;
+  ep.restart_interval = P.block_restart_interval;
+  ep.checksum = P.checksum;
+  ep.format_version = P.format_version;
+  ep.output_level = (uint32_t)P.output_level;
+  ep.max_output_file_size = P.max_output_file_size;
+  const bool run = n_cap && P.index_block_restart_interval == 1;
+  if (run && !j->gp_small.empty() && P.output_level > 0) {
+    const uint32_t G = (uint32_t)j->gp_small.size();
+    CU(j->gp_keys_d.reserve(sizeof(GpKey) * 2 * G));
+    CU(j->gp_ranks_d.reserve(8 * 3 * (size_t)G));
+    CU(j->gp_size_d.reserve(8 * (size_t)G));
+    CU(j->gp_same_d.reserve(G + 16));
+    CU(j->gp_cuts_d.reserve(sizeof(GpCut) * (2 * (size_t)G + 2)));
+    GpKey* keys = j->gp_keys_d.as<GpKey>();
+    if (int rc = upload_small(j, keys, j->gp_small.data(), sizeof(GpKey) * G)) return rc;
+    if (int rc = upload_small(j, keys + G, j->gp_large.data(), sizeof(GpKey) * G)) return rc;
+    if (int rc = upload_small(j, j->gp_size_d.p, j->gp_size.data(), 8 * (size_t)G)) return rc;
+    if (int rc = upload_small(j, j->gp_same_d.p, j->gp_same.data(), G)) return rc;
+    uint64_t* ranks = j->gp_ranks_d.as<uint64_t>();
+    ep.gp.n = G;
+    ep.gp.dynamic_file_size = P.level_compaction_dynamic_file_size;
+    ep.gp.lo = ranks;
+    ep.gp.eq = ranks + G;
+    ep.gp.hi = ranks + 2 * G;
+    ep.gp.size = j->gp_size_d.as<uint64_t>();
+    ep.gp.next_same = j->gp_same_d.as<uint8_t>();
+    ep.gp.target_output_file_size = P.target_output_file_size ? P.target_output_file_size : P.max_output_file_size;
+    ep.gp.max_compaction_bytes = P.max_compaction_bytes ? P.max_compaction_bytes : ep.gp.target_output_file_size * 25;
+    ep.gp_cuts = j->gp_cuts_d.as<GpCut>();
+    ep.gp_ncuts = reinterpret_cast<uint32_t*>(small + kSlotGpCuts);
+  }
+  if (run && j->hc_cap == 0) {
+    j->hc_cap = (uint32_t)std::min<uint64_t>((uint64_t)(P.block_size - 1) / 40 + 3, kEncHalo);
+  }
+  if (run)
+    if (int rc = enqueue_tables(j, cols, ep, src, W, err, small)) return rc;
+  if (int rc = checked_sync(j, h, W.files, &frs)) return rc;
+  uint64_t n_out = 0;
+  if (int rc = counts(h, &n_out)) return rc;
   if (n_out) {
+    if (n_out > n_cap) return fail(B200C_ERR_CUDA, "internal: more output entries than the encoder was sized for");
     if (P.index_block_restart_interval != 1)
       return fail(B200C_ERR_NOT_SUPPORTED, "index_block_restart_interval != 1 is not built on the device");
-    EncodeParams ep{};
-    ep.block_size = P.block_size;
-    ep.block_size_limit = P.block_size_deviation ? (uint32_t)(((uint64_t)P.block_size * (100 - P.block_size_deviation) + 99) / 100) : 0;
-    ep.restart_interval = P.block_restart_interval;
-    ep.checksum = P.checksum;
-    ep.format_version = P.format_version;
-    ep.output_level = (uint32_t)P.output_level;
-    ep.max_output_file_size = P.max_output_file_size;
-    if (!j->gp_small.empty() && P.output_level > 0) {
-      const uint32_t G = (uint32_t)j->gp_small.size();
-      CU(j->gp_keys_d.reserve(sizeof(GpKey) * 2 * G));
-      CU(j->gp_ranks_d.reserve(8 * 3 * (size_t)G));
-      CU(j->gp_size_d.reserve(8 * (size_t)G));
-      CU(j->gp_same_d.reserve(G + 16));
-      CU(j->gp_cuts_d.reserve(sizeof(GpCut) * (2 * (size_t)G + 2)));
-      GpKey* keys = j->gp_keys_d.as<GpKey>();
-      if (int rc = upload_small(j, keys, j->gp_small.data(), sizeof(GpKey) * G)) return rc;
-      if (int rc = upload_small(j, keys + G, j->gp_large.data(), sizeof(GpKey) * G)) return rc;
-      if (int rc = upload_small(j, j->gp_size_d.p, j->gp_size.data(), 8 * (size_t)G)) return rc;
-      if (int rc = upload_small(j, j->gp_same_d.p, j->gp_same.data(), G)) return rc;
-      uint64_t* ranks = j->gp_ranks_d.as<uint64_t>();
-      launch_gp_ranks(mcols, keys, keys + G, G, ranks, ranks + G, ranks + 2 * G, st);
-      j->launches += 1;
-      ep.gp.n = G;
-      ep.gp.dynamic_file_size = P.level_compaction_dynamic_file_size;
-      ep.gp.lo = ranks;
-      ep.gp.eq = ranks + G;
-      ep.gp.hi = ranks + 2 * G;
-      ep.gp.size = j->gp_size_d.as<uint64_t>();
-      ep.gp.next_same = j->gp_same_d.as<uint8_t>();
-      ep.gp.target_output_file_size = P.target_output_file_size ? P.target_output_file_size : P.max_output_file_size;
-      ep.gp.max_compaction_bytes = P.max_compaction_bytes ? P.max_compaction_bytes : ep.gp.target_output_file_size * 25;
-      ep.gp_cuts = j->gp_cuts_d.as<GpCut>();
-      ep.gp_ncuts = reinterpret_cast<uint32_t*>(small + kSlotGpCuts);
-    }
-    uint64_t hop = (uint64_t)(P.block_size - 1) / std::max<uint32_t>(min_s1, 1) + 3;
-    if (hop > (uint64_t)kEncHalo) return fail(B200C_ERR_NOT_SUPPORTED, "block_size / smallest entry exceeds the encoder's 2048-entry block window");
-    const uint32_t hc = (uint32_t)hop;
+    if ((uint32_t)h[kSlotEnc + 1] > (uint32_t)kEncHalo)
+      return fail(B200C_ERR_NOT_SUPPORTED, "block_size / smallest entry exceeds the encoder's 2048-entry block window");
+    if (h[kSlotEnc + 1] >> 32) {
+      j->hc_cap = (uint32_t)h[kSlotEnc + 1];
+      if (int rc = enqueue_tables(j, cols, ep, src, W, err, small)) return rc;
+      if (int rc = checked_sync(j, h, W.files, &frs)) return rc;
+    }
+    if (h[kSlotEnc] != n_out) return fail(B200C_ERR_CUDA, "internal: the encoder did not run on the merged entries");
+    KeyCols mcols = cols;
+    mcols.n = n_out;
     const uint64_t etiles = (n_out + kEncTile - 1) / kEncTile;
-    CU(j->rows.reserve(sizeof(TileRow) * etiles * hc));
-    CU(j->tstate.reserve(sizeof(TileState) * etiles));
-    const uint64_t egroups = (etiles + kEncGroupTiles - 1) / kEncGroupTiles;
-    CU(j->grows.reserve(sizeof(TileRow) * egroups * hc));
-    CU(j->gstate.reserve(sizeof(TileState) * egroups));
-    CU(j->gflag.reserve(4 * egroups));
-    CU(j->nxt.reserve(2 * (n_out + 1)));
-    CU(j->disk.reserve(4 * (n_out + 1)));
-    CU(j->files_rec.reserve(sizeof(FileRec) * (kMaxOutFiles + 2)));
-    W.rows = j->rows.as<TileRow>();
-    W.tstate = j->tstate.as<TileState>();
-    W.grows = j->grows.as<TileRow>();
-    W.gstate = j->gstate.as<TileState>();
-    W.gflag = j->gflag.as<uint32_t>();
-    W.nxt = j->nxt.as<uint16_t>();
-    W.disk = j->disk.as<uint32_t>();
-    W.files = j->files_rec.as<FileRec>();
-    W.scan_tmp = j->scan_tmp.as<uint64_t>();
-    CU(j->gsync.reserve(8 * egroups + 16));
-    CU(cudaMemsetAsync(j->gsync.p, 0, 8 * egroups + 16, st));
-    W.gdone = j->gsync.as<uint32_t>();
-    W.gready = W.gdone + egroups;
-    uint32_t* sflag = reinterpret_cast<uint32_t*>(small + kSlotStitchDone);
-    CU(cudaEventRecord(j->evx[0], st));
-    CU(cudaStreamWaitEvent(j->st2, j->evx[0], 0));
-    {
-      const size_t slot = j->kt_begin("~encode.stitch", j->st2);
-      launch_encode_stitch(mcols, ep, W, etiles, hc, err, 1, sflag, j->st2, &j->launches);
-      j->kt_end(slot, j->st2);
-    }
-    j->kt_begin("encode.tables");
-    launch_encode_tables(mcols, ep, W, etiles, hc, max_s1, err, st);
-    j->kt_end();
-    {
-      const size_t slot = j->kt_begin("~encode.stitch_retry", j->st2);
-      launch_encode_stitch(mcols, ep, W, etiles, hc, err, 2, sflag, j->st2, &j->launches);
-      j->kt_end(slot, j->st2);
-    }
-    CU(cudaEventRecord(j->evx[1], j->st2));
-    CU(cudaStreamWaitEvent(st, j->evx[1], 0));
-    j->kt_begin("encode.tilestate");
-    launch_encode_tilestate(mcols, W, etiles, hc, err, st, &j->launches);
-    j->kt_end();
-    j->launches += 1;
-    if (P.bloom_millibits_per_key) {
-      j->kt_begin("encode.bloom_count");
-      CU(j->bloom_hashes.reserve(8 * (n_out + 1)));
-      launch_bloom_count(mcols, n_out, W.files, small + kSlotTotals + 1, P.bloom_millibits_per_key, j->bloom_hashes.as<uint64_t>(), j->sms, st);
-      j->kt_end();
-      j->launches += 2;
-    }
-    if (int rc = checked_sync(j, h, W.files, &frs)) return rc;
     const uint64_t nblocks = j->nblocks_out = h[kSlotTotals];
     const uint32_t nfiles = j->nfiles_out = (uint32_t)h[kSlotTotals + 1];
     if (nfiles == 0 || nfiles > kMaxOutFiles) return fail(B200C_ERR_CUDA, "internal: bad output file count");
@@ -1114,33 +1157,38 @@
     j->launches += 3;
   }
   CU(cudaEventRecord(j->ev[2], st));
-  uint64_t h[kSmallSlots];
-  if (int rc = checked_sync(j, h)) return rc;
-  if (clipped ? h[kSlotTotalIn] > n_decoded : h[kSlotTotalIn] != n_decoded)
-    return fail(B200C_ERR_CORRUPTION, "decoded entry count differs from rocksdb.num.entries");
-  MergeCounters mc;
-  memcpy(&mc, h + kSlotCounters, sizeof mc);
-  const uint64_t n_out = mc.n_out;
-  j->n_out = n_out;
-  j->stats.num_output_records = n_out;
-  j->stats.num_input_deletion_records = mc.n_input_deletions;
-  j->stats.num_records_replaced = mc.n_hidden;
-  j->stats.num_expired_deletion_records = mc.n_obsolete;
-  j->stats.num_record_drop_user = mc.n_user_drop;
-  j->stats.total_input_raw_key_bytes = mc.raw_key_bytes;
-  {
-    uint64_t all = 0;
-    for (auto& in : j->inputs) all += in.tail.raw_value_size;
-    if (clipped) all = range_value_bytes;
-    j->stats.total_input_raw_value_bytes = all - mc.raw_value_bytes;
-  }
+  auto merge_results = [&](const uint64_t* h, uint64_t* n_out) {
+    if (clipped ? h[kSlotTotalIn] > n_decoded : h[kSlotTotalIn] != n_decoded)
+      return fail(B200C_ERR_CORRUPTION, "decoded entry count differs from rocksdb.num.entries");
+    MergeCounters mc;
+    memcpy(&mc, h + kSlotCounters, sizeof mc);
+    *n_out = mc.n_out;
+    j->n_out = mc.n_out;
+    j->stats.num_output_records = mc.n_out;
+    j->stats.num_input_deletion_records = mc.n_input_deletions;
+    j->stats.num_records_replaced = mc.n_hidden;
+    j->stats.num_expired_deletion_records = mc.n_obsolete;
+    j->stats.num_record_drop_user = mc.n_user_drop;
+    j->stats.total_input_raw_key_bytes = mc.raw_key_bytes;
+    {
+      uint64_t all = 0;
+      for (auto& in : j->inputs) all += in.tail.raw_value_size;
+      if (clipped) all = range_value_bytes;
+      j->stats.total_input_raw_value_bytes = all - mc.raw_value_bytes;
+    }
+    return (int)B200C_OK;
+  };
   if (until == 2) {
+    uint64_t h[kSmallSlots], n_out;
+    if (int rc = checked_sync(j, h)) return rc;
+    if (int rc = merge_results(h, &n_out)) return rc;
     j->stage_done = 2;
     j->stats.kernel_launches = j->launches;
     return B200C_OK;
   }
 
-  if (int rc = encode_stage(j, j->mrg.cols(n_out), n_out, (uint32_t)h[kSlotMinS1], (uint32_t)(h[kSlotMinS1] >> 32), W, err, small)) return rc;
+  const EncodeSource src{&counters->n_out, small + kSlotTotalIn, n_decoded, clipped};
+  if (int rc = encode_stage(j, j->mrg.cols(N), src, W, err, small, merge_results)) return rc;
   return finish_run(j);
 }
 
@@ -1181,10 +1229,11 @@
     j->kt_end();
     j->launches++;
   }
-  uint64_t h[kSmallSlots];
-  rc = checked_sync(j, h);
-  if (rc) return rc;
-  rc = encode_stage(j, mcols, n, (uint32_t)h[kSlotMinS1], (uint32_t)(h[kSlotMinS1] >> 32), W, err, small);
+  const EncodeSource src{&counters->n_out, nullptr, 0, false};
+  rc = encode_stage(j, mcols, src, W, err, small, [&](const uint64_t*, uint64_t* n_out) {
+    *n_out = n;
+    return (int)B200C_OK;
+  });
   if (rc) return rc;
   j->n_out = n;
   j->stats.num_output_records = n;
diff --git a/toplingdb_b200/csrc/encode.cu b/toplingdb_b200/csrc/encode.cu
--- a/toplingdb_b200/csrc/encode.cu
+++ b/toplingdb_b200/csrc/encode.cu
@@ -399,13 +399,15 @@
   uint16_t nxt[kTT];
   uint32_t disk[kTT];
 };
+__device__ __forceinline__ bool narrow_window(uint32_t max_s1) { return ((uint64_t)max_s1 + 64) * (uint64_t)(kW + 1) < (1ull << 32); }
 template <typename PT>
 __global__ void __launch_bounds__(kEncThreads, sizeof(PT) == 4 ? 3 : 2)
-encode_tables_kernel(KeyCols m, EncodeParams ep, EncodeWork wk, uint64_t n, uint32_t hc, uint16_t* __restrict__ g_nxt,
-                     uint32_t* __restrict__ g_disk, uint32_t* __restrict__ err) {
+encode_tables_kernel(KeyCols m, EncodeParams ep, EncodeWork wk, uint16_t* __restrict__ g_nxt, uint32_t* __restrict__ g_disk,
+                     uint32_t* __restrict__ err) {
   extern __shared__ __align__(16) uint8_t smem_raw[];
   TablesSmem<PT>& s = *reinterpret_cast<TablesSmem<PT>*>(smem_raw);
-  const uint64_t tile = blockIdx.x, wstart = tile * (uint64_t)kTT;
+  const uint64_t n = *wk.enc_n, tile = blockIdx.x, wstart = tile * (uint64_t)kTT;
+  if (wstart >= n || narrow_window(wk.min_s1[1]) != (sizeof(PT) == 4)) return;
   const CutParams cp = make_cut(ep.block_size, ep.block_size_limit, ep.restart_interval);
   build_window(s.w, m, wk.esz, wk.eshared, n, tile, cp.R);
   const uint32_t tl = s.w.wlen < (uint32_t)kTT ? s.w.wlen : (uint32_t)kTT;
@@ -441,6 +443,7 @@
     g_disk[wstart + j] = s.disk[j];
   }
   __syncthreads();
+  const uint32_t hc = *wk.enc_hc;
   for (uint32_t c = threadIdx.x; c < hc; c += kEncThreads) {
     uint32_t x = c, nb = 0;
     uint64_t bytes = 0;
@@ -465,7 +468,7 @@
   __threadfence();
   __syncthreads();
   __shared__ uint32_t s_last;
-  const uint64_t g = tile / kEncGroupTiles, ntiles = (n + kTT - 1) / kTT;
+  const uint64_t g = tile / kEncGroupTiles, ntiles = (*wk.enc_n + kTT - 1) / kTT;
   const uint64_t t0 = g * kEncGroupTiles, t1 = (t0 + kEncGroupTiles) < ntiles ? (t0 + kEncGroupTiles) : ntiles;
   if (threadIdx.x == 0) s_last = atomicAdd(&wk.gdone[g], 1u) + 1 == (uint32_t)(t1 - t0);
   __syncthreads();
@@ -650,6 +653,30 @@
   uint32_t done;
   uint32_t refill;
 };
+__device__ __forceinline__ uint64_t cross_rows(const TileRow* cache, uint64_t first, uint64_t i, uint64_t end, uint64_t span, uint32_t hc,
+                                               uint64_t n, uint64_t next_ev, bool cut_files, uint64_t fmax, WalkState& st,
+                                               TileState* __restrict__ states, uint32_t* __restrict__ flags) {
+  if (i < first || i >= end) return i;
+  uint64_t base = i * span;
+  if (st.a < base || st.a - base >= hc) return i;
+  uint32_t cc = (uint32_t)(st.a - base), row = (uint32_t)(i - first) * hc;
+  while (i < end) {
+    const TileRow r = cache[row + cc];
+    const uint64_t ex = base + r.exit;
+    if (r.exit == 0xffffffffu || (cut_files && st.foff + r.bytes >= fmax) || ex >= n || next_ev <= ex) break;
+    states[i] = TileState{st.a, st.blk, st.foff, st.f, 0};
+    if (flags) flags[i] = 0;
+    st.a = ex;
+    st.blk += r.nblk;
+    st.foff += r.bytes;
+    i++;
+    base += span;
+    row += hc;
+    if (ex < base || ex - base >= hc) break;
+    cc = (uint32_t)(ex - base);
+  }
+  return i;
+}
 template <typename T, int kDepth>
 __device__ __forceinline__ void coop_copy_cg(T* __restrict__ dst, const T* __restrict__ src, uint32_t n) {
   const uint32_t nt = blockDim.x;
@@ -668,11 +695,13 @@
   }
 }
 __global__ void __launch_bounds__(kEncThreads)
-encode_stitch_kernel(KeyCols m, EncodeParams ep, EncodeWork wk, uint64_t n, uint64_t ntiles, uint32_t hc, uint32_t cache_bytes,
-                     uint32_t* __restrict__ err, uint32_t attempt, uint32_t* __restrict__ sflag, uint32_t timeout_ns) {
+encode_stitch_kernel(KeyCols m, EncodeParams ep, EncodeWork wk, uint32_t cache_bytes, uint32_t* __restrict__ err, uint32_t attempt,
+                     uint32_t* __restrict__ sflag, uint32_t timeout_ns) {
   extern __shared__ __align__(16) uint8_t smem_raw[];
   StitchSmem& s = *reinterpret_cast<StitchSmem*>(smem_raw);
   if (attempt == 2 && *reinterpret_cast<volatile uint32_t*>(sflag) != 0) return;
+  const uint64_t n = *wk.enc_n, ntiles = (n + kTT - 1) / kTT;
+  const uint32_t hc = *wk.enc_hc;
   bool first_wait = attempt == 1;
   TileRow* gcache = reinterpret_cast<TileRow*>(smem_raw + ((sizeof(StitchSmem) + 15) & ~(size_t)15));
   TileRow* tcache = gcache + cache_bytes / sizeof(TileRow);
@@ -709,6 +738,10 @@
           break;
         }
         if (ct < ctend) {
+          const uint64_t tl_end = ctend < ntiles - 1 ? ctend : ntiles - 1;
+          ct = cross_rows(tcache, cta, ct, cta + ctn < tl_end ? cta + ctn : tl_end, kTT, hc, n, next_ev, ep.output_level != 0,
+                          ep.max_output_file_size, st, wk.tstate, nullptr);
+          if (ct >= ctend) continue;
           const uint64_t t = ct, tstart = t * (uint64_t)kTT, tend = (tstart + kTT) < n ? (tstart + kTT) : n;
           if (st.a < tend && !(t >= cta && t < cta + ctn)) {
             req = 3;
@@ -740,6 +773,8 @@
           fin = 1;
           break;
         }
+        cg = cross_rows(gcache, cga, cg, cga + cgn < ngroups - 1 ? cga + cgn : ngroups - 1, (uint64_t)kEncGroup * kTT, hc, n, next_ev,
+                        ep.output_level != 0, ep.max_output_file_size, st, wk.gstate, wk.gflag);
         const uint64_t gg = cg, t0 = gg * kEncGroup, gstart = t0 * (uint64_t)kTT;
         const uint64_t t1 = (t0 + kEncGroup) < ntiles ? (t0 + kEncGroup) : ntiles;
         const uint64_t gend = (t1 * (uint64_t)kTT) < n ? (t1 * (uint64_t)kTT) : n;
@@ -905,10 +940,12 @@
   }
 }
 
-__global__ void encode_tilestate_kernel(EncodeWork wk, uint64_t n, uint64_t ntiles, uint32_t hc, uint32_t* __restrict__ err) {
+__global__ void encode_tilestate_kernel(EncodeWork wk, uint32_t* __restrict__ err) {
   const uint64_t g = blockIdx.x * (uint64_t)blockDim.x + threadIdx.x;
+  const uint64_t n = *wk.enc_n, ntiles = (n + kTT - 1) / kTT;
   const uint64_t ngroups = (ntiles + kEncGroup - 1) / kEncGroup;
   if (g >= ngroups || wk.gflag[g]) return;
+  const uint32_t hc = *wk.enc_hc;
   const TileState gs = wk.gstate[g];
   uint64_t a = gs.entry, blk = gs.blk, foff = gs.file_off;
   const uint64_t t0 = g * kEncGroup, t1 = (t0 + kEncGroup) < ntiles ? (t0 + kEncGroup) : ntiles;
@@ -1853,9 +1890,11 @@
   return lo;
 }
 __global__ void __launch_bounds__(256)
-bloom_count_kernel(KeyCols m, uint64_t n, FileRec* __restrict__ files, const uint64_t* __restrict__ nfiles_dev, uint64_t* __restrict__ hashes) {
+bloom_count_kernel(KeyCols m, const uint64_t* __restrict__ n_dev, FileRec* __restrict__ files, const uint64_t* __restrict__ nfiles_dev,
+                   uint64_t* __restrict__ hashes) {
   const uint32_t nfiles = (uint32_t)*nfiles_dev;
   if (nfiles == 0 || nfiles > kMaxOutFiles) return;
+  const uint64_t n = *n_dev;
   const unsigned lane = threadIdx.x & 31;
   constexpr int kU = 4;
   const uint64_t warp0 = ((uint64_t)blockIdx.x * blockDim.x + threadIdx.x) >> 5, nwarps = ((uint64_t)gridDim.x * blockDim.x) >> 5;
@@ -1919,10 +1958,11 @@
     files[f].filter_bytes = cnt ? (uint64_t)bloom_bits_bytes(cnt, millibits) + kBloomMetadataLen + 5 : 0;
   }
 }
-void launch_bloom_count(KeyCols m, uint64_t n, FileRec* files, const uint64_t* nfiles_dev, uint32_t millibits, uint64_t* hashes, int sms, cudaStream_t st) {
-  if (n == 0) return;
-  const uint64_t blocks = (n + 1023) / 1024;
-  bloom_count_kernel<<<(unsigned)(blocks < (unsigned)sms * 8 ? blocks : (unsigned)sms * 8), 256, 0, st>>>(m, n, files, nfiles_dev, hashes);
+void launch_bloom_count(KeyCols m, const uint64_t* n_dev, uint64_t n_cap, FileRec* files, const uint64_t* nfiles_dev, uint32_t millibits,
+                        uint64_t* hashes, int sms, cudaStream_t st) {
+  if (n_cap == 0) return;
+  const uint64_t blocks = (n_cap + 1023) / 1024;
+  bloom_count_kernel<<<(unsigned)(blocks < (unsigned)sms * 8 ? blocks : (unsigned)sms * 8), 256, 0, st>>>(m, n_dev, files, nfiles_dev, hashes);
   bloom_layout_kernel<<<(kMaxOutFiles + 255) / 256, 256, 0, st>>>(files, nfiles_dev, millibits);
 }
 constexpr uint32_t kBloomSliceBytes = 176 * 1024;
@@ -2036,12 +2076,14 @@
   file_block_trailer_kernel<<<(nfiles + 3) / 4, 128, 0, st>>>(files, nfiles, kFilterBlock, cksum, out_base, contrib, contrib_off);
 }
 
-__global__ void gp_rank_kernel(KeyCols m, const GpKey* __restrict__ smallest, const GpKey* __restrict__ largest, uint32_t n,
-                               uint64_t* __restrict__ lo, uint64_t* __restrict__ eq, uint64_t* __restrict__ hi) {
+__global__ void gp_rank_kernel(KeyCols m, const uint64_t* __restrict__ n_dev, const GpKey* __restrict__ smallest,
+                               const GpKey* __restrict__ largest, uint32_t n, uint64_t* __restrict__ lo, uint64_t* __restrict__ eq,
+                               uint64_t* __restrict__ hi) {
   const uint32_t i = blockIdx.x * blockDim.x + threadIdx.x;
   if (i >= n) return;
+  const uint64_t entries = *n_dev;
   auto bound = [&](const GpKey& k, bool upper) -> uint64_t {
-    uint64_t a = 0, b = m.n;
+    uint64_t a = 0, b = entries;
     while (a < b) {
       const uint64_t mid = a + ((b - a) >> 1);
       const ulonglong2 p = m.pfx[mid];
@@ -2055,9 +2097,9 @@
   eq[i] = bound(largest[i], false);
   hi[i] = bound(largest[i], true);
 }
-void launch_gp_ranks(KeyCols m, const GpKey* smallest, const GpKey* largest, uint32_t n, uint64_t* lo, uint64_t* eq, uint64_t* hi,
-                     cudaStream_t st) {
-  if (n) gp_rank_kernel<<<(n + 63) / 64, 64, 0, st>>>(m, smallest, largest, n, lo, eq, hi);
+void launch_gp_ranks(KeyCols m, const uint64_t* n_dev, const GpKey* smallest, const GpKey* largest, uint32_t n, uint64_t* lo, uint64_t* eq,
+                     uint64_t* hi, cudaStream_t st) {
+  if (n) gp_rank_kernel<<<(n + 63) / 64, 64, 0, st>>>(m, n_dev, smallest, largest, n, lo, eq, hi);
 }
 
 __global__ void scatter_tails_kernel(const TailCopy* __restrict__ recs, const uint8_t* __restrict__ staged, uint8_t* __restrict__ out) {
@@ -2098,8 +2140,22 @@
   const uint64_t tiles = (n_cap + kEncTile - 1) / kEncTile;
   encode_sizes_kernel<<<(unsigned)(tiles < (unsigned)sms * 8 ? tiles : (unsigned)sms * 8), 256, 0, st>>>(m, n_dev, w.esz, w.eshared, w.tstat, tprefix_out, w.min_s1);
 }
-void launch_encode_tables(KeyCols m, EncodeParams ep, EncodeWork w, uint64_t ntiles, uint32_t hc, uint32_t max_s1, uint32_t* err,
-                          cudaStream_t st) {
+__global__ void encode_begin_kernel(const unsigned long long* __restrict__ n_src, const uint64_t* __restrict__ total_in, uint64_t n_decoded,
+                                    uint32_t clipped, const uint32_t* __restrict__ min_s1, const uint32_t* __restrict__ err, uint32_t block_size,
+                                    uint32_t hc_cap, uint64_t* __restrict__ enc, uint32_t* __restrict__ sflag) {
+  const uint64_t hop = (uint64_t)(block_size - 1) / (*min_s1 ? *min_s1 : 1u) + 3;
+  bool run = (*err & ~(uint32_t)kFlagHasSingleDelete) == 0 && hop <= (uint64_t)kEncHalo;
+  if (total_in) run = run && (clipped ? *total_in <= n_decoded : *total_in == n_decoded);
+  const bool redo = run && hop > hc_cap;
+  enc[0] = run && !redo ? (uint64_t)*n_src : 0;
+  enc[1] = (hop < 0xffffffffull ? hop : 0xffffffffull) | (redo ? 1ull << 32 : 0);
+  *sflag = 0;
+}
+void launch_encode_begin(const unsigned long long* n_src, const uint64_t* total_in, uint64_t n_decoded, uint32_t clipped, const uint32_t* min_s1,
+                         const uint32_t* err, uint32_t block_size, uint32_t hc_cap, uint64_t* enc, uint32_t* sflag, cudaStream_t st) {
+  encode_begin_kernel<<<1, 1, 0, st>>>(n_src, total_in, n_decoded, clipped, min_s1, err, block_size, hc_cap, enc, sflag);
+}
+void launch_encode_tables(KeyCols m, EncodeParams ep, EncodeWork w, uint64_t ntiles, uint32_t* err, cudaStream_t st, uint64_t* launches) {
   if (ntiles == 0) return;
   static PerDeviceFlag attr;
   const uint64_t dev_bit = attr.bit_of_current_device();
@@ -2108,12 +2164,11 @@
     cudaFuncSetAttribute(encode_tables_kernel<uint64_t>, cudaFuncAttributeMaxDynamicSharedMemorySize, (int)sizeof(TablesSmem<uint64_t>));
     attr.set(dev_bit);
   }
-  if (((uint64_t)max_s1 + 64) * (uint64_t)(kW + 1) < (1ull << 32))
-    encode_tables_kernel<uint32_t><<<(unsigned)ntiles, kEncThreads, sizeof(TablesSmem<uint32_t>), st>>>(m, ep, w, m.n, hc, w.nxt, w.disk, err);
-  else
-    encode_tables_kernel<uint64_t><<<(unsigned)ntiles, kEncThreads, sizeof(TablesSmem<uint64_t>), st>>>(m, ep, w, m.n, hc, w.nxt, w.disk, err);
-}
-void launch_encode_stitch(KeyCols m, EncodeParams ep, EncodeWork w, uint64_t ntiles, uint32_t hc, uint32_t* err, uint32_t attempt,
+  encode_tables_kernel<uint32_t><<<(unsigned)ntiles, kEncThreads, sizeof(TablesSmem<uint32_t>), st>>>(m, ep, w, w.nxt, w.disk, err);
+  encode_tables_kernel<uint64_t><<<(unsigned)ntiles, kEncThreads, sizeof(TablesSmem<uint64_t>), st>>>(m, ep, w, w.nxt, w.disk, err);
+  if (launches) *launches += 2;
+}
+void launch_encode_stitch(KeyCols m, EncodeParams ep, EncodeWork w, uint64_t ntiles, uint32_t hc_cap, uint32_t* err, uint32_t attempt,
                           uint32_t* sflag, cudaStream_t st, uint64_t* launches) {
   if (ntiles == 0) return;
   static PerDeviceFlag attr;
@@ -2125,20 +2180,20 @@
   }
   const size_t fixed = (sizeof(StitchSmem) + 15) & ~(size_t)15;
   uint32_t cache_bytes = 16 * 1024;
-  while (cache_bytes < hc * (uint32_t)sizeof(TileRow)) cache_bytes *= 2;
+  while (cache_bytes < hc_cap * (uint32_t)sizeof(TileRow)) cache_bytes *= 2;
   size_t smem = fixed + 2 * (size_t)cache_bytes;
   if (attempt == 1) {
     const uint32_t big = (uint32_t)(((kSolo - fixed) / 2) & ~(size_t)15);
     if (big > cache_bytes) cache_bytes = big;
     smem = kSolo;
   }
-  encode_stitch_kernel<<<1, kEncThreads, smem, st>>>(m, ep, w, m.n, ntiles, hc, cache_bytes, err, attempt, sflag, 300000u);
+  encode_stitch_kernel<<<1, kEncThreads, smem, st>>>(m, ep, w, cache_bytes, err, attempt, sflag, 300000u);
   if (launches) *launches += 1;
 }
-void launch_encode_tilestate(KeyCols m, EncodeWork w, uint64_t ntiles, uint32_t hc, uint32_t* err, cudaStream_t st, uint64_t* launches) {
+void launch_encode_tilestate(EncodeWork w, uint64_t ntiles, uint32_t* err, cudaStream_t st, uint64_t* launches) {
   if (ntiles == 0) return;
   const uint64_t ngroups = (ntiles + kEncGroup - 1) / kEncGroup;
-  encode_tilestate_kernel<<<(unsigned)((ngroups + 63) / 64), 64, 0, st>>>(w, m.n, ntiles, hc, err);
+  encode_tilestate_kernel<<<(unsigned)((ngroups + 63) / 64), 64, 0, st>>>(w, err);
   if (launches) *launches += 1;
 }
 void launch_encode_blocklist(KeyCols m, EncodeParams ep, EncodeWork w, uint64_t ntiles, uint64_t nblk_cap, uint32_t* err,
diff --git a/toplingdb_b200/csrc/kernels.h b/toplingdb_b200/csrc/kernels.h
--- a/toplingdb_b200/csrc/kernels.h
+++ b/toplingdb_b200/csrc/kernels.h
@@ -120,11 +120,12 @@
   uint32_t* gp_ncuts;
 };
 using GpKey = BoundKey;
-void launch_bloom_count(KeyCols m, uint64_t n, FileRec* files, const uint64_t* nfiles_dev, uint32_t millibits, uint64_t* hashes, int sms, cudaStream_t st);
+void launch_bloom_count(KeyCols m, const uint64_t* n_dev, uint64_t n_cap, FileRec* files, const uint64_t* nfiles_dev, uint32_t millibits,
+                        uint64_t* hashes, int sms, cudaStream_t st);
 void launch_bloom_build(const uint64_t* hashes, uint64_t n, const FileRec* files, uint32_t nfiles, uint32_t max_filter_bytes, uint32_t millibits, uint32_t cksum,
                         uint8_t* const* out_base, uint64_t* contrib, const uint64_t* contrib_off, cudaStream_t st);
-void launch_gp_ranks(KeyCols m, const GpKey* smallest, const GpKey* largest, uint32_t n, uint64_t* lo, uint64_t* eq, uint64_t* hi,
-                     cudaStream_t st);
+void launch_gp_ranks(KeyCols m, const uint64_t* n_dev, const GpKey* smallest, const GpKey* largest, uint32_t n, uint64_t* lo, uint64_t* eq,
+                     uint64_t* hi, cudaStream_t st);
 struct BlockRec {
   uint64_t first_entry;
   uint64_t file_off;
@@ -171,6 +172,8 @@
   const unsigned long long* tprefix;
   uint64_t nstat;
   uint32_t* min_s1;
+  const uint64_t* enc_n;
+  const uint32_t* enc_hc;
   TileRow* rows;
   TileRow* grows;
   TileState* gstate;
@@ -191,11 +194,12 @@
   uint32_t* disk;
 };
 void launch_encode_sizes(KeyCols m, const unsigned long long* n_dev, EncodeWork w, unsigned long long* tprefix_out, uint64_t n_cap, int sms, cudaStream_t st);
-void launch_encode_tables(KeyCols m, EncodeParams ep, EncodeWork w, uint64_t ntiles, uint32_t hc, uint32_t max_s1, uint32_t* err,
-                          cudaStream_t st);
-void launch_encode_stitch(KeyCols m, EncodeParams ep, EncodeWork w, uint64_t ntiles, uint32_t hc, uint32_t* err, uint32_t attempt,
+void launch_encode_begin(const unsigned long long* n_src, const uint64_t* total_in, uint64_t n_decoded, uint32_t clipped, const uint32_t* min_s1,
+                         const uint32_t* err, uint32_t block_size, uint32_t hc_cap, uint64_t* enc, uint32_t* sflag, cudaStream_t st);
+void launch_encode_tables(KeyCols m, EncodeParams ep, EncodeWork w, uint64_t ntiles, uint32_t* err, cudaStream_t st, uint64_t* launches);
+void launch_encode_stitch(KeyCols m, EncodeParams ep, EncodeWork w, uint64_t ntiles, uint32_t hc_cap, uint32_t* err, uint32_t attempt,
                           uint32_t* sflag, cudaStream_t st, uint64_t* launches);
-void launch_encode_tilestate(KeyCols m, EncodeWork w, uint64_t ntiles, uint32_t hc, uint32_t* err, cudaStream_t st, uint64_t* launches);
+void launch_encode_tilestate(EncodeWork w, uint64_t ntiles, uint32_t* err, cudaStream_t st, uint64_t* launches);
 void launch_encode_blocklist(KeyCols m, EncodeParams ep, EncodeWork w, uint64_t ntiles, uint64_t nblk_cap, uint32_t* err,
                              cudaStream_t st);
 void launch_encode_filestats(KeyCols m, EncodeWork w, uint32_t nfiles, cudaStream_t st);
```

Result: faster. 286,400, median of 6 (+1.4%).
